# sidfeels/cosmos-predict2.5

Measured on AMD Instinct MI355X. Metric: frames/sec, Predict2.5-2B Image2World 720p×121f, 35 UniPC steps, CP=1/8, higher is better.
Workload: dtype bf16

## Files before the change

cosmos-predict2.5_amd/cosmos_predict2/_native.py:

```python

from __future__ import annotations

import ctypes
import os
from typing import Dict, NamedTuple, Optional, Tuple

import torch

_DEFAULT_LIB_PATH = os.path.join(os.path.dirname(os.path.abspath(__file__)), "_lib", "libcp25.so")
_LIB_PATH = _DEFAULT_LIB_PATH
_lib: Optional[ctypes.CDLL] = None

c_int64_p = ctypes.POINTER(ctypes.c_int64)


class UniPCParams(ctypes.Structure):

    _fields_ = [
        ("sigma", ctypes.c_float),
        ("use_corr", ctypes.c_int),
        ("order_c", ctypes.c_int),
        ("c_a", ctypes.c_float),
        ("c_b", ctypes.c_float),
        ("c_c", ctypes.c_float),
        ("c_inv_rk", ctypes.c_float),
        ("c_rho0", ctypes.c_float),
        ("c_rho_last", ctypes.c_float),
        ("order_p", ctypes.c_int),
        ("p_a", ctypes.c_float),
        ("p_b", ctypes.c_float),
        ("p_c", ctypes.c_float),
        ("p_inv_rk", ctypes.c_float),
        ("p_rho0", ctypes.c_float),
    ]


class CP25Tensor(ctypes.Structure):

    _fields_ = [
        ("data", ctypes.c_void_p),
        ("dtype", ctypes.c_int32),
        ("ndim", ctypes.c_int32),
        ("shape", ctypes.c_int64 * 6),
        ("strides", ctypes.c_int64 * 6),
    ]


DT_BF16, DT_F32, DT_F8E4M3, DT_U8 = 1, 2, 3, 4
_DTYPES = {torch.bfloat16: DT_BF16, torch.float32: DT_F32, torch.float8_e4m3fn: DT_F8E4M3, torch.uint8: DT_U8}

_P = ctypes.c_void_p
_I64 = ctypes.c_int64
_I = ctypes.c_int
_F = ctypes.c_float
_D = ctypes.c_double
_T =ctypes.POINTER(CP25Tensor)

SIGNATURES = {
    "cp25_attn_fwd": [_P, _P, _P, _P, _I, _I, _I, _I, _I, c_int64_p, c_int64_p, c_int64_p, c_int64_p, _F, _P],
    "cp25_attn_fwd_split": [_P, _P, _P, _P, _I, _I, _I, _I, _I, c_int64_p, c_int64_p, c_int64_p, c_int64_p, _F, _I,
                            _P, ctypes.c_size_t, _P],
    "cp25_attn_fwd_bounded": [_P, _P, _P, _P, _I, _I, _I, _I, _I, c_int64_p, c_int64_p, c_int64_p, c_int64_p, _F, _F,
                              _F, _I, _P, ctypes.c_size_t, _P],
    "cp25_attn_fwd_prescaled_kslots": [_P, _P, _P, _P, _I, _I, _I, _I, _I, c_int64_p, c_int64_p, c_int64_p, c_int64_p,
                                       _F, _F, _P, _I, _I, _P, ctypes.c_size_t, _P],
    "cp25_attn_fwd_prescaled": [_P, _P, _P, _P, _I, _I, _I, _I, _I, c_int64_p, c_int64_p, c_int64_p, c_int64_p, _F,
                                _F, _I, _P, ctypes.c_size_t, _P],
    "cp25_attn_fwd_prescaled_fp8qk": [_P, _P, _P, _P, _I, _I, _I, _I, _I, c_int64_p, c_int64_p, c_int64_p, c_int64_p, _F,
                                _F, _I, _P, ctypes.c_size_t, _P],
    "cp25_cast_fp8_e4m3": [_P, _I64, _P, _I64, _I64, _I64, _F, _P],
    "cp25_attn_fwd_prescaled_fp8": [_P, _P, _P, _P, _P, _I, _I, _I, _I, _I, c_int64_p, c_int64_p, c_int64_p, _F, _F, _I,
                                    _P, ctypes.c_size_t, _P],
    "cp25_v_fp8t_bytes": [_I, _I, _I],
    "cp25_cast_v_fp8t": [_P, c_int64_p, _I, _I, _I, _I, _P, _P, _P],
    "cp25_attn_fwd_prescaled_qnorm": [_P, _P, _P, _P, _I, _I, _I, _I, _I, c_int64_p, c_int64_p, c_int64_p, c_int64_p, _F,
                                      _F, _P, _I, _P, _P, _P, _F, _F, _I, _P, ctypes.c_size_t, _P],
    "cp25_attn_workspace_bytes": [_I, _I, _I, _I],
    "cp25_attn_tail_workspace_bytes": [_I, _I, _I, _I],
    "cp25_attn_kernel": [_I, _F, _F, _F, _I, _I],
    "cp25_attn_plan": [_I, _I, _I, _I, _I],
    "cp25_attn_na3d": [_P, _P, _P, _P, _I, _I, _I, _I, _I, _I, c_int64_p, c_int64_p, c_int64_p, c_int64_p, _P, _P, _I, _I,
                       ctypes.POINTER(ctypes.c_int), ctypes.POINTER(ctypes.c_int), _F, _I, _P],
    "cp25_ln_mod": [_P, _I64, _I64, _P, _P, _P, _P, _I64, _I64, _P, _P, _I64, _I, _I, _I64, _I64, _F, _P],
    "cp25_ln_mod_fp8": [_P, _I64, _I64, _P, _P, _P, _P, _I64, _I64, _P, _P, _P, _I64, _I, _I, _I64, _I64, _F, _P],
    "cp25_ln_mod_cam": [_P, _I64, _I64, _P, _P, _P, _P, _I64, _I64, _P, _I64, _I64, _P, _P, _I64, _I, _I, _I64, _I64, _F,
                        _P],
    "cp25_ln_mod_cam_fp8": [_P, _I64, _I64, _P, _P, _P, _P, _I64, _I64, _P, _I64, _I64, _P, _P, _P, _I64, _I, _I, _I64,
                            _I64, _F, _P],
    "cp25_plucker_tokens": [_P, _P, _P, _I, _I, _I, _P],
    "cp25_final_ln_mod": [_P, _P, _P, _I64, _I64, _P, _P, _I64, _I64, _P, _I64, _I, _I, _I64, _I64, _F, _P],
    "cp25_layer_norm": [_P, _I64, _P, _P, _P, _I64, _I64, _I, _F, _P],
    "cp25_head_rmsnorm_rope": [_P, _I64, _I64, _I, _I, _I, _P, _P, _P, _P, _I64, _F, _P],
    "cp25_head_rmsnorm_rope_scaled": [_P, _I64, _I64, _I, _I, _I, _P, _P, _P, _P, _I64, _F, _F, _P],
    "cp25_head_rmsnorm_rope_nmax": [_P, _I64, _I64, _I, _I, _I, _P, _P, _P, _P, _I64, _F, _F, _P, _P],
    "cp25_copy_rows": [_P, _I64, _P, _I64, _I64, _I64, _P],
    "cp25_gelu": [_P, _I64, _P],
    "cp25_gemm_epi": [_P, _I64, _P, _I64, _P, _I64, _I, _I, _I, _I, _P],
    "cp25_gemm_f32": [_P, _I64, _I64, _P, _I64, _I64, _P, _I64, _I64, _P, _I64, _I64, _I, _I, _I, _I, _I, _P, _I64,
                      _P],
    "cp25_gemm_f32_workspace_floats": [_I, _I, _I, _I],
    "cp25_gemm_hnorm": [_P, _I64, _P, _I64, _P, _I64, _I, _I, _I, _P, _F, _F, _P],
    "cp25_gemm_qkv": [_P, _I64, _P, _I64, _P, _I64, _I, _I, _I, _I, _I, _P, _P, _P, _I, _F, _P],
    "cp25_gemm_res": [_P, _I64, _P, _I64, _P, _I64, _I, _I, _I, _P, _I64, _I64, _P, _I64, _I64, _I, _I64, _I64, _P],
    "cp25_gemm_sm_epi": [_P, _I64, _P, _I64, _P, _I64, _I, _I, _I, _I, _I, _P, _I64, _P],
    "cp25_gemm_sm_res": [_P, _I64, _P, _I64, _P, _I64, _I, _I, _I, _P, _I64, _I64, _P, _I64, _I64, _I, _I64, _I64, _I, _P,
                         _I64, _P],
    "cp25_gemm_sm_hnorm": [_P, _I64, _P, _I64, _P, _I64, _I, _I, _I, _P, _F, _F, _I, _P, _I64, _P],
    "cp25_gemm_sm_qkv": [_P, _I64, _P, _I64, _P, _I64, _I, _I, _I, _I, _I, _P, _P, _P, _I, _F, _I, _P, _I64, _P],
    "cp25_gemm_sm_plan": [_I, _I, _I, _I, _I],
    "cp25_gemm_sm_workspace_bytes": [_I, _I, _I, _I],
    "cp25_gemm_fp8": [_P, _I64, _P, _P, _I64, _P, _P, _I64, _I, _I, _I, _P],
    "cp25_gemm_fp8_res": [_P, _I64, _P, _P, _I64, _P, _P, _I64, _I, _I, _I, _P, _I64, _I64, _P, _I64, _I64, _I, _I64,
                          _I64, _P],
    "cp25_quant_fp8_rows": [_P, _P, _P, _I64, _I64, _P],
    "cp25_gelu_quant_fp8": [_P, _P, _P, _I64, _I64, _P],
    "cp25_patchify": [_P, _P, _P, _P, _P, _I64, _I64, _I64, _P],
    "cp25_patchify_ld": [_P, _P, _P, _P, _P, _I64, _I64, _I64, _I64, _P],
    "cp25_cfg_velocity": [_P, _I, _P, _P, _P, _F, _I, _P, _I64, _I64, _I64, _P],
    "cp25_trig_patchify_ld": [_P, _P, _P, _P, _D, _P, _P, _I64, _I64, _I64, _I64, _P],
    "cp25_trig_x0_step": [_P, _P, _P, _P, _P, _P, _P, _I, _D, _D, _D, _I, _I64, _I64, _I64, _P],
    "cp25_kv_put": [_P, _I64, _I64, _I64, _I64, _P, _P, _I64, _I64, _I64, _I, _I64, _I64, _P],
    "cp25_stream_patchify_ld": [_P, _F, _F, _P, _P, _I64, _I64, _P],
    "cp25_stream_x0_step": [_P, _P, _P, _P, _F, _F, _F, _F, _D, _I, _I64, _P],
    "cp25_unipc_step": [_P, _P, _P, _P, _P, _I64, ctypes.POINTER(UniPCParams), _P],
    "cp25_conv3d": [ctypes.POINTER(ctypes.c_void_p), _I, _P, _P, _P, _P, _I, _I, _I, _I, _I, _I, _I, _I, _I, _I,
                    _I, _I, _I, _I, _I, _I, _P],
    "cp25_rms_norm_silu": [_P, _P, _P, _I64, _I, _I, _P],
    "cp25_conv3d_select": [_I],
    "cp25_attn_cross_select": [_I],
    "cp25_attn_self_select": [_I],
    "cp25_softmax_rows": [_P, _I64, _I, _I64, _F, _P, _I64, _P],
    "cp25_vae_attn": [_P, _I64, _I64, _P, _I64, _I64, _P, _I64, _I64, _P, _I64, _I64, _I, _I, _I, _I, _F, _P, _I64,
                      _P],
    "cp25_vae_attn_workspace_bytes": [_I, _I, _I, _I],
    "cp25_attn_fwd_t": [_T, _T, _T, _T, _F, _P, ctypes.c_size_t, _P],
    "cp25_gemm_epi_t": [_T, _T, _T, _I, _P],
    "cp25_conv3d_t": [_T, _I, _T, _T, _T, _I, _I, _I, _I, _I, _I, _P],
    "cp25_resize_crop_u8": [_P, c_int64_p, _I, _I, _I, _I, _P, c_int64_p, _P, _P, _P, _I, _P, _P, _P, _I, _I, _I, _I,
                            _I, _I, _I, _P],
    "cp25_u8_to_clip": [_P, c_int64_p, _I, _I, _I, _I, _P, _P],
    "cp25_clip_to_u8": [_P, c_int64_p, _I, _I, _I, _I, _P, c_int64_p, _P],
    "cp25_lora_merge": [_P, _I64, _P, _P, _I64, _I64, _I, _F, _P],
}


def library_path() -> str:
    return _LIB_PATH


def load_library() -> ctypes.CDLL:
    global _lib
    if _lib is not None:
        return _lib
    if not os.path.exists(_LIB_PATH):
        raise RuntimeError(
            f"libcp25.so not found at {_LIB_PATH}: build it with `make -C cosmos-predict2.5_amd/csrc` "
            "(or __graft_entry__.build()). There is no non-native fallback."
        )
    lib = ctypes.CDLL(_LIB_PATH)
    lab = os.path.abspath(_LIB_PATH) != os.path.abspath(_DEFAULT_LIB_PATH)
    for name, argtypes in SIGNATURES.items():
        fn = getattr(lib, name, None)
        if fn is None:
            if argtypes is None or lab:
                continue
            raise RuntimeError(f"libcp25.so does not export {name}")
        if argtypes is not None:
            fn.argtypes = argtypes
        fn.restype = {"cp25_attn_workspace_bytes": ctypes.c_size_t, "cp25_attn_tail_workspace_bytes": ctypes.c_size_t, "cp25_v_fp8t_bytes": ctypes.c_int64,
                      "cp25_gemm_f32_workspace_floats": ctypes.c_int64,
                      "cp25_gemm_sm_workspace_bytes": ctypes.c_int64,
                      "cp25_attn_kernel": ctypes.c_char_p,
                      "cp25_vae_attn_workspace_bytes": ctypes.c_int64}.get(name, ctypes.c_int)
    _lib = lib
    return lib


_ERRORS = {-22: "invalid shape/stride/pointer", -95: "unsupported dtype/size", -5: "kernel launch failed"}


def _check(name: str, rc: int) -> None:
    if rc != 0:
        msg = f"{name} failed with code {rc} ({_ERRORS.get(rc, 'unknown')})"
        if rc == -5:
            raise RuntimeError(msg)
        raise ValueError(msg)


def _ptr(t: Optional[torch.Tensor]) -> Optional[int]:
    if t is None:
        return None
    if not t.is_cuda:
        raise RuntimeError("cp25 kernels need device (HBM) tensors; got a CPU tensor")
    return t.data_ptr()


def _stream(device: torch.device) -> int:
    return torch.cuda.current_stream(device).cuda_stream


def tensor_desc(t: Optional[torch.Tensor]) -> Optional[CP25Tensor]:
    if t is None:
        return None
    if t.dim() > 6:
        raise ValueError(f"cp25_tensor holds at most 6 dimensions, got {t.dim()}")
    if t.dtype not in _DTYPES:
        raise ValueError(f"no cp25 dtype for {t.dtype}")
    d = CP25Tensor()
    d.data = _ptr(t)
    d.dtype = _DTYPES[t.dtype]
    d.ndim = t.dim()
    for i in range(t.dim()):
        d.shape[i] = t.shape[i]
        d.strides[i] = t.stride(i)
    return d


def _ref(d: Optional[CP25Tensor]):
    return None if d is None else ctypes.byref(d)


def attn_fwd_t(q: torch.Tensor, k: torch.Tensor, v: torch.Tensor, o: torch.Tensor, softmax_scale: float,
               workspace: Optional[torch.Tensor] = None) -> torch.Tensor:
    lib = load_library()
    ws = 0 if workspace is None else workspace.numel() * workspace.element_size()
    _check("cp25_attn_fwd_t", lib.cp25_attn_fwd_t(*(_ref(tensor_desc(t)) for t in (q, k, v, o)), float(softmax_scale),
                                                  _ptr(workspace), ws, _stream(q.device)))
    return o


def gemm_epi_t(a: torch.Tensor, w: torch.Tensor, c: torch.Tensor, epilogue: int = 0) -> torch.Tensor:
    lib = load_library()
    _check("cp25_gemm_epi_t", lib.cp25_gemm_epi_t(_ref(tensor_desc(a)), _ref(tensor_desc(w)), _ref(tensor_desc(c)),
                                                  int(epilogue), _stream(a.device)))
    return c


def conv3d_t(x: torch.Tensor, weight: torch.Tensor, bias: Optional[torch.Tensor], out: torch.Tensor, *,
             pad_front: int = 0, stride_t: int = 1, stride_hw: int = 1, pad: tuple = (0, 0, 0, 0)) -> torch.Tensor:
    lib = load_library()
    _check("cp25_conv3d_t", lib.cp25_conv3d_t(_ref(tensor_desc(x)), int(pad_front), _ref(tensor_desc(weight)),
                                              _ref(tensor_desc(bias)), _ref(tensor_desc(out)), stride_t, stride_hw,
                                              pad[0], pad[1], pad[2], pad[3], _stream(x.device)))
    return out


def _i64x3(vals) -> ctypes.Array:
    arr = (ctypes.c_int64 * 3)(*[int(v) for v in vals])
    return arr


_ATTN_SPLIT: Optional[int] = int(os.environ["CP25_ATTN_SPLIT"]) if os.environ.get("CP25_ATTN_SPLIT") else None


def set_attn_split(n: Optional[int]) -> Optional[int]:
    global _ATTN_SPLIT
    prev, _ATTN_SPLIT = _ATTN_SPLIT, (None if n is None else int(n))
    return prev


def attn_plan(B: int, H: int, Lq: int, Lk: int, D: int = 128) -> int:
    n = load_library().cp25_attn_plan(B, H, Lq, Lk, D)
    _check("cp25_attn_plan", min(n, 0))
    return n


def attn_fwd(q: torch.Tensor, k: torch.Tensor, v: torch.Tensor, out: Optional[torch.Tensor] = None,
             softmax_scale: Optional[float] = None, n_split: Optional[int] = None,
             norm_bounds: Optional[Tuple[float, float]] = None, prescaled: bool = False,
             fp8_qk: Optional[Tuple[torch.Tensor, torch.Tensor]] = None,
             fp8_v: Optional[Tuple[torch.Tensor, torch.Tensor]] = None,
             k_norm_slots: Optional[torch.Tensor] = None, q_norm: Optional[dict] = None) -> torch.Tensor:
    lib = load_library()
    if q.dtype != torch.bfloat16 or k.dtype != torch.bfloat16 or v.dtype != torch.bfloat16:
        raise ValueError("attn_fwd expects bf16 q/k/v (attention() recasts to bf16 first)")
    B, Lq, H, D = q.shape
    Bk, Lk, Hk, Dk = k.shape
    if (Bk, Hk, Dk) != (B, H, D) or tuple(v.shape) != tuple(k.shape):
        raise ValueError(f"shape mismatch q{tuple(q.shape)} k{tuple(k.shape)} v{tuple(v.shape)}")
    for t in (q, k, v):
        if t.stride(3) != 1:
            raise ValueError("head dim must be contiguous")
    if out is None:
        out = torch.empty((B, Lq, H, D), dtype=torch.bfloat16, device=q.device)
    scale = float(D) ** -0.5 if softmax_scale is None else float(softmax_scale)
    planned = n_split is None and not _ATTN_SPLIT
    if n_split is None:
        n_split = min(_ATTN_SPLIT, (Lk + 63) // 64) if _ATTN_SPLIT else attn_plan(B, H, Lq, Lk, D)
    ws_bytes = lib.cp25_attn_workspace_bytes(B, H, Lq, n_split)
    if planned and n_split == 1 and fp8_qk is None and k_norm_slots is None:
        ws_bytes = lib.cp25_attn_tail_workspace_bytes(B, H, Lq, Lk)
    ws = torch.empty(((ws_bytes + 15) // 16 * 4,), dtype=torch.float32, device=q.device) if ws_bytes else None
    qb, kb = (0.0, 0.0) if norm_bounds is None else (float(norm_bounds[0]), float(norm_bounds[1]))
    if not (qb >= 0.0 and kb >= 0.0):
        raise ValueError(f"norm_bounds must be >= 0, got {norm_bounds}")
    strides = [_i64x3((t.stride(0), t.stride(1), t.stride(2))) for t in (q, k, v, out)]
    if prescaled:
        if fp8_qk is not None:
            if q_norm is not None:
                raise ValueError("q_norm: the fp8 forms read e4m3 copies of the normalised q")
            if qb * kb > 60.0 or qb <= 0.0 or kb <= 0.0:
                raise ValueError(f"fp8 Q K^T needs norm bounds with product <= 60, got {norm_bounds}")
            q8, k8 = fp8_qk
            if q8.dtype != torch.uint8 or k8.dtype != torch.uint8 or q8.shape != q.shape or k8.shape != k.shape:
                raise ValueError("fp8_qk: uint8 (e4m3 bit pattern) views shaped like q and k expected")
            if q8.stride(3) != 1 or k8.stride(3) != 1:
                raise ValueError("fp8_qk: head dim must be contiguous")
            strides[0] = _i64x3((q8.stride(0), q8.stride(1), q8.stride(2)))
            strides[1] = _i64x3((k8.stride(0), k8.stride(1), k8.stride(2)))
            if fp8_v is not None:
                if 1.13 * qb * kb > 30.0:
                    raise ValueError(f"fp8 P.V needs 1.13 x the norm-bound product <= 30, got {norm_bounds}")
                v8t, amax = fp8_v
                if v8t.dtype != torch.uint8 or v8t.numel() != lib.cp25_v_fp8t_bytes(B, H, Lk) or \
                        amax.dtype != torch.float32 or amax.numel() < B * H:
                    raise ValueError("fp8_v: (v8t uint8 of cp25_v_fp8t_bytes, v_amax float32 [B*H]) expected")
                rc = lib.cp25_attn_fwd_prescaled_fp8(_ptr(q8), _ptr(k8), _ptr(v8t), _ptr(amax), _ptr(out), B, H, Lq, Lk,
                                                     D, strides[0], strides[1], strides[3], qb, kb, int(n_split),
                                                     _ptr(ws), ws_bytes, _stream(q.device))
                _check("cp25_attn_fwd_prescaled_fp8", rc)
                return out
            rc = lib.cp25_attn_fwd_prescaled_fp8qk(_ptr(q8), _ptr(k8), _ptr(v), _ptr(out), B, H, Lq, Lk, D, *strides,
                                                   qb, kb, int(n_split), _ptr(ws), ws_bytes, _stream(q.device))
            _check("cp25_attn_fwd_prescaled_fp8qk", rc)
            return out
        if k_norm_slots is not None:
            if k_norm_slots.dtype != torch.float32 or k_norm_slots.numel() != 2048 or not k_norm_slots.is_contiguous():
                raise ValueError("k_norm_slots: a contiguous float32 [64, 32] slot buffer expected")
        if q_norm is not None:
            w, cos, sin = q_norm["weight"], q_norm.get("cos"), q_norm.get("sin")
            if w.dtype != torch.bfloat16 or w.numel() != D or not w.is_contiguous() or w.device != q.device:
                raise ValueError("q_norm: weight must be a contiguous bf16 [128] device tensor")
            if (cos is None) != (sin is None):
                raise ValueError("q_norm: cos and sin go together")
            if cos is not None:
                for t in (cos, sin):
                    if t.dtype != torch.float32 or not t.is_contiguous() or t.dim() != 2 or t.shape[1] != 64 or \
                            t.shape[0] < Lq or t.device != q.device:
                        raise ValueError(f"q_norm: cos/sin must be contiguous float32 [>= {Lq}, 64] device tables")
            rc = lib.cp25_attn_fwd_prescaled_qnorm(
                _ptr(q), _ptr(k), _ptr(v), _ptr(out), B, H, Lq, Lk, D, *strides, qb, kb, _ptr(k_norm_slots),
                64 if k_norm_slots is not None else 0, _ptr(w), _ptr(cos), _ptr(sin), float(q_norm.get("eps", 1e-6)),
                float(q_norm.get("out_scale", 1.0)), int(n_split), _ptr(ws), ws_bytes, _stream(q.device))
            _check("cp25_attn_fwd_prescaled_qnorm", rc)
            return out
        if k_norm_slots is not None:
            rc = lib.cp25_attn_fwd_prescaled_kslots(_ptr(q), _ptr(k), _ptr(v), _ptr(out), B, H, Lq, Lk, D, *strides, qb,
                                                    kb, _ptr(k_norm_slots), 64, int(n_split), _ptr(ws), ws_bytes,
                                                    _stream(q.device))
            _check("cp25_attn_fwd_prescaled_kslots", rc)
            return out
        rc = lib.cp25_attn_fwd_prescaled(_ptr(q), _ptr(k), _ptr(v), _ptr(out), B, H, Lq, Lk, D, *strides, qb, kb,
                                         int(n_split), _ptr(ws), ws_bytes, _stream(q.device))
        _check("cp25_attn_fwd_prescaled", rc)
        return out
    if q_norm is not None:
        raise ValueError("q_norm needs prescaled=True (the DiT's attention form)")
    rc = lib.cp25_attn_fwd_bounded(
        _ptr(q), _ptr(k), _ptr(v), _ptr(out), B, H, Lq, Lk, D,
        _i64x3((q.stride(0), q.stride(1), q.stride(2))),
        _i64x3((k.stride(0), k.stride(1), k.stride(2))),
        _i64x3((v.stride(0), v.stride(1), v.stride(2))),
        _i64x3((out.stride(0), out.stride(1), out.stride(2))),
        scale, qb, kb, int(n_split), _ptr(ws), ws_bytes, _stream(q.device),
    )
    _check("cp25_attn_fwd_bounded", rc)
    return out


NA_TILE_ROWS = 128


def attn_na3d(q: torch.Tensor, k: torch.Tensor, v: torch.Tensor, plan, out: Optional[torch.Tensor] = None,
              softmax_scale: Optional[float] = None, prescaled: bool = False) -> torch.Tensor:
    lib = load_library()
    if q.dtype != torch.bfloat16 or k.dtype != torch.bfloat16 or v.dtype != torch.bfloat16:
        raise ValueError("attn_na3d expects bf16 q/k/v")
    if q.dim() != 4 or tuple(k.shape) != tuple(q.shape) or tuple(v.shape) != tuple(q.shape):
        raise ValueError(f"attn_na3d: q/k/v [B, L, H, D] of one shape expected, got q{tuple(q.shape)} "
                         f"k{tuple(k.shape)} v{tuple(v.shape)}")
    B, L, H, D = q.shape
    T, Hg, Wg = (int(x) for x in plan.grid)
    if L != T * Hg * Wg:
        raise ValueError(f"attn_na3d: {L} tokens do not fill the plan's grid {tuple(plan.grid)}")
    for t in (q, k, v):
        if t.stride(3) != 1:
            raise ValueError("head dim must be contiguous")
    q_tok, box = plan.q_tok, plan.box
    if q_tok.dtype != torch.int32 or box.dtype != torch.int32 or not q_tok.is_contiguous() or not box.is_contiguous() \
            or q_tok.dim() != 2 or q_tok.shape[1] != NA_TILE_ROWS or tuple(box.shape) != (q_tok.shape[0], 4) \
            or q_tok.device != q.device or box.device != q.device:
        raise ValueError(f"attn_na3d: plan tables must be contiguous int32 q_tok [n, {NA_TILE_ROWS}] and box [n, 4] "
# ... 882 lines not shown
```

cosmos-predict2.5_amd/cosmos_predict2/dit.py:

```python
from __future__ import annotations

import math
from dataclasses import dataclass
from typing import Dict, List, Optional, Tuple

import torch
import torch.nn.functional as F

from . import _native as N
from .checkpoint import LoraAdapters, split_lora_state_dict
from .context_parallel import all_gather_into_async, kv_chunk_views, run_lanes
from .net_config import DiTConfig
from .sparse_attn import PlanCache, sparse_block_params

BF16 = torch.bfloat16
F32 = torch.float32


def state_dict_shapes(cfg: DiTConfig) -> Dict[str, Tuple[Tuple[int, ...], torch.dtype]]:
    D, A, Ctx = cfg.model_channels, cfg.adaln_lora_dim, cfg.crossattn_emb_channels
    hd = cfg.head_dim
    dim_h = hd // 6 * 2
    dim_t = hd - 2 * dim_h
    len_max = max(cfg.max_img_h // cfg.patch_spatial, cfg.max_img_w // cfg.patch_spatial,
# ... 195 lines not shown
            return self
        return Geometry(T=len(self.frames), Hp=self.Hp, Wp=self.Wp, tok0=0, n_tok=self.n_tok, n_views=self.n_views)

    @property
    def T_view(self) -> int:
        return self.T // self.n_views

    @property
    def L_view(self) -> int:
        return self.L // self.n_views

    @property
    def hw(self) -> int:
        return self.Hp * self.Wp

    @property
    def L(self) -> int:
        return self.T * self.Hp * self.Wp


def _require_gemm(w: torch.Tensor, what: str = "projection") -> None:
    n_out, k = w.shape
    if not N.gemm_supported(n_out, k):
        raise ValueError(f"{what} weight [{n_out}, {k}]: the own GEMM needs N % 256 == 0 and K % 64 == 0")


def _rows(h, m: int):
    return h if isinstance(h, tuple) else h.view(m, -1)


class MinimalV1LVGDiT:

    def __init__(self, cfg: DiTConfig, device="cuda"):
        if cfg.head_dim != 128:
            raise ValueError("the MI355X attention kernel is built for head_dim 128 (2B and 14B both use it)")
        if cfg.patch_temporal != 1 or cfg.patch_spatial != 2 or cfg.out_channels != 16:
            raise ValueError("patch (1,2,2) with 16 latent channels is the layout this build serves")
        self.cfg = cfg
        self.device = torch.device(device)
        self.sd: Dict[str, torch.Tensor] = {}
        self._rope_cache: Dict[Tuple[int, int, int], Tuple[torch.Tensor, torch.Tensor]] = {}
        self.cp_group = None
        self.force_lanes = False
        self.attn_events: Optional[list] = None
        self.comm_events: Optional[list] = None
        self.linear_precision = "bf16"
        self._fp8_w: Dict[str, Tuple[torch.Tensor, torch.Tensor]] = {}
        self.lora_info: List[dict] = []
        self._borrowed: set = set()
        self.exact_q_rounding = False
        self.attention_precision = "bf16"
        self.share_cfg_block0 = True
        self.data_tight_k_bound = True
        self.fused_q_norm = True
        self._x_embed_w128 = None
        self.stream_gemm = "tile256"
        self.stream_gemm_force_split: Optional[int] = None
        self._sg: Optional[str] = None
        self._sg_plans: Dict[Tuple[int, int, int, int], "N.GemmSmPlan"] = {}
        self.sparse_params = sparse_block_params(cfg.num_blocks, cfg.n_dense_blocks, cfg.natten_parameters or None)
        self.has_sparse_blocks = any(sp is not None for sp in self.sparse_params)
        if self.has_sparse_blocks and (cfg.n_cameras_emb or cfg.cross_view_attn_map):
            raise NotImplementedError("sparse (neighborhood) self-attention is not built for multi-view / cross-view "
                                      "nets")
        self._na_plans = PlanCache(self.device)
        self.camera_cache = "all"
        if cfg.camera_dim:
            for other, what in ((self.has_sparse_blocks, "sparse (neighborhood) blocks"),
                                (cfg.action_dim, "action embedders"),
                                (cfg.n_cameras_emb or cfg.cross_view_attn_map or cfg.adaln_view_embedding,
                                 "a multi-view net")):
                if other:
                    raise ValueError(f"a camera-conditioned net (camera_dim = {cfg.camera_dim}) combined with {what} "
                                     "is not built")
            if not N.gemm_supported(cfg.model_channels, cfg.camera_dim):
                raise ValueError(f"cam_encoder weight [{cfg.model_channels}, {cfg.camera_dim}]: the own GEMM needs "
                                 "N % 256 == 0 and K % 64 == 0")

    def set_linear_precision(self, precision: str) -> None:
        if precision not in ("bf16", "fp8"):
            raise ValueError(f"linear precision must be 'bf16' or 'fp8', got {precision!r}")
        self.linear_precision = precision
        self._fp8_w = {}

    STREAM_GEMM_MODES = ("tile256", "small", "small_splitk")

    def _check_stream_gemm(self) -> None:
        if self.stream_gemm not in self.STREAM_GEMM_MODES:
            raise ValueError(f"stream_gemm must be one of {self.STREAM_GEMM_MODES}, got {self.stream_gemm!r}")
        if self.stream_gemm != "tile256" and self.linear_precision == "fp8":
            raise ValueError(f"stream_gemm={self.stream_gemm!r} with linear_precision='fp8': the small-M GEMMs are bf16 "
                             "only (a small-M fp8 form is not built)")
        fs = self.stream_gemm_force_split
        if fs is not None and (not isinstance(fs, int) or fs < 1):
            raise ValueError(f"stream_gemm_force_split must be None or an int >= 1, got {fs!r}")

    def set_stream_gemm(self, mode: str) -> None:
        old, self.stream_gemm = self.stream_gemm, mode
        try:
            self._check_stream_gemm()
        except ValueError:
            self.stream_gemm = old
            raise

    def _sm_split(self, M: int, w: torch.Tensor, epilogue: int) -> Optional[int]:
        if self._sg is None:
# ... 266 lines not shown
        self.refresh_norm_bounds()
        self._rope_cache.clear()

    def refresh_norm_bounds(self) -> None:
        cfg, p = self.cfg, self.sd
        hd = cfg.head_dim

        def nb(w: torch.Tensor) -> float:
            return float(w.float().abs().max()) * hd ** 0.5 * 1.02

        self.attn_bounds = [(nb(p[f"blocks.{i}.self_attn.q_norm.weight"]), nb(p[f"blocks.{i}.self_attn.k_norm.weight"]))
                            for i in range(cfg.num_blocks)]
        self.xattn_bounds = [(nb(p[f"blocks.{i}.cross_attn.q_norm.weight"]),
                              nb(p[f"blocks.{i}.cross_attn.k_norm.weight"])) for i in range(cfg.num_blocks)]
        if cfg.cross_view_attn_map:
            self.cvattn_bounds = [(nb(p[f"blocks.{i}.cross_view_attn.q_norm.weight"]),
                                   nb(p[f"blocks.{i}.cross_view_attn.k_norm.weight"])) for i in range(cfg.num_blocks)]

    def _sparse_plan(self, i: int, geo: "Geometry", cp_size: int = 1, kv=None, cv_nbrs=None):
        sp = self.sparse_params[i]
        if sp is None:
            return None
        if cp_size > 1:
            raise NotImplementedError("sparse (neighborhood) self-attention under context parallelism (cp_size > 1) is "
                                      "not built")
        if kv is not None:
            raise NotImplementedError("sparse (neighborhood) self-attention over a K/V cache (forward_frame) is not "
                                      "built")
        if self.attention_precision != "bf16":
            raise NotImplementedError("fp8 attention is not built for sparse (neighborhood) blocks")
        if cv_nbrs is not None or geo.n_views > 1 or geo.frames is not None:
            raise NotImplementedError("sparse (neighborhood) self-attention is not built for multi-view inputs")
        if geo.tok0 != 0 or geo.n_tok != geo.L:
            raise NotImplementedError("sparse (neighborhood) self-attention needs the whole token grid on one rank")
        if geo.T == 1:
            return None
        return self._na_plans.get((geo.T, geo.Hp, geo.Wp), sp)

    def attention_kernels(self, L: int) -> Dict[str, str]:
        hd = self.cfg.head_dim
        out = {}
        if self.has_sparse_blocks:
            pre = self._self_attn_mode(0, hd)[1].get("prescaled", False)
            out["sparse"] = "attn_na3d<box, %sonline max>" % ("prescaled, " if pre else "")
            out["sparse_blocks"] = ",".join(str(i) for i, sp in enumerate(self.sparse_params) if sp is not None)
        for name, bounds, lk in (("self", self.attn_bounds[0], L), ("cross", self.xattn_bounds[0], 512)):
            _, kw = self._attn_mode(bounds, hd)
            fp8 = 0
            if name == "self" and kw.get("prescaled") and self.attention_precision != "bf16":
                qb, kb = kw["norm_bounds"]
                fp8 = 0 if qb * kb > 60.0 else (2 if self.attention_precision == "fp8" and 1.13 * qb * kb <= 30.0 else 1)
            pre = kw.get("prescaled", False)
            if name == "self" and self._k_slots(kw) is not None and self.cp_group is None:
                pre = 2
            out[name] = N.attn_kernel_name(lk, kw.get("softmax_scale"), kw["norm_bounds"], pre, fp8)
        return out

    def state_dict_keys(self) -> List[str]:
        return list(state_dict_shapes(self.cfg).keys())

    def enable_context_parallel(self, process_group) -> None:
        self.cp_group = process_group

    def disable_context_parallel(self) -> None:
        self.cp_group = None

    @property
    def is_context_parallel_enabled(self) -> bool:
        return self.cp_group is not None

    @torch.no_grad()
    def prepare_context(self, crossattn_emb: torch.Tensor) -> ContextCache:
        cfg = self.cfg
        p = self.sd
        B, Lc, c_in = crossattn_emb.shape
        if cfg.use_crossattn_projection:
            ctx = self._bias_linear(crossattn_emb.reshape(B * Lc, c_in), "crossattn_proj.0", N.EPI_GELU)
        else:
            ctx = crossattn_emb.to(device=self.device, dtype=BF16).reshape(B * Lc, c_in).contiguous()
        H, hd = cfg.num_heads, cfg.head_dim
        ks, vs = [], []
        for i in range(cfg.num_blocks):
            wk, wv = p[f"blocks.{i}.cross_attn.k_proj.weight"], p[f"blocks.{i}.cross_attn.v_proj.weight"]
            _require_gemm(wk, "cross-attention k_proj")
            _require_gemm(wv, "cross-attention v_proj")
            k = N.gemm_epi(ctx, wk)
            N.head_rmsnorm_rope(k, n_rows=B * Lc, B=1, H=H, head_off=0,
                                weight=p[f"blocks.{i}.cross_attn.k_norm.weight"])
            v = N.gemm_epi(ctx, wv)
            ks.append(k.view(B, Lc, H, hd))
            vs.append(v.view(B, Lc, H, hd))
        return ContextCache(B=B, k=ks, v=vs)

    @torch.no_grad()
    def prepare_camera(self, camera_rows: torch.Tensor, geo: Geometry,
                       camera_cache: Optional[str] = None) -> CameraCache:
        cfg = self.cfg
        if not cfg.camera_dim:
            raise ValueError("prepare_camera on a net without cam_encoder (camera_dim = 0)")
        mode = self.camera_cache if camera_cache is None else camera_cache
        if mode not in ("all", "none"):
            raise ValueError(f"camera_cache must be 'all' or 'none', got {mode!r}")
        if camera_rows.dim() == 4:
            camera_rows = camera_rows.reshape(-1, camera_rows.shape[-1])
        n = geo.n_tok or geo.L
        if camera_rows.dim() != 2 or tuple(camera_rows.shape) != (n, cfg.camera_dim):
            raise ValueError(f"camera rows {tuple(camera_rows.shape)}: expected [{n}, {cfg.camera_dim}] for the "
# ... 454 lines not shown
            return m[..., :D], m[..., D:2 * D], m[..., 2 * D:]

        common = dict(n_tok=n, B=B, tok0=geo.tok0, hw=geo.hw)
        lnk = dict(common, fp8=self.linear_precision == "fp8")
        lnk1 = dict(lnk, B=1)

        def cam_kw(i):
            return {} if camera is None else dict(cam=self._cam_emb(camera, i))

        if prefix is None:
            sh, sc, _ = mod(0, 0, 1 if share0 else None)
            x = x_in
            h = N.ln_mod(x, sh, sc, x_st=x_in.stride(0), x_sb=0 if Bx == 1 else x_in.stride(1),
                         **cam_kw(0), **(lnk1 if share0 else lnk))
        else:
            x, h = prefix
        y = None
        gate_prev = None
        for i in range(cfg.num_blocks):
            pre = f"blocks.{i}."
            Bs = 1 if (share0 and i == 0) else B
            if prefix is not None and i == 0:
                pass
            else:
                o = torch.empty((n, Bs, D), dtype=BF16, device=self.device)
                ev = None
                if self.attn_events is not None:
                    ev = (torch.cuda.Event(enable_timing=True), torch.cuda.Event(enable_timing=True))
                plan = self._sparse_plan(i, geo, cp_size if cp is not None else 1, kv, cv_nbrs)
                if plan is not None:
                    q_scale, attn_kw = self._self_attn_mode(i, hd)
                    qkv = self._qkv_k_normed(h, i, n * Bs, Bs, cos, sin)
                    N.head_rmsnorm_rope(qkv, n_rows=n * Bs, B=Bs, H=H, head_off=0,
                                        weight=p[pre + "self_attn.q_norm.weight"], cos=cos, sin=sin, out_scale=q_scale)
                    q3 = qkv.view(n, Bs, 3 * D)
                    q, kk, vv = (q3[:, :, c * D:(c + 1) * D].view(n, Bs, H, hd).transpose(0, 1) for c in range(3))
                    if ev is not None:
                        ev[0].record()
                    N.attn_na3d(q, kk, vv, plan, out=o.view(n, Bs, H, hd).transpose(0, 1),
                                softmax_scale=attn_kw.get("softmax_scale"), prescaled=attn_kw.get("prescaled", False))
                    lk = plan.keys_per_query
                elif cp is None or cp_size == 1:
                    q_scale, attn_kw = self._self_attn_mode(i, hd)
                    kslots = self._k_slots(attn_kw) if kv is None else None
                    qkv = self._qkv_k_normed(h, i, n * Bs, Bs, cos, sin, kslots)
                    if self._q_norm_in_attention(attn_kw):
                        attn_kw = dict(attn_kw, q_norm=dict(weight=p[pre + "self_attn.q_norm.weight"], cos=cos, sin=sin,
                                                            out_scale=q_scale))
                    else:
                        N.head_rmsnorm_rope(qkv, n_rows=n * Bs, B=Bs, H=H, head_off=0,
                                            weight=p[pre + "self_attn.q_norm.weight"], cos=cos, sin=sin,
                                            out_scale=q_scale)
                    if kslots is not None:
                        attn_kw = dict(attn_kw, k_norm_slots=kslots)
                    q = qkv.view(n, Bs, 3 * D)[:, :, :D].view(n, Bs, H, hd).transpose(0, 1)
                    kk = qkv.view(n, Bs, 3 * D)[:, :, D:2 * D].view(n, Bs, H, hd).transpose(0, 1)
                    vv = qkv.view(n, Bs, 3 * D)[:, :, 2 * D:].view(n, Bs, H, hd).transpose(0, 1)
                    if kv is not None:
                        cache, slot, n_valid = kv
                        N.kv_put(qkv, cache.k[i], cache.v[i], B=Bs, k_col0=D, v_col0=2 * D, row0=slot * n)
                        kk, vv = cache.k[i][:, : n_valid * n], cache.v[i][:, : n_valid * n]
                    else:
                        attn_kw = self._fp8_qk(qkv[:, :D], qkv[:, D:2 * D], Bs, H, hd, attn_kw, vv)
                    if ev is not None:
                        ev[0].record()
                    if cv_nbrs is not None:
                        self._per_view_attention(q, kk, vv, o.view(n, Bs, H, hd).transpose(0, 1), geo, attn_kw)
                    else:
                        N.attn_fwd(q, kk, vv, out=o.view(n, Bs, H, hd).transpose(0, 1), **attn_kw)
                    lk = kk.shape[1] if cv_nbrs is None else geo.L_view
                else:
                    yield from self._cp_self_attention(i, h, o, cos, sin, n, B, cp, cp_size,
                                                       ev[0] if ev is not None else None,
                                                       views=geo if cv_nbrs is not None else None)
                    lk = cp_size * (n if cv_nbrs is None else geo.L_view)
                if ev is not None:
                    ev[1].record()
                    self.attn_events.append((ev[0], ev[1], 4.0 * Bs * H * n * lk * hd))
                nb = 1 if Bs == 1 and B > 1 else None
                _, _, g_sa = mod(i, 0, nb)
                sh, sc, _ = mod(i, 1, nb)
                if i == 0:
                    x_st, x_sb = x_in.stride(0), (0 if Bx == 1 else x_in.stride(1))
                else:
                    x_st, x_sb = B * D, D
                wo = p[pre + "self_attn.output_proj.weight"]
                if cv_nbrs is not None:
                    fused = self._fused_res(o.view(n * Bs, D), wo, Bs, geo.hw)
                    x, _ = self._proj_res(o.view(n * Bs, D), wo, pre + "self_attn.output_proj", x, x_st, x_sb, g_sa, Bs,
                                          geo, n, lnk, None if fused else sh, None if fused else sc)
                    x, h = self._cross_view(i, x, B, geo, cv_nbrs, mods[i, 1], lnk, sh, sc)
                else:
                    x, h = self._proj_res(o.view(n * Bs, D), wo, pre + "self_attn.output_proj", x, x_st, x_sb, g_sa, Bs,
                                          geo, n, lnk, sh, sc)
            if prefix_only:
                return x, h
            xq_scale, xattn_kw = self._attn_mode(self.xattn_bounds[i], hd)
            hq, wq = _rows(h, n * Bs), p[pre + "cross_attn.q_proj.weight"]
            qc = None
            if self._own(hq, wq):
                S = self._sm_split(hq.shape[0], wq, N.EPI_HNORM)
                if S is not None:
                    qc = N.gemm_sm_hnorm(hq, wq, p[pre + "cross_attn.q_norm.weight"], out_scale=xq_scale, split=S)
                else:
                    qc = N.gemm_hnorm(hq, wq, p[pre + "cross_attn.q_norm.weight"], out_scale=xq_scale)
            if qc is None:
                qc = self._proj(hq, wq, pre + "cross_attn.q_proj")
# ... 164 lines not shown
```

cosmos-predict2.5_amd/csrc/attn_common.h:

```cpp
#pragma once
#include "cp25_common.h"
#include "attn_route.h"

#include <algorithm>
#include <type_traits>

namespace cp25attn {

constexpr int kWaves = 8;
constexpr int kQRows = 32;
static_assert(kQBlk == kWaves * kQRows && kThreads == kWaves * 64, "attn_route.h's launch geometry");

typedef __attribute__((address_space(3))) const char* lds_char_ptr;

typedef float f32x2 __attribute__((ext_vector_type(2)));
typedef __bf16 bf16x2v __attribute__((ext_vector_type(2)));
__device__ __forceinline__ f32x2 hn2_sumsq8(const f32x2* x) {
#pragma clang fp contract(off)
  f32x2 ss = {0.f, 0.f};
#pragma unroll
  for (int e = 0; e < 8; ++e) ss += x[e] * x[e];
  return ss;
}
__device__ __forceinline__ f32x2 hn2_norm(f32x2 x, f32x2 rstd, f32x2 w) {
// ... 10 lines not shown
template <int N, int I = 0, class F>
__device__ __forceinline__ void static_for(F&& f) {
  if constexpr (I < N) {
    f(std::integral_constant<int, I>{});
    static_for<N, I + 1>(f);
  }
}

__device__ __forceinline__ int lane_fresh() {
  int l;
  asm volatile("v_mbcnt_lo_u32_b32 %0, -1, 0\n\tv_mbcnt_hi_u32_b32 %0, -1, %0" : "=v"(l));
  return l;
}

__device__ __forceinline__ float wave_swap_sum(float x) {
  auto r = __builtin_amdgcn_permlane32_swap(__float_as_uint(x), __float_as_uint(x), false, false);
  return __uint_as_float(r[0]) + __uint_as_float(r[1]);
}
__device__ __forceinline__ float group4_sum(float x) {
  x += __shfl_xor(x, 16);
  return x + __shfl_xor(x, 32);
}
__device__ __forceinline__ float group4_max(float x) {
  auto r = __builtin_amdgcn_permlane16_swap(__float_as_uint(x), __float_as_uint(x), false, false);
  x = fmaxf(__uint_as_float(r[0]), __uint_as_float(r[1]));
  auto s = __builtin_amdgcn_permlane32_swap(__float_as_uint(x), __float_as_uint(x), false, false);
  return fmaxf(__uint_as_float(s[0]), __uint_as_float(s[1]));
}

struct AttnArgs {
  const unsigned short* q; const unsigned short* k; const unsigned short* v; unsigned short* o;
  int64_t q_sb, q_sl, q_sh;
  int64_t k_sb, k_sl, k_sh;
  int64_t v_sb, v_sl, v_sh;
  int64_t o_sb, o_sl, o_sh;
  int B, H, Lq, Lk;
  int nqb;
  int nsplit;
  int tps;
  int ntk_v;
  const float* v_amax;
  float s_init;
  float* o_part;
  float* lse_part;
  float scale_log2;
  float kbound;
  const float* kslots;
  int n_kslots;
  const unsigned short* qn_w;
  const float* qn_cos;
  const float* qn_sin;
  float qn_eps, qn_scale;
  int qn_row0;
#ifdef CP25_ATTN_PROBE
  unsigned long long* probe;
  int probe_t0, probe_wg;
#endif
};

constexpr int kKStride16 = 288;
constexpr int kVStride16 = 288;
constexpr int kKBuf16 = kKBlk * kKStride16;
constexpr int kVBuf16 = kKBlk * kVStride16;
constexpr int kLds16 = 2 * kKBuf16 + 2 * kVBuf16;

typedef void (*AttnKernel)(AttnArgs);
AttnKernel wq_kernel(int rows, int mode, bool tail);

}
```

cosmos-predict2.5_amd/csrc/attn_fwd.hip:

```cpp
#include "attn_common.h"

namespace {
using namespace cp25attn;

constexpr int kAheadDefault = 2;

constexpr bool kQCopyStagger = true;
constexpr int kOStr = 264;
constexpr int kQSlot = kQRows * kOStr;
constexpr int kLdsP = kLds16 + kWaves * kQSlot;

template <int kKind, bool kPre, int kMode, bool kPersist = false, int kGate = 0, int kTail = 0>
__global__ void __launch_bounds__(kThreads, 2) attn_fwd_m16(AttnArgs a) {
  __shared__ __attribute__((aligned(16))) char smem[kPersist ? kLdsP : kLds16];
  constexpr int KB1 = kKBuf16, VB0 = 2 * kKBuf16;
  static_assert(kMode >= 0 && kMode <= 2 && (kMode != 1 || kPre), "kMode: 0 fixed, 1 zero shift, 2 online");
  static_assert(!kPersist || (kKind == 1 && kMode != 0), "persistent form: cross-attention, zero shift or online");
  constexpr bool online = kMode == 2;
  constexpr bool kInit = kPre && kMode != 1;
  constexpr int kAhead = !kPersist ? 3 : kAheadDefault;

  const int tile = xcd_remap(blockIdx.x, gridDim.x);
  int blk0 = 0, blk_end = 0;
  if constexpr (kPersist) {
// ... 61 lines not shown
      const int bh_t = (blk0 + tb) / a.nqb;
      const int b_t = bh_t / a.H, h_t = bh_t % a.H;
      base = group_b ? (const char*)(a.k + b_t * a.k_sb + h_t * a.k_sh) : (const char*)(a.v + b_t * a.v_sb + h_t * a.v_sh);
    } else {
      kt = t;
      base = sbase;
    }
    const int rows = (kPersist && t >= ntiles) ? 0 : min(Lk - kt * kKBlk, kKBlk);
    const int nbytes = rows > 0 ? (int)((rows - 1) * sl * 2) + 2 * kD : 0;
    const auto rsrc = __builtin_amdgcn_make_buffer_rsrc((void*)(base + (int64_t)kt * kKBlk * sl * 2), (short)0, nbytes,
                                                        0x00020000);
    int off = st_off;
    if constexpr (kPersist) {
      const int uf = ((wave_u & 3) << 6) + lane_fresh();
      off = (uf >> 4) * (int)(sl * 2) + (uf & 15) * 16;
    }
#pragma unroll
    for (int i = 0; i < 4; ++i)
      st[i] = __builtin_bit_cast(u32x4, __builtin_amdgcn_raw_buffer_load_b128(rsrc, off + i * st_step, 0, 0));
  };
  char* const k_wr = smem + srow * kKStride16 + sch * 16;
  char* const v_wr = smem + VB0 + srow * kVStride16 + sch * 16;

  constexpr bool kDmaK = !kPersist;
  constexpr bool kDmaV = kDmaK;
  const int wb = wave_u & 3;
  int dma_off[5];
#pragma unroll
  for (int j = 0; j < 5; ++j) {
    const int bb = 1024 * (wb + 4 * j) + 16 * lane;
    const int row = bb / kKStride16, cb = bb - row * kKStride16;
    dma_off[j] = cb < 2 * kD ? row * (int)(sl * 2) + cb : 0;
  }
  auto dma_tile = [&](int t, auto BUF) __attribute__((always_inline)) {
    constexpr int kb = decltype(BUF)::value ? KB1 : 0;
    const char* tsrc = sbase + (int64_t)t * kKBlk * sl * 2;
    const int rows = min(Lk - t * kKBlk, kKBlk);
    if (rows <= 0) return;
    const unsigned lds0 = (unsigned)(uintptr_t)(lds_char_ptr)(smem + (group_b ? kb : VB0 + (kb ? kVBuf16 : 0)));
#pragma unroll
    for (int j = 0; j < 5; ++j) {
      if (wb + 4 * j >= 18) break;
      int off = dma_off[j];
      if (__builtin_expect(rows < kKBlk, 0)) {
        const int bb = 1024 * (wb + 4 * j) + 16 * lane;
        const int row = bb / kKStride16, cb = bb - row * kKStride16;
        off = cb < 2 * kD ? min(row, rows - 1) * (int)(sl * 2) + cb : 0;
      }
      asm volatile("s_mov_b32 m0, %2\n\ts_nop 0\n\tglobal_load_lds_dwordx4 %0, %1" ::"v"(off), "s"(tsrc),
                   "s"(lds0 + 1024 * (wb + 4 * j)) : "memory");
    }
  };

  if constexpr (kDmaK) {
    if (group_b) {
      dma_tile(0, std::integral_constant<int, 0>{});
      if (ntiles > 1) dma_tile(1, std::integral_constant<int, 1>{});
    } else if constexpr (kDmaV) {
      dma_tile(0, std::integral_constant<int, 0>{});
    }
  }

  int q_row[2];
  bf16x8 qf[2][4];
#pragma unroll
  for (int qh = 0; qh < 2; ++qh) {
    q_row[qh] = qb * kQBlk + wave * kQRows + 16 * qh + c16;
    const unsigned short* src = qp + (int64_t)min(q_row[qh], a.Lq - 1) * a.q_sl + 8 * g;
#pragma unroll
    for (int s = 0; s < 4; ++s) qf[qh][s] = *reinterpret_cast<const bf16x8*>(src + 32 * s);
  }
  if constexpr (!kPersist) {
    if (a.qn_w != nullptr) {
      bf16x8 wv[4];
#pragma unroll
      for (int s = 0; s < 4; ++s) wv[s] = *reinterpret_cast<const bf16x8*>(a.qn_w + 32 * s + 8 * g);
      const bool rope = a.qn_cos != nullptr;
      f32x4 rc[2][2][2], rsn[2][2][2];
      if (rope) {
#pragma unroll
        for (int qh = 0; qh < 2; ++qh) {
          const int64_t t0 = (a.qn_row0 + min(q_row[qh], a.Lq - 1)) * 64 + 8 * g;
#pragma unroll
          for (int s1 = 0; s1 < 2; ++s1)
#pragma unroll
            for (int hf = 0; hf < 2; ++hf) {
              rc[qh][s1][hf] = *reinterpret_cast<const f32x4*>(a.qn_cos + t0 + 32 * s1 + 4 * hf);
              rsn[qh][s1][hf] = *reinterpret_cast<const f32x4*>(a.qn_sin + t0 + 32 * s1 + 4 * hf);
            }
        }
      }
      const f32x2 scale2 = {a.qn_scale, a.qn_scale};
#pragma unroll
      for (int qh = 0; qh < 2; ++qh) {
        f32x2 x[4][4];
#pragma unroll
        for (int s = 0; s < 4; ++s)
#pragma unroll
          for (int q = 0; q < 4; ++q)
            x[s][q] = f32x2{static_cast<float>(qf[qh][s][2 * q]), static_cast<float>(qf[qh][s][2 * q + 1])};
        f32x2 c01[8], c23[8];
#pragma unroll
        for (int e = 0; e < 8; ++e) {
          c01[e] = f32x2{x[0][e >> 1][e & 1], x[1][e >> 1][e & 1]};
          c23[e] = f32x2{x[2][e >> 1][e & 1], x[3][e >> 1][e & 1]};
        }
        const f32x2 p01 = hn2_sumsq8(c01), p23 = hn2_sumsq8(c23);
        const f32x2 aa = p01 + p23;
        float ss = aa.x + aa.y;
        ss += __shfl_xor(ss, 32);
        ss += __shfl_xor(ss, 16);
        const float rstd = hn_rstd(ss, a.qn_eps);
        const f32x2 rstd2 = {rstd, rstd};
#pragma unroll
        for (int s = 0; s < 4; ++s)
#pragma unroll
          for (int q = 0; q < 4; ++q)
            x[s][q] = hn2_norm(x[s][q], rstd2,
                               f32x2{static_cast<float>(wv[s][2 * q]), static_cast<float>(wv[s][2 * q + 1])});
        f32x2 y[4][4];
#pragma unroll
        for (int s = 0; s < 4; ++s)
#pragma unroll
          for (int q = 0; q < 4; ++q) y[s][q] = x[s][q];
        if (rope) {
#pragma unroll
          for (int s = 0; s < 4; ++s)
#pragma unroll
            for (int q = 0; q < 4; ++q) {
              const f32x4 cc = rc[qh][s & 1][q >> 1], sn = rsn[qh][s & 1][q >> 1];
              const int o = 2 * (q & 1);
              y[s][q] = hn2_rope(x[s][q], x[s ^ 2][q], s < 2 ? -1.f : 1.f, f32x2{cc[o], cc[o + 1]},
                                 f32x2{sn[o], sn[o + 1]});
            }
        }
#pragma unroll
        for (int s = 0; s < 4; ++s)
#pragma unroll
          for (int q = 0; q < 4; ++q) {
            const bf16x2v h = __builtin_convertvector(y[s][q] * scale2, bf16x2v);
            qf[qh][s][2 * q] = h.x;
            qf[qh][s][2 * q + 1] = h.y;
          }
      }
    }
  }

  float gate_kbound = a.kbound;
  if constexpr (kGate != 0) {
    static_assert(kPre && !kPersist && ((kGate == 1 && kMode == 0) || (kGate == 2 && kMode == 2)), "gated pair");
    __shared__ float gate_max[kWaves];
    float km = lane < a.n_kslots ? a.kslots[32 * lane] : 0.f;
    float qm = 0.f;
#pragma unroll
    for (int qh = 0; qh < 2; ++qh) {
      float qq = 0.f;
#pragma unroll
      for (int s = 0; s < 4; ++s)
#pragma unroll
        for (int e = 0; e < 8; ++e) {
          const float x = static_cast<float>(qf[qh][s][e]);
          qq = fmaf(x, x, qq);
        }
      qm = fmaxf(qm, sqrtf(group4_sum(qq)));
    }
#pragma unroll
    for (int m = 32; m >= 1; m >>= 1) {
      km = fmaxf(km, __shfl_xor(km, m));
      qm = fmaxf(qm, __shfl_xor(qm, m));
    }
    if (lane == 0) gate_max[wave] = qm;
    __syncthreads();
#pragma unroll
    for (int w = 0; w < kWaves; ++w) qm = fmaxf(qm, gate_max[w]);
    const bool fixed_ok = km > 0.f && qm * km * 1.001f <= kGateFixed;
    gate_kbound = km * 1.001f;
    if (fixed_ok != (kGate == 1)) {
      if constexpr (kDmaK) asm volatile("s_waitcnt vmcnt(0)" ::: "memory");
      return;
    }
  }

  f32x4 o[8][2];
#pragma unroll
  for (int d = 0; d < 8; ++d)
#pragma unroll
    for (int qh = 0; qh < 2; ++qh) o[d][qh] = f32x4{0.f, 0.f, 0.f, 0.f};
  f32x4 lsum[2] = {{0.f, 0.f, 0.f, 0.f}, {0.f, 0.f, 0.f, 0.f}};
  typedef short s16x8v __attribute__((ext_vector_type(8)));
  const bf16x8 ones8 = __builtin_bit_cast(bf16x8, s16x8v{0x3f80, 0x3f80, 0x3f80, 0x3f80, 0x3f80, 0x3f80, 0x3f80, 0x3f80});

  const float cs = kPre ? 1.f : a.scale_log2;
  float m_run[2] = {0.f, 0.f};
  if constexpr (kMode == 0) {
#pragma unroll
    for (int qh = 0; qh < 2; ++qh) {
      float qq = 0.f;
#pragma unroll
      for (int s = 0; s < 4; ++s)
#pragma unroll
        for (int e = 0; e < 8; ++e) {
          const float x = static_cast<float>(qf[qh][s][e]);
          qq = fmaf(x, x, qq);
// ... 331 lines not shown
#ifdef CP25_ATTN_PROBE
      probe_t = t;
#endif
      ATTN_STAMP(t, 0);
      if constexpr (kDmaK) {
        if (t + 2 < ntiles) dma_tile(t + 2, PAR);
      } else {
        if (t + 2 < ntiles) write_k(PAR);
      }
      softmax(t);
      if constexpr (!kDmaK) {
        if (t + 2 < ntiles) load_tile(t + 3);
      }
      ATTN_STAMP(t, 1);
      static_for<kAhead>([&](auto NC) __attribute__((always_inline)) { issue_pair(PAR, NC); });
      asm volatile("s_waitcnt lgkmcnt(%0)" ::"i"(2 * kAhead) : "memory");
      __builtin_amdgcn_s_barrier();
      asm volatile("" ::: "memory");
#ifdef CP25_ATTN_PROBE
      if (probe_on && (unsigned)(t - a.probe_t0) < 32u) asm volatile("s_memtime %0" : "=s"(probe_b2)::"memory");
#endif
      mfma_phase(PAR, std::true_type{});
      if constexpr (kDmaK) asm volatile("s_waitcnt vmcnt(0)" ::: "memory");
      __syncthreads();
    };
    for (int t = 0; t + 1 < ntiles; t += 2) {
      step(B0{}, t);
      step(B1{}, t + 1);
    }
    if (ntiles & 1) step(B0{}, ntiles - 1);
  }

#ifdef CP25_ATTN_PROBE
  if (probe_on) {
    asm volatile("s_memtime %0\n\ts_memrealtime %1\n\ts_waitcnt lgkmcnt(0)" : "=s"(probe_clk[2]), "=s"(probe_clk[3])::"memory");
    for (int i = lane; i < 128; i += 64)
      a.probe[((size_t)blockIdx.x * kWaves + wave_u) * 128 + i] = probe_lds[wave_u * 128 + i];
    if (lane < 5)
      a.probe[(size_t)a.probe_wg * kWaves * 128 + ((size_t)blockIdx.x * kWaves + wave_u) * 8 + lane] =
          lane == 0 ? probe_clk[0] : lane == 1 ? probe_clk[1] : lane == 2 ? probe_clk[2] : lane == 3 ? probe_clk[3]
                                                                                                    : probe_resc;
  }
#undef ATTN_STAMP
#endif
  if constexpr (kPersist) {
    store_block(blk_end - 1);
    return;
  }
#pragma unroll
  for (int qh = 0; qh < 2; ++qh) {
    const float l_tot = lsum[qh][0];
    const float inv = 1.f / l_tot;
    if (q_row[qh] >= a.Lq) continue;
    if (a.nsplit > 1) {
      const int64_t row = ((int64_t)(split * a.B + b) * a.H + h) * a.Lq + q_row[qh];
      float* op = a.o_part + row * kD + 4 * g;
#pragma unroll
      for (int db = 0; db < 8; ++db) {
        f32x4 w;
#pragma unroll
        for (int e = 0; e < 4; ++e) w[e] = o[db][qh][e] * inv;
        *reinterpret_cast<f32x4*>(op + 16 * db) = w;
      }
      if (g == 0) a.lse_part[row] = m_run[qh] + __log2f(l_tot);
    } else if constexpr (kKind == 1) {
      store_rows16(a.o + b * a.o_sb + h * a.o_sh + (int64_t)q_row[qh] * a.o_sl, qh, inv, g);
    } else {
      unsigned short* op = a.o + b * a.o_sb + h * a.o_sh + (int64_t)q_row[qh] * a.o_sl + 4 * g;
#pragma unroll
      for (int db = 0; db < 8; ++db) {
        u16x4 w;
#pragma unroll
        for (int e = 0; e < 4; ++e) w[e] = f2bf(o[db][qh][e] * inv);
        *reinterpret_cast<u16x4*>(op + 16 * db) = w;
      }
    }
  }
}

constexpr int kVStride = 320;
constexpr int kVBuf = kKBlk * kVStride;
constexpr int kLdsF8 = 2 * kVBuf + 2 * kKBlk * 144;

template <int kKind, int kF8>
__global__ void __launch_bounds__(kThreads, 2) attn_fwd_f8(AttnArgs a) {
  __shared__ __attribute__((aligned(16))) char smem[kLdsF8];
  static_assert(kF8 == 1 || kF8 == 3, "kF8: 1 fp8 Q K^T, 3 + fp8 P.V with P bytes without exp2");
  constexpr int KSTR = 144;
  constexpr int KB1 = kKBlk * KSTR;
  constexpr int VB0 = 2 * kKBlk * KSTR, VB1 = VB0 + kVBuf;
  constexpr int VSTR8 = 80;
  typedef int i32x8 __attribute__((ext_vector_type(8)));

  const int tile = xcd_remap(blockIdx.x, gridDim.x);
  const int qb = tile % a.nqb;
  const int bhs = tile / a.nqb;
  const int split = bhs % a.nsplit, bh = bhs / a.nsplit;
  const int b = bh / a.H, h = bh % a.H;
  const int key0 = split * a.tps * kKBlk;
  const int Lk = min(a.Lk - key0, a.tps * kKBlk);

  const int tid = threadIdx.x;
  const int lane = tid & 63;
  const int wave = tid >> 6;
  const int l31 = lane & 31;
  const int hl = lane >> 5;
// ... 276 lines not shown
}

__global__ void __launch_bounds__(256) attn_merge_splits(const float* __restrict__ o_part,
                                                        const float* __restrict__ lse_part, unsigned short* o,
                                                        int nsplit, int B, int H, int Lq, int64_t o_sb,
                                                        int64_t o_sl, int64_t o_sh) {
  const int64_t rows = (int64_t)B * H * Lq;
  const int64_t gid = (int64_t)blockIdx.x * blockDim.x + threadIdx.x;
  const int64_t row = gid >> 5;
  if (row >= rows) return;
  const int d = (int)(gid & 31) * 4;
  float mx = -INFINITY;
  for (int s = 0; s < nsplit; ++s) mx = fmaxf(mx, lse_part[s * rows + row]);
  f32x4 acc = {0.f, 0.f, 0.f, 0.f};
  float den = 0.f;
  for (int s = 0; s < nsplit; ++s) {
    const float l = lse_part[s * rows + row];
    if (!(l > -INFINITY)) continue;
    const float w = __builtin_amdgcn_exp2f(l - mx);
    const f32x4 v = *reinterpret_cast<const f32x4*>(o_part + (s * rows + row) * kD + d);
    acc += w * v;
    den += w;
  }
  const float inv = den > 0.f ? 1.f / den : 0.f;
  const int q = (int)(row % Lq);
  const int bh = (int)(row / Lq);
  const int b = bh / H, h = bh % H;
  u16x4 w;
#pragma unroll
  for (int e = 0; e < 4; ++e) w[e] = f2bf(acc[e] * inv);
  *reinterpret_cast<u16x4*>(o + b * o_sb + (int64_t)q * o_sl + h * o_sh + d) = w;
}

int g_num_cus = 0;
int num_cus() {
  if (g_num_cus == 0) {
    int dev = 0, n = 0;
    if (hipGetDevice(&dev) != hipSuccess ||
        hipDeviceGetAttribute(&n, hipDeviceAttributeMultiprocessorCount, dev) != hipSuccess || n <= 0)
      n = 256;
    g_num_cus = n;
  }
  return g_num_cus;
}

int g_self_form = 1;
int g_xattn_form = 1;

unsigned wide_built() {
  unsigned m = 0;
  for (int rows : {320, 384})
    for (int mode : {0, 1})
      if (wq_kernel(rows, mode, false)) m |= wide_bit(rows, mode);
  return m;
}

AttnQuery route_query(int Lk, bool prescaled, float softmax_scale, float q_norm_bound, float k_norm_bound, int fp8,
                      bool has_kslots, bool has_qnorm, int n_split) {
  return AttnQuery{Lk, prescaled, prescaled ? 1.f : softmax_scale * 1.4426950408889634f, q_norm_bound, k_norm_bound,
                   fp8, has_kslots, has_qnorm, n_split, g_self_form, g_xattn_form, wide_built()};
}

template <bool kPre, int kMode>
AttnKernel m16_plain(bool cross, bool tail) {
  if (tail) return attn_fwd_m16<0, kPre, kMode, false, 0, 1>;
  return cross ? attn_fwd_m16<1, kPre, kMode> : attn_fwd_m16<0, kPre, kMode>;
}
AttnKernel m16_kernel(const AttnRoute& r, bool tail) {
  const bool cross = r.kind == AttnKind::cross;
  if (r.gated) return cross ? attn_fwd_m16<1, true, 2, false, 2> : attn_fwd_m16<0, true, 2, false, 2>;
  if (r.persistent) {
    if (!r.prescaled) return attn_fwd_m16<1, false, 2, true>;
    return r.mode == 2 ? attn_fwd_m16<1, true, 2, true> : attn_fwd_m16<1, true, 1, true>;
  }
  if (!r.prescaled) return r.mode == 2 ? m16_plain<false, 2>(cross, tail) : m16_plain<false, 0>(cross, tail);
  return r.mode == 2 ? m16_plain<true, 2>(cross, tail)
                     : (r.mode == 1 ? m16_plain<true, 1>(cross, tail) : m16_plain<true, 0>(cross, tail));
}
AttnKernel m16_gate_fixed_kernel(const AttnRoute& r) {
  return r.kind == AttnKind::cross ? attn_fwd_m16<1, true, 0, false, 1> : attn_fwd_m16<0, true, 0, false, 1>;
}
AttnKernel f8_kernel(const AttnRoute& r) {
  const bool cross = r.kind == AttnKind::cross;
  if (r.f8 == 3) return cross ? attn_fwd_f8<1, 3> : attn_fwd_f8<0, 3>;
  return cross ? attn_fwd_f8<1, 1> : attn_fwd_f8<0, 1>;
}
AttnKernel route_kernel(const AttnRoute& r, bool tail) {
  if (r.family == AttnFamily::f8) return f8_kernel(r);
  return r.family == AttnFamily::wq ? wq_kernel(r.rows, r.mode, tail) : m16_kernel(r, tail);
}

}

extern "C" int cp25_attn_self_select(int form) {
  if (form != 0 && form != 1 && !wq_kernel(form, 0, false)) return CP25_ERR_INVAL;
  const int prev = g_self_form;
  g_self_form = form;
  return prev;
}

extern "C" int cp25_attn_cross_select(int form) {
  if (form != 0 && form != 1) return CP25_ERR_INVAL;
  const int prev = g_xattn_form;
  g_xattn_form = form;
  return prev;
}

#ifdef CP25_ATTN_PROBE
static unsigned long long* g_probe = nullptr;
static int g_probe_t0 = 0, g_probe_wg = 0;
extern "C" void cp25_attn_probe_set(unsigned long long* probe, int t0, int n_wg) {
  g_probe = probe;
  g_probe_t0 = t0;
  g_probe_wg = n_wg;
}
#endif

struct AttnCall {
  const void *q, *k, *v;
  void* o;
  int B, H, Lq, Lk, D;
  const int64_t *q_strides, *k_strides, *v_strides, *o_strides;
  float softmax_scale, q_norm_bound, k_norm_bound;
  int n_split;
  void* workspace;
  size_t ws_bytes;
  hipStream_t stream;
  bool prescaled;
  int fp8;
  const float* v_amax;
  const float* kslots;
  int n_kslots;
  const void* qn_w;
  const float *qn_cos, *qn_sin;
  float qn_eps, qn_scale;
};

static int attn_launch(const AttnCall& c) {
  const int B = c.B, H = c.H, Lq = c.Lq, Lk = c.Lk, fp8 = c.fp8, n_split = c.n_split;
  const float q_norm_bound = c.q_norm_bound, k_norm_bound = c.k_norm_bound;
  const bool fp8qk = fp8 >= 1;
  if (c.D != kD) return CP25_ERR_DTYPE;
  if (fp8qk && !c.prescaled) return CP25_ERR_INVAL;
  if (fp8 == 2 && (!c.v_amax || ((uintptr_t)c.v_amax & 3))) return CP25_ERR_INVAL;
  if (fp8qk && !(q_norm_bound > 0.f && k_norm_bound > 0.f && (double)q_norm_bound * k_norm_bound <= (double)kTopF8))
    return CP25_ERR_INVAL;
  if (fp8 == 2 && kF8Round * (double)q_norm_bound * k_norm_bound > kF8PvSpan) return CP25_ERR_INVAL;
  if (B <= 0 || H <= 0 || Lq <= 0 || Lk <= 0) return CP25_ERR_INVAL;
  if (!c.q || !c.k || !c.v || !c.o) return CP25_ERR_INVAL;
  if (!(c.softmax_scale > 0.f) || !(q_norm_bound >= 0.f) || !(k_norm_bound >= 0.f) || q_norm_bound > 1e18f ||
      k_norm_bound > 1e18f)
    return CP25_ERR_INVAL;
  const int64_t* ss[4] = {c.q_strides, c.k_strides, c.v_strides, c.o_strides};
  for (int i = 0; i < 4; ++i)
    for (int j = 0; j < 3; ++j)
      if (!(fp8 == 2 && i == 2) && ss[i][j] % (fp8qk && i < 2 ? 16 : 8) != 0) return CP25_ERR_INVAL;
  if ((int64_t)kKBlk * c.k_strides[1] * (fp8qk ? 1 : 2) >= (1ll << 31) ||
      (fp8 != 2 && (int64_t)kKBlk * c.v_strides[1] * 2 >= (1ll << 31)))
    return CP25_ERR_INVAL;
  if (c.k_strides[1] <= 0 || (fp8 != 2 && c.v_strides[1] <= 0)) return CP25_ERR_INVAL;
  if (((uintptr_t)c.q | (uintptr_t)c.k | (uintptr_t)c.v | (uintptr_t)c.o) & 15) return CP25_ERR_INVAL;
  const int64_t ntiles = cdiv(Lk, kKBlk);
  if (n_split < 1 || n_split > ntiles) return CP25_ERR_INVAL;
  const int64_t tps = cdiv(ntiles, n_split);
  if (cdiv(ntiles, tps) != n_split) return CP25_ERR_INVAL;
  const int64_t rows = (int64_t)B * H * Lq;
  if (n_split > 1) {
    if (!c.workspace || ((uintptr_t)c.workspace & 15) || c.ws_bytes < cp25_attn_workspace_bytes(B, H, Lq, n_split))
      return CP25_ERR_INVAL;
  }
  const AttnQuery query = route_query(Lk, c.prescaled, c.softmax_scale, q_norm_bound, k_norm_bound, fp8,
                                      c.kslots != nullptr, c.qn_w != nullptr, n_split);
  const AttnRoute route = attn_route(query);
  const int qblk = route.rows;
  const int64_t cus = num_cus();
  TailSeg tail[kMaxTailSegs];
  int n_tail = 0;
  if (n_split == 1 && fp8 == 0 && !c.kslots && c.workspace && !((uintptr_t)c.workspace & 15)) {
    size_t need = 0;
    n_tail = plan_tail(B, H, Lq, Lk, qblk, cus, tail, &need, nullptr);
    if (c.ws_bytes < need) n_tail = 0;
  }
  AttnArgs a;
  a.q = (const unsigned short*)c.q; a.k = (const unsigned short*)c.k; a.v = (const unsigned short*)c.v;
  a.o = (unsigned short*)c.o;
  a.q_sb = c.q_strides[0]; a.q_sl = c.q_strides[1]; a.q_sh = c.q_strides[2];
  a.k_sb = c.k_strides[0]; a.k_sl = c.k_strides[1]; a.k_sh = c.k_strides[2];
  a.v_sb = c.v_strides[0]; a.v_sl = c.v_strides[1]; a.v_sh = c.v_strides[2];
  a.o_sb = c.o_strides[0]; a.o_sl = c.o_strides[1]; a.o_sh = c.o_strides[2];
  a.B = B; a.H = H; a.Lq = Lq; a.Lk = Lk;
  a.nqb = (int)cdiv(Lq, qblk);
  a.nsplit = n_split;
  a.tps = (int)tps;
  a.ntk_v = (int)ntiles;
  a.v_amax = c.v_amax;
  a.s_init = fp8 == 2 ? -std::max(0.f, (float)kF8Round * q_norm_bound * k_norm_bound - 15.f) : 0.f;
  a.o_part = n_split > 1 ? (float*)c.workspace : nullptr;
  a.lse_part = n_split > 1 ? (float*)c.workspace + (size_t)n_split * rows * kD : nullptr;
  a.scale_log2 = query.scale_log2;
  a.kbound = q_norm_bound > 0.f ? k_norm_bound : 0.f;
  a.kslots = c.kslots;
  a.n_kslots = c.n_kslots;
  a.qn_w = (const unsigned short*)c.qn_w;
  a.qn_cos = c.qn_cos;
  a.qn_sin = c.qn_sin;
  a.qn_eps = c.qn_eps;
  a.qn_scale = c.qn_w ? c.qn_scale : 1.f;
  a.qn_row0 = 0;
#ifdef CP25_ATTN_PROBE
  a.probe = g_probe;
  a.probe_t0 = g_probe_t0;
  a.probe_wg = g_probe_wg;
#endif
  const int64_t nwg = (int64_t)a.nqb * B * H * n_split;
  if (nwg > 0x7fffffff) return CP25_ERR_INVAL;
  const dim3 threads(route.threads);
  int64_t grid = nwg;
  if (route.gated) {
    hipLaunchKernelGGL(m16_gate_fixed_kernel(route), dim3((unsigned)nwg), threads, 0, c.stream, a);
    CP25_LAUNCH_CHECK();
  } else if (route.persistent) {
    grid = std::min<int64_t>(nwg, cus);
  } else if (n_tail) {
    grid = nwg - nwg % cus;
  }
  hipLaunchKernelGGL(route_kernel(route, false), dim3((unsigned)grid), threads, 0, c.stream, a);
  CP25_LAUNCH_CHECK();
  for (int i = grid < nwg ? 0 : n_tail; i < n_tail; ++i) {
    const TailSeg& g = tail[i];
    const int b = g.bh / H, h = g.bh % H;
    const int64_t row0 = (int64_t)g.qb_lo * qblk;
    AttnArgs t = a;
    t.q = a.q + b * a.q_sb + h * a.q_sh + row0 * a.q_sl;
    t.k = a.k + b * a.k_sb + h * a.k_sh;
    t.v = a.v + b * a.v_sb + h * a.v_sh;
    t.o = a.o + b * a.o_sb + h * a.o_sh + row0 * a.o_sl;
    t.B = 1; t.H = 1;
    t.Lq = (int)(std::min<int64_t>(Lq, row0 + (int64_t)g.nblk * qblk) - row0);
    t.qn_row0 = (int)row0;
    t.nqb = g.nblk;
    t.nsplit = g.s;
    t.tps = (int)cdiv(ntiles, g.s);
    t.o_part = (float*)c.workspace;
    t.lse_part = (float*)c.workspace + (size_t)g.s * t.Lq * kD;
    hipLaunchKernelGGL(route_kernel(route, true), dim3((unsigned)(g.nblk * g.s)), threads, 0, c.stream, t);
    CP25_LAUNCH_CHECK();
    hipLaunchKernelGGL(attn_merge_splits, dim3((unsigned)cdiv((int64_t)t.Lq * 32, 256)), dim3(256), 0, c.stream,
                       t.o_part, t.lse_part, t.o, g.s, 1, 1, t.Lq, a.o_sb, a.o_sl, a.o_sh);
    CP25_LAUNCH_CHECK();
  }
  if (n_split > 1) {
    hipLaunchKernelGGL(attn_merge_splits, dim3((unsigned)cdiv(rows * 32, 256)), dim3(256), 0, c.stream, a.o_part,
                       a.lse_part, a.o, n_split, B, H, Lq, a.o_sb, a.o_sl, a.o_sh);
    CP25_LAUNCH_CHECK();
  }
  return CP25_OK;
}

constexpr float kLn2 = 0.6931471805599453f;

extern "C" int cp25_attn_fwd_prescaled_fp8qk(const void* q8, const void* k8, const void* v, void* o, int B, int H,
                                             int Lq, int Lk, int D, const int64_t* q_strides,
                                             const int64_t* k_strides, const int64_t* v_strides,
                                             const int64_t* o_strides, float q_norm_bound, float k_norm_bound,
                                             int n_split, void* workspace, size_t ws_bytes, hipStream_t stream) {
  return attn_launch({.q = q8, .k = k8, .v = v, .o = o, .B = B, .H = H, .Lq = Lq, .Lk = Lk, .D = D,
                      .q_strides = q_strides, .k_strides = k_strides, .v_strides = v_strides, .o_strides = o_strides,
                      .softmax_scale = kLn2, .q_norm_bound = q_norm_bound, .k_norm_bound = k_norm_bound,
                      .n_split = n_split, .workspace = workspace, .ws_bytes = ws_bytes, .stream = stream,
                      .prescaled = true, .fp8 = 1});
}
// ... 52 lines not shown
                                     float q_norm_bound, float k_norm_bound, int n_split, void* workspace,
                                     size_t ws_bytes, hipStream_t stream) {
  return attn_launch({.q = q, .k = k, .v = v, .o = o, .B = B, .H = H, .Lq = Lq, .Lk = Lk, .D = D,
                      .q_strides = q_strides, .k_strides = k_strides, .v_strides = v_strides, .o_strides = o_strides,
                      .softmax_scale = softmax_scale, .q_norm_bound = q_norm_bound, .k_norm_bound = k_norm_bound,
                      .n_split = n_split, .workspace = workspace, .ws_bytes = ws_bytes, .stream = stream});
}

extern "C" int cp25_attn_fwd_prescaled(const void* q, const void* k, const void* v, void* o, int B, int H, int Lq,
                                       int Lk, int D, const int64_t* q_strides, const int64_t* k_strides,
                                       const int64_t* v_strides, const int64_t* o_strides, float q_norm_bound,
                                       float k_norm_bound, int n_split, void* workspace, size_t ws_bytes,
                                       hipStream_t stream) {
  return attn_launch({.q = q, .k = k, .v = v, .o = o, .B = B, .H = H, .Lq = Lq, .Lk = Lk, .D = D,
                      .q_strides = q_strides, .k_strides = k_strides, .v_strides = v_strides, .o_strides = o_strides,
                      .softmax_scale = kLn2, .q_norm_bound = q_norm_bound, .k_norm_bound = k_norm_bound,
                      .n_split = n_split, .workspace = workspace, .ws_bytes = ws_bytes, .stream = stream,
                      .prescaled = true});
}

extern "C" int cp25_attn_fwd_prescaled_kslots(const void* q, const void* k, const void* v, void* o, int B, int H, int Lq,
                                              int Lk, int D, const int64_t* q_strides, const int64_t* k_strides,
                                              const int64_t* v_strides, const int64_t* o_strides, float q_norm_bound,
                                              float k_norm_bound, const float* k_norm_slots, int n_slots, int n_split,
                                              void* workspace, size_t ws_bytes, hipStream_t stream) {
  if (!k_norm_slots || n_slots < 1 || n_slots > 64 || ((uintptr_t)k_norm_slots & 3)) return CP25_ERR_INVAL;
  return attn_launch({.q = q, .k = k, .v = v, .o = o, .B = B, .H = H, .Lq = Lq, .Lk = Lk, .D = D,
                      .q_strides = q_strides, .k_strides = k_strides, .v_strides = v_strides, .o_strides = o_strides,
                      .softmax_scale = kLn2, .q_norm_bound = q_norm_bound, .k_norm_bound = k_norm_bound,
                      .n_split = n_split, .workspace = workspace, .ws_bytes = ws_bytes, .stream = stream,
                      .prescaled = true, .kslots = k_norm_slots, .n_kslots = n_slots});
}

extern "C" int cp25_attn_fwd_prescaled_qnorm(const void* q, const void* k, const void* v, void* o, int B, int H, int Lq,
                                             int Lk, int D, const int64_t* q_strides, const int64_t* k_strides,
                                             const int64_t* v_strides, const int64_t* o_strides, float q_norm_bound,
                                             float k_norm_bound, const float* k_norm_slots, int n_slots,
                                             const void* q_norm_weight, const float* cos_tab, const float* sin_tab,
                                             float eps, float q_scale, int n_split, void* workspace, size_t ws_bytes,
                                             hipStream_t stream) {
  if (k_norm_slots && (n_slots < 1 || n_slots > 64 || ((uintptr_t)k_norm_slots & 3))) return CP25_ERR_INVAL;
  if (!q_norm_weight || ((uintptr_t)q_norm_weight & 15) || (!cos_tab) != (!sin_tab) || !(eps >= 0.f) ||
      !(q_scale > 0.f))
    return CP25_ERR_INVAL;
  if ((((uintptr_t)cos_tab) | ((uintptr_t)sin_tab)) & 15) return CP25_ERR_INVAL;
  return attn_launch({.q = q, .k = k, .v = v, .o = o, .B = B, .H = H, .Lq = Lq, .Lk = Lk, .D = D,
                      .q_strides = q_strides, .k_strides = k_strides, .v_strides = v_strides, .o_strides = o_strides,
                      .softmax_scale = kLn2, .q_norm_bound = q_norm_bound, .k_norm_bound = k_norm_bound,
                      .n_split = n_split, .workspace = workspace, .ws_bytes = ws_bytes, .stream = stream,
                      .prescaled = true, .kslots = k_norm_slots, .n_kslots = k_norm_slots ? n_slots : 0,
                      .qn_w = q_norm_weight, .qn_cos = cos_tab, .qn_sin = sin_tab, .qn_eps = eps, .qn_scale = q_scale});
}

extern "C" const char* cp25_attn_kernel(int Lk, float softmax_scale, float q_norm_bound, float k_norm_bound,
                                        int prescaled, int fp8) {
  return attn_route_name(attn_route(route_query(Lk, prescaled != 0, softmax_scale, q_norm_bound, k_norm_bound, fp8,
                                                prescaled == 2, false, 1)));
}
```

cosmos-predict2.5_amd/csrc/attn_route.h:

```cpp
#pragma once
#include <algorithm>
#include <cstddef>
#include <cstdint>

namespace cp25attn {

constexpr int kD = 128;
constexpr int kQBlk = 256;
constexpr int kKBlk = 64;
constexpr int kThreads = 512;
constexpr int kWqThreads = 256;
constexpr float kTop = 96.f;
constexpr float kMaxBound = 98.f;
constexpr float kPDrop = 60.f;
constexpr float kGateFixed = 110.f;
constexpr float kTopF8 = 60.f;
constexpr float kLazy = 24.f;
constexpr double kF8Round = 1.13;
constexpr double kF8PvSpan = 30.0;
constexpr int kCrossMaxKeys = 4096;
constexpr int kWq320MaxKeys = 8192;

constexpr int64_t ceil_div(int64_t a, int64_t b) { return (a + b - 1) / b; }


enum class AttnFamily { m16, wq, f8 };
enum class AttnKind { self, cross };

constexpr unsigned wide_bit(int rows, int mode) {
  return (rows == 320 || rows == 384) && (mode == 0 || mode == 1) ? 1u << (2 * (rows == 384) + mode) : 0u;
}

struct AttnQuery {
  int Lk;
  bool prescaled;
  float scale_log2;
  float q_norm_bound, k_norm_bound;
  int fp8;
  bool has_kslots;
  bool has_qnorm;
  int n_split;
  int self_form;
  int cross_form;
  unsigned wide_built;
};

struct AttnRoute {
  AttnFamily family;
  AttnKind kind;
  bool prescaled;
  int mode;
  bool gated;
  bool persistent;
  int f8;
  int rows;
  int threads;
};

inline int wide_rows_of(int self_form, int Lk) {
  if (self_form == 0 || Lk <= kCrossMaxKeys) return 0;
  return self_form == 1 ? (Lk > kWq320MaxKeys ? 384 : 320) : self_form;
}

inline AttnRoute attn_route(const AttnQuery& q) {
  const bool cross = q.Lk <= kCrossMaxKeys;
  const double bb = (double)q.q_norm_bound * q.k_norm_bound * (q.prescaled ? 1.0 : q.scale_log2);
  int mode;
  if (!(q.q_norm_bound > 0.f && q.k_norm_bound > 0.f)) mode = 2;
  else if (!cross && bb <= kGateFixed) mode = 0;
  else if (bb > kMaxBound) mode = 2;
  else mode = q.prescaled && bb <= kTop ? 1 : 0;

  AttnRoute r{AttnFamily::m16, cross ? AttnKind::cross : AttnKind::self, q.prescaled, mode, false, false, 0, kQBlk,
              kThreads};
  if (q.prescaled && q.has_kslots && (cross ? mode != 1 : mode == 2)) {
    r.gated = true;
    r.mode = 2;
  } else if (q.fp8 != 0) {
    r.family = AttnFamily::f8;
    r.prescaled = true;
    r.mode = 0;
    r.f8 = q.fp8 == 2 ? 3 : 1;
  } else if (q.cross_form == 1 && cross && q.n_split == 1 && !q.has_qnorm && mode != 0 &&
             ceil_div(q.Lk, kKBlk) >= 2) {
    r.persistent = true;
  } else if (q.prescaled && mode != 2) {
    const int rows = wide_rows_of(q.self_form, q.Lk);
    if (rows && (q.wide_built & wide_bit(rows, mode))) {
      r.family = AttnFamily::wq;
      r.rows = rows;
      r.threads = kWqThreads;
    }
  }
  return r;
}

struct AttnRouteName { AttnFamily family; AttnKind kind; bool prescaled; int mode; bool gated, persistent; int f8, rows;
                       const char* name; };
constexpr AttnRouteName kRouteNames[] = {
    {AttnFamily::m16, AttnKind::self, false, 0, false, false, 0, 256, "attn_fwd_m16<self, fixed shift>"},
    {AttnFamily::m16, AttnKind::self, false, 2, false, false, 0, 256, "attn_fwd_m16<self, online max>"},
    {AttnFamily::m16, AttnKind::self, true, 0, false, false, 0, 256, "attn_fwd_m16<self, prescaled, fixed shift>"},
    {AttnFamily::m16, AttnKind::self, true, 1, false, false, 0, 256, "attn_fwd_m16<self, prescaled, zero shift>"},
    {AttnFamily::m16, AttnKind::self, true, 2, false, false, 0, 256, "attn_fwd_m16<self, prescaled, online max>"},
    {AttnFamily::m16, AttnKind::cross, false, 0, false, false, 0, 256, "attn_fwd_m16<cross, fixed shift>"},
    {AttnFamily::m16, AttnKind::cross, false, 2, false, false, 0, 256, "attn_fwd_m16<cross, online max>"},
    {AttnFamily::m16, AttnKind::cross, true, 0, false, false, 0, 256, "attn_fwd_m16<cross, prescaled, fixed shift>"},
    {AttnFamily::m16, AttnKind::cross, true, 1, false, false, 0, 256, "attn_fwd_m16<cross, prescaled, zero shift>"},
    {AttnFamily::m16, AttnKind::cross, true, 2, false, false, 0, 256, "attn_fwd_m16<cross, prescaled, online max>"},
    {AttnFamily::m16, AttnKind::self, true, 2, true, false, 0, 256,
     "attn_fwd_m16<self, prescaled, gated fixed shift | online max>"},
    {AttnFamily::m16, AttnKind::cross, true, 2, true, false, 0, 256,
     "attn_fwd_m16<cross, prescaled, gated fixed shift | online max>"},
    {AttnFamily::m16, AttnKind::cross, false, 2, false, true, 0, 256, "attn_fwd_m16<cross, online max, persistent>"},
    {AttnFamily::m16, AttnKind::cross, true, 1, false, true, 0, 256,
     "attn_fwd_m16<cross, prescaled, zero shift, persistent>"},
    {AttnFamily::m16, AttnKind::cross, true, 2, false, true, 0, 256,
     "attn_fwd_m16<cross, prescaled, online max, persistent>"},
    {AttnFamily::wq, AttnKind::self, true, 0, false, false, 0, 320,
     "attn_fwd_wq<self, prescaled, 320 rows, fixed shift>"},
    {AttnFamily::wq, AttnKind::self, true, 1, false, false, 0, 320,
     "attn_fwd_wq<self, prescaled, 320 rows, zero shift>"},
    {AttnFamily::wq, AttnKind::self, true, 0, false, false, 0, 384,
     "attn_fwd_wq<self, prescaled, 384 rows, fixed shift>"},
    {AttnFamily::wq, AttnKind::self, true, 1, false, false, 0, 384,
     "attn_fwd_wq<self, prescaled, 384 rows, zero shift>"},
    {AttnFamily::f8, AttnKind::self, true, 0, false, false, 1, 256, "attn_fwd_f8<self, fp8 Q K^T>"},
    {AttnFamily::f8, AttnKind::cross, true, 0, false, false, 1, 256, "attn_fwd_f8<cross, fp8 Q K^T>"},
    {AttnFamily::f8, AttnKind::self, true, 0, false, false, 3, 256, "attn_fwd_f8<self, fp8 Q K^T + fp8 P.V>"},
    {AttnFamily::f8, AttnKind::cross, true, 0, false, false, 3, 256, "attn_fwd_f8<cross, fp8 Q K^T + fp8 P.V>"},
};

inline const char* attn_route_name(const AttnRoute& r) {
  for (const AttnRouteName& n : kRouteNames)
    if (n.family == r.family && n.kind == r.kind && n.prescaled == r.prescaled && n.mode == r.mode &&
        n.gated == r.gated && n.persistent == r.persistent && n.f8 == r.f8 && n.rows == r.rows)
      return n.name;
  return nullptr;
}


inline double split_cost(int64_t nwg, int64_t ntiles, int s, int64_t rows, int64_t cus) {
  const int64_t tps = ceil_div(ntiles, s);
  double cost = (double)ceil_div(nwg * s, cus) * (double)(tps + 44);
  if (s > 1) cost += (2.0 * s + 0.5) * (double)rows * kD * 4 / 9.0e6;
  return cost;
}

struct TailSeg { int bh, qb_lo, nblk, s; };
constexpr int kMaxTailSegs = 4;
inline int plan_tail(int B, int H, int Lq, int Lk, int qblk, int64_t cus, TailSeg* seg, size_t* ws_need,
                     double* saved) {
  const int64_t nqb = ceil_div(Lq, qblk), ntiles = ceil_div(Lk, kKBlk);
  const int64_t nwg = nqb * B * H;
  const int64_t r = nwg % cus;
  *ws_need = 0;
  if (saved) *saved = 0.0;
  if (r == 0 || nwg < cus || Lk <= kCrossMaxKeys) return 0;
  int n = 0;
  double cost = 0.0;
  size_t need = 0;
  for (int64_t t = nwg - r; t < nwg;) {
    const int bh = (int)(t / nqb), qb = (int)(t % nqb);
    const int nblk = (int)std::min<int64_t>(nqb - qb, nwg - t);
    if (n == kMaxTailSegs) return 0;
    const int64_t rows = std::min<int64_t>(Lq, (int64_t)(qb + nblk) * qblk) - (int64_t)qb * qblk;
    int s = 1;
    for (int c = 2; c <= 8 && c <= ntiles; ++c) {
      const int64_t tps = ceil_div(ntiles, c);
      if (ceil_div(ntiles, tps) == c && (int64_t)nblk * c <= cus) s = c;
    }
    if (s == 1 && qblk != kQBlk) {
      double best = 1e300;
      for (int c = 2; c <= 8 && c <= ntiles; ++c) {
        const int64_t tps = ceil_div(ntiles, c);
        if (ceil_div(ntiles, tps) != c) continue;
        const double cc = split_cost(nblk, ntiles, c, rows, cus);
        if (cc < best) { best = cc; s = c; }
      }
    }
    if (s == 1) return 0;
    seg[n++] = TailSeg{bh, qb, nblk, s};
    cost += split_cost(nblk, ntiles, s, rows, cus) + 8.0;
    need = std::max<size_t>(need, (size_t)s * rows * (kD + 1) * sizeof(float));
    t += nblk;
  }
  const double unsplit = (double)(ntiles + 44);
  if (cost >= 0.9 * unsplit) return 0;
  if (qblk != kQBlk && unsplit - cost < 0.005 * (double)ceil_div(nwg, cus) * unsplit) return 0;
  *ws_need = need;
  if (saved) *saved = unsplit - cost;
  return n;
}

inline int plan_split(int B, int H, int Lq, int Lk, int qblk, int64_t cus) {
  const int64_t nqb = ceil_div(Lq, qblk), ntiles = ceil_div(Lk, kKBlk);
  const int64_t nwg = nqb * B * H;
  const int64_t rows = (int64_t)B * H * Lq;
  int best = 1;
  double best_cost = 1e300;
  for (int s = 1; s <= 8 && s <= ntiles; ++s) {
    const int64_t tps = ceil_div(ntiles, s);
    if (ceil_div(ntiles, tps) != s) continue;
    double cost = split_cost(nwg, ntiles, s, rows, cus);
    if (s == 1) {
      TailSeg seg[kMaxTailSegs];
      size_t need;
      double saved;
      if (plan_tail(B, H, Lq, Lk, qblk, cus, seg, &need, &saved) > 0) cost -= saved;
    }
    if (cost < best_cost * 0.995) { best_cost = cost; best = s; }
  }
  return best;
}

inline size_t tail_workspace_bytes(int B, int H, int Lq, int Lk, int self_form, int64_t cus) {
  TailSeg seg[kMaxTailSegs];
  size_t need = 0, best = 0;
  for (int qblk : {kQBlk, wide_rows_of(self_form, Lk)})
    if (qblk > 0 && plan_tail(B, H, Lq, Lk, qblk, cus, seg, &need, nullptr) > 0) best = std::max(best, need);
  return best;
}

}
```

cosmos-predict2.5_amd/csrc/attn_wide.hip:

```cpp
#include "attn_common.h"

namespace cp25attn {
namespace {

constexpr int kAheadWq = 2;
constexpr int kRingWq = kAheadWq + 1;
static_assert(kWqThreads == 4 * 64, "one wave per SIMD");

constexpr int wq_stage(int nq) { return 17 * nq; }
constexpr int wq_frag(int nq, int m) { return m < nq ? -1 : (m - nq) / nq; }
constexpr int wq_qb(int nq, int m) { return m < nq ? m : (m - nq) % nq; }
constexpr bool wq_read_gap(int nq, int m) { return m >= nq && (m - nq) % nq == 0; }
constexpr int wq_sm_op(int nq, int m) {
  if (wq_read_gap(nq, m)) return -1;
  int idx = 0;
  for (int x = 0; x < m; ++x) idx += !wq_read_gap(nq, x);
  return idx < 12 * nq ? idx : -1;
}
constexpr int wq_sm_count(int nq) {
  int n = 0;
  for (int m = 0; m < wq_stage(nq); ++m) n += wq_sm_op(nq, m) >= 0;
  return n;
}
static_assert(wq_sm_count(5) == 60 && wq_sm_count(6) == 72, "every softmax instruction has a gap");
constexpr int wq_dma_at(int nq, int M) {
  return M < wq_stage(nq) && wq_read_gap(nq, M) && wq_frag(nq, M) < 10 ? wq_frag(nq, M) : -1;
}
constexpr int wq_m0_at(int nq, int M) { return wq_dma_at(nq, M + 1); }

__device__ __forceinline__ u32x4 tile_rsrc(const char* base, int64_t sl, int rows) {
  const uint64_t p = (uint64_t)base;
  const unsigned n = rows > 0 ? (unsigned)((rows - 1) * sl * 2 + 2 * kD) : 0u;
  return u32x4{(unsigned)p, (unsigned)(p >> 32) & 0xffffu, n, 0x00020000u};
}

#define WQ_MFMA "v_mfma_f32_16x16x32_bf16 "

template <int kNQ, int kMode, int kTail = 0>
__global__ void __launch_bounds__(kWqThreads, 1) attn_fwd_wq(AttnArgs a) {
  static_assert(kMode == 0 || kMode == 1, "kMode: 0 fixed shift, 1 zero shift");
  static_assert(kNQ >= 4 && kNQ <= 6, "query blocks per wave");
  __shared__ __attribute__((aligned(16))) char smem[kLds16];
  constexpr bool kInit = kMode != 1;
  constexpr int KB1 = kKBuf16, VB0 = 2 * kKBuf16;
  constexpr int kR = kRingWq;
  constexpr int kRowsW = 16 * kNQ;
  constexpr int kRowsG = 4 * kRowsW;
  constexpr int kNS = wq_stage(kNQ);
  constexpr int kQA = (256 - 36 * kNQ - 4) / 16 < kNQ ? (256 - 36 * kNQ - 4) / 16 : kNQ;

  const int tile = xcd_remap(blockIdx.x, gridDim.x);
  const int qblk = tile % a.nqb;
  const int bhs = tile / a.nqb;
  const int split = bhs % a.nsplit, bh = bhs / a.nsplit;
  const int b = bh / a.H, h = bh % a.H;
  const int key0 = split * a.tps * kKBlk;
  const int Lk = min(a.Lk - key0, a.tps * kKBlk);
  const int ntk = (Lk + kKBlk - 1) / kKBlk;
  const int tid = threadIdx.x;
  const int lane = tid & 63;
  const int wave = __builtin_amdgcn_readfirstlane(tid >> 6);
  const int c16 = lane & 15;
  const int g = lane >> 4;
  const int row_w = qblk * kRowsG + wave * kRowsW;

  const unsigned short* qp = a.q + b * a.q_sb + h * a.q_sh;
  const char* const kbase = (const char*)(a.k + b * a.k_sb + h * a.k_sh + (int64_t)key0 * a.k_sl);
  const char* const vbase = (const char*)(a.v + b * a.v_sb + h * a.v_sh + (int64_t)key0 * a.v_sl);

  int dk[5], dv[5];
#pragma unroll
  for (int j = 0; j < 5; ++j) {
    const int bb = 1024 * (wave + 4 * j) + 16 * lane;
    const int row = bb / kKStride16, cb = bb - row * kKStride16;
    dk[j] = cb < 2 * kD ? row * (int)(a.k_sl * 2) + cb : 0;
    dv[j] = cb < 2 * kD ? row * (int)(a.v_sl * 2) + cb : 0;
  }
  const unsigned lds_wave = (unsigned)(uintptr_t)(lds_char_ptr)smem + 1024u * (unsigned)wave;
  auto k_rsrc = [&](int t) __attribute__((always_inline)) {
    return tile_rsrc(kbase + (int64_t)t * kKBlk * a.k_sl * 2, a.k_sl, min(Lk - t * kKBlk, kKBlk));
  };
  auto v_rsrc = [&](int t) __attribute__((always_inline)) {
    return tile_rsrc(vbase + (int64_t)t * kKBlk * a.v_sl * 2, a.v_sl, min(Lk - t * kKBlk, kKBlk));
  };
  auto set_m0 = [&](unsigned dst, auto OFFC) __attribute__((always_inline)) {
    asm volatile("s_add_u32 m0, %0, %1" ::"s"(dst), "i"(decltype(OFFC)::value) : "memory");
  };
  auto dma_load = [&](const u32x4& rs, int off) __attribute__((always_inline)) {
    asm volatile("buffer_load_dwordx4 %0, %1, 0 offen lds" ::"v"(off), "s"(rs) : "memory");
  };
  auto dma_tile = [&](const u32x4& rs, const int* offs, unsigned dst) __attribute__((always_inline)) {
    static_for<5>([&](auto JC) __attribute__((always_inline)) {
      constexpr int j = decltype(JC)::value;
      if (j < 4 || wave < 2) {
        set_m0(dst, std::integral_constant<int, 4096 * j>{});
        asm volatile("s_nop 0" ::: "memory");
        dma_load(rs, offs[j]);
      }
    });
  };

  dma_tile(k_rsrc(0), dk, lds_wave);
  dma_tile(k_rsrc(1), dk, lds_wave + KB1);
  dma_tile(v_rsrc(0), dv, lds_wave + VB0);

  bf16x8 qa[kNQ][4];
#pragma unroll
  for (int qb = 0; qb < kNQ; ++qb) {
    const int r = row_w + 16 * qb + c16;
    const unsigned short* src = qp + (int64_t)min(r, a.Lq - 1) * a.q_sl + 8 * g;
#pragma unroll
    for (int s = 0; s < 4; ++s) qa[qb][s] = *reinterpret_cast<const bf16x8*>(src + 32 * s);
  }
  if (a.qn_w != nullptr) {
    bf16x8 wv[4];
#pragma unroll
    for (int s = 0; s < 4; ++s) wv[s] = *reinterpret_cast<const bf16x8*>(a.qn_w + 32 * s + 8 * g);
    const bool rope = a.qn_cos != nullptr;
    const f32x2 scale2 = {a.qn_scale, a.qn_scale};
#pragma unroll
    for (int qb = 0; qb < kNQ; ++qb) {
      const int r = row_w + 16 * qb + c16;
      f32x4 rc[2][2], rsn[2][2];
      if (rope) {
        const int64_t t0 = (a.qn_row0 + min(r, a.Lq - 1)) * 64 + 8 * g;
#pragma unroll
        for (int s1 = 0; s1 < 2; ++s1)
#pragma unroll
          for (int hf = 0; hf < 2; ++hf) {
            rc[s1][hf] = *reinterpret_cast<const f32x4*>(a.qn_cos + t0 + 32 * s1 + 4 * hf);
            rsn[s1][hf] = *reinterpret_cast<const f32x4*>(a.qn_sin + t0 + 32 * s1 + 4 * hf);
          }
      }
      f32x2 x[4][4];
#pragma unroll
      for (int s = 0; s < 4; ++s)
#pragma unroll
        for (int q = 0; q < 4; ++q)
          x[s][q] = f32x2{static_cast<float>(qa[qb][s][2 * q]), static_cast<float>(qa[qb][s][2 * q + 1])};
      f32x2 c01[8], c23[8];
#pragma unroll
      for (int e = 0; e < 8; ++e) {
        c01[e] = f32x2{x[0][e >> 1][e & 1], x[1][e >> 1][e & 1]};
        c23[e] = f32x2{x[2][e >> 1][e & 1], x[3][e >> 1][e & 1]};
      }
      const f32x2 p01 = hn2_sumsq8(c01), p23 = hn2_sumsq8(c23);
      const f32x2 aa = p01 + p23;
      float ss = aa.x + aa.y;
      ss += __shfl_xor(ss, 32);
      ss += __shfl_xor(ss, 16);
      const float rstd = hn_rstd(ss, a.qn_eps);
      const f32x2 rstd2 = {rstd, rstd};
#pragma unroll
      for (int s = 0; s < 4; ++s)
#pragma unroll
        for (int q = 0; q < 4; ++q)
          x[s][q] = hn2_norm(x[s][q], rstd2,
                             f32x2{static_cast<float>(wv[s][2 * q]), static_cast<float>(wv[s][2 * q + 1])});
      f32x2 y[4][4];
#pragma unroll
      for (int s = 0; s < 4; ++s)
#pragma unroll
        for (int q = 0; q < 4; ++q) y[s][q] = x[s][q];
      if (rope) {
#pragma unroll
        for (int s = 0; s < 4; ++s)
#pragma unroll
          for (int q = 0; q < 4; ++q) {
            const f32x4 cc = rc[s & 1][q >> 1], sn = rsn[s & 1][q >> 1];
            const int o = 2 * (q & 1);
            y[s][q] = hn2_rope(x[s][q], x[s ^ 2][q], s < 2 ? -1.f : 1.f, f32x2{cc[o], cc[o + 1]},
                               f32x2{sn[o], sn[o + 1]});
          }
      }
#pragma unroll
      for (int s = 0; s < 4; ++s)
#pragma unroll
        for (int q = 0; q < 4; ++q) {
          const bf16x2v hh = __builtin_convertvector(y[s][q] * scale2, bf16x2v);
          qa[qb][s][2 * q] = hh.x;
          qa[qb][s][2 * q + 1] = hh.y;
        }
    }
  }

  float m_run[kNQ];
#pragma unroll
  for (int qb = 0; qb < kNQ; ++qb) m_run[qb] = 0.f;
  if constexpr (kMode == 0) {
#pragma unroll
    for (int qb = 0; qb < kNQ; ++qb) {
      float qq = 0.f;
#pragma unroll
      for (int s = 0; s < 4; ++s)
#pragma unroll
        for (int e = 0; e < 8; ++e) {
          const float x = static_cast<float>(qa[qb][s][e]);
          qq = fmaf(x, x, qq);
        }
      const float b_row = sqrtf(group4_sum(qq)) * a.kbound;
      m_run[qb] = floorf(fminf(b_row + kPDrop, 126.f - b_row));
    }
  }
  f32x4 minit[kNQ];
#pragma unroll
  for (int qb = 0; qb < kNQ; ++qb) {
    minit[qb] = f32x4{-m_run[qb], -m_run[qb], -m_run[qb], -m_run[qb]};
    asm volatile("" : "+v"(minit[qb]));
  }

  f32x4 oacc[8][kNQ], lacc[kNQ];
#pragma unroll
  for (int db = 0; db < 8; ++db)
#pragma unroll
    for (int qb = 0; qb < kNQ; ++qb) {
      oacc[db][qb] = f32x4{0.f, 0.f, 0.f, 0.f};
      asm volatile("s_nop 2" : "+a"(oacc[db][qb]));
    }
#pragma unroll
  for (int qb = 0; qb < kNQ; ++qb) {
    lacc[qb] = f32x4{0.f, 0.f, 0.f, 0.f};
    asm volatile("s_nop 2" : "+a"(lacc[qb]));
  }
  static_for<kNQ>([&](auto QC) __attribute__((always_inline)) {
    constexpr int qb = decltype(QC)::value;
    (void)qa;
#pragma unroll
    for (int s = 0; s < 4; ++s) {
      if constexpr (qb < kQA) asm volatile("s_nop 2" : "+a"(qa[qb][s]));
      else asm volatile("s_nop 2" : "+v"(qa[qb][s]));
    }
  });
  typedef short s16x8v __attribute__((ext_vector_type(8)));
  bf16x8 ones8 = __builtin_bit_cast(bf16x8, s16x8v{0x3f80, 0x3f80, 0x3f80, 0x3f80, 0x3f80, 0x3f80, 0x3f80, 0x3f80});
  asm volatile("s_nop 2" : "+a"(ones8));
  const unsigned k_rd_lds = (unsigned)(uintptr_t)(lds_char_ptr)(smem + c16 * kKStride16 + 16 * g);
  const unsigned v_rd_lds =
      (unsigned)(uintptr_t)(lds_char_ptr)(smem + VB0 + (4 * g + (c16 >> 2)) * kVStride16 + 8 * (c16 & 3));

  f32x4 S[2][2][kNQ];
  bf16x8 P[2][kNQ];
  bf16x8 ring[kR];
  float ex[2];
  unsigned pk[4];
  unsigned k_cur = 0, v_cur = 0;

  auto issue = [&](auto FC, auto SLOTC) __attribute__((always_inline)) {
    constexpr int F = decltype(FC)::value, slot = decltype(SLOTC)::value;
    constexpr int st = F / 16, f = F % 16;
    (void)ring;
    (void)k_cur;
    (void)v_cur;
    if constexpr (f >= 8) {
      constexpr int j = f - 8;
      constexpr int off = (2 * st + (j & 1)) * 16 * kKStride16 + 64 * (j >> 1);
      asm volatile("ds_read_b128 %0, %1 offset:%2" : "=v"(ring[slot]) : "v"(k_cur), "i"(off));
    } else {
      constexpr int off = 32 * st * kVStride16 + 32 * f;
      s16x4 lo, hi;
      asm volatile("ds_read_b64_tr_b16 %0, %1 offset:%2" : "=v"(lo) : "v"(v_cur), "i"(off));
      asm volatile("ds_read_b64_tr_b16 %0, %1 offset:%2" : "=v"(hi) : "v"(v_cur), "i"(off + 16 * kVStride16));
      typedef short s16x8 __attribute__((ext_vector_type(8)));
      const s16x8 r = {lo[0], lo[1], lo[2], lo[3], hi[0], hi[1], hi[2], hi[3]};
      ring[slot] = __builtin_bit_cast(bf16x8, r);
    }
  };

  auto mask_keys = [&](auto SPC, int k0) __attribute__((always_inline)) {
    constexpr int SP = decltype(SPC)::value;
    if (__builtin_expect(k0 + 32 > Lk, 0)) {
      asm volatile("s_nop 15\n\ts_nop 15" ::: "memory");
#pragma unroll
      for (int kbl = 0; kbl < 2; ++kbl)
#pragma unroll
        for (int i = 0; i < 4; ++i)
          if (k0 + 16 * kbl + 4 * g + i >= Lk) {
#pragma unroll
            for (int qb = 0; qb < kNQ; ++qb) S[SP][kbl][qb][i] = -INFINITY;
          }
    }
  };

  auto body = [&](auto FULLC, int t) __attribute__((always_inline)) {
    constexpr bool FULL = decltype(FULLC)::value;
    constexpr int NF = FULL ? 32 : 16;
    constexpr auto frag_of = [](int n) constexpr { return FULL ? n : (n < 8 ? 8 + n : 16 + n); };
    constexpr auto seq_of = [](int F) constexpr { return FULL ? F : (F < 16 ? F - 8 : F - 16); };
    constexpr auto nreads = [](int F) constexpr { return F % 16 < 8 ? 2 : 1; };
    k_cur = k_rd_lds + (((t + 1) & 1) ? (unsigned)KB1 : 0u);
    v_cur = v_rd_lds + ((t & 1) ? (unsigned)kVBuf16 : 0u);
    u32x4 rk = {0u, 0u, 0u, 0u}, rv = {0u, 0u, 0u, 0u};
    unsigned dst_k = 0, dst_v = 0;
    if constexpr (FULL) {
      mask_keys(std::integral_constant<int, 1>{}, 64 * t + 32);
      rk = k_rsrc(t + 2);
      rv = v_rsrc(t + 1);
      dst_k = lds_wave + ((t & 1) ? (unsigned)KB1 : 0u);
      dst_v = lds_wave + (unsigned)VB0 + (((t + 1) & 1) ? (unsigned)kVBuf16 : 0u);
    }
    static_for<kAheadWq>([&](auto IC) __attribute__((always_inline)) {
      constexpr int n = decltype(IC)::value;
      issue(std::integral_constant<int, frag_of(n)>{}, std::integral_constant<int, n % kR>{});
    });
    __builtin_amdgcn_sched_barrier(0);
    static_for<2 * kNS>([&](auto MC) __attribute__((always_inline)) {
      constexpr int M = decltype(MC)::value;
      constexpr int st = M / kNS, m = M % kNS;
      constexpr int f = wq_frag(kNQ, m), qb = wq_qb(kNQ, m);
      constexpr int F = 16 * st + (f < 0 ? 0 : f);
      constexpr bool has_mfma = f >= 8 || FULL;
      constexpr bool has_sm = st == 1 || FULL;
      (void)S;
      (void)ex;
      (void)pk;
      (void)oacc;
      (void)lacc;
      (void)ones8;
      (void)P;
      (void)minit;
      (void)qa;
      (void)ring;
      (void)rk;
      (void)rv;
      (void)dst_k;
      (void)dst_v;
      if constexpr (m == 0 && st == 1) {
        if constexpr (!FULL) asm volatile("s_nop 15" ::: "memory");
        mask_keys(std::integral_constant<int, 0>{}, 64 * (t + 1));
        __builtin_amdgcn_sched_barrier(0);
      }
      if constexpr (has_mfma) {
        if constexpr (f >= 0 && qb == 0) {
          constexpr int n = seq_of(F);
          constexpr int pending = [=]() constexpr {
            int p = 0;
            for (int i = 1; i < kAheadWq; ++i)
              if (n + i < NF) p += nreads(frag_of(n + i));
            return p;
          }();
          asm volatile("s_waitcnt lgkmcnt(%0)" ::"i"(pending), "v"(ring[n % kR]) : "memory");
        }
        if constexpr (f < 0) {
          asm volatile(WQ_MFMA "%0, %1, %2, %0" : "+a"(lacc[qb]) : "a"(ones8), "v"(P[st][qb]));
        } else if constexpr (f < 8) {
          asm volatile(WQ_MFMA "%0, %1, %2, %0" : "+a"(oacc[f][qb]) : "v"(ring[seq_of(F) % kR]), "v"(P[st][qb]));
        } else {
          constexpr int kbl = (f - 8) & 1, s = (f - 8) >> 1;
          constexpr int ri = seq_of(F) % kR;
          if constexpr (qb < kQA) {
            if constexpr (s == 0 && kInit)
              asm volatile(WQ_MFMA "%0, %1, %2, %3"
                           : "=&v"(S[st][kbl][qb]) : "v"(ring[ri]), "a"(qa[qb][s]), "v"(minit[qb]));
            else if constexpr (s == 0)
              asm volatile(WQ_MFMA "%0, %1, %2, 0" : "=&v"(S[st][kbl][qb]) : "v"(ring[ri]), "a"(qa[qb][s]));
            else
              asm volatile(WQ_MFMA "%0, %1, %2, %0" : "+v"(S[st][kbl][qb]) : "v"(ring[ri]), "a"(qa[qb][s]));
          } else {
            if constexpr (s == 0 && kInit)
              asm volatile(WQ_MFMA "%0, %1, %2, %3"
                           : "=&v"(S[st][kbl][qb]) : "v"(ring[ri]), "v"(qa[qb][s]), "v"(minit[qb]));
            else if constexpr (s == 0)
              asm volatile(WQ_MFMA "%0, %1, %2, 0" : "=&v"(S[st][kbl][qb]) : "v"(ring[ri]), "v"(qa[qb][s]));
            else
              asm volatile(WQ_MFMA "%0, %1, %2, %0" : "+v"(S[st][kbl][qb]) : "v"(ring[ri]), "v"(qa[qb][s]));
          }
        }
      }
      __builtin_amdgcn_sched_barrier(0);
      if constexpr (has_mfma && f >= 0 && qb == 0) {
        constexpr int n = seq_of(F) + kAheadWq;
        if constexpr (n < NF) issue(std::integral_constant<int, frag_of(n)>{}, std::integral_constant<int, n % kR>{});
      }
      if constexpr (FULL) {
        constexpr int dm = wq_m0_at(kNQ, M), dl = wq_dma_at(kNQ, M);
        if constexpr (dm >= 0) {
          constexpr int j = dm % 5;
          if (j < 4 || wave < 2) set_m0(dm < 5 ? dst_k : dst_v, std::integral_constant<int, 4096 * j>{});
        }
        if constexpr (dl >= 0) {
          constexpr int j = dl % 5;
          if (j < 4 || wave < 2) dma_load(dl < 5 ? rk : rv, dl < 5 ? dk[j] : dv[j]);
        }
      }
      if constexpr (has_sm) {
        if constexpr (!has_mfma) asm volatile("s_nop 1" ::: "memory");
        constexpr int op = wq_sm_op(kNQ, m);
        if constexpr (op >= 0) {
          constexpr int q = op / 12, r = op % 12, pair = r / 3, w = r % 3;
          if constexpr (w < 2) {
            constexpr int j = 2 * pair + w;
            asm volatile("v_exp_f32 %0, %1" : "=v"(ex[w]) : "v"(S[1 - st][j >> 2][q][j & 3]));
          } else {
            pk[pair] = __builtin_bit_cast(unsigned, __builtin_convertvector(f32x2{ex[0], ex[1]}, bf16x2v));
            asm volatile("" ::"v"(pk[pair]));
            if constexpr (pair == 3) P[1 - st][q] = __builtin_bit_cast(bf16x8, u32x4{pk[0], pk[1], pk[2], pk[3]});
          }
        }
      }
      __builtin_amdgcn_sched_barrier(0);
    });
    if constexpr (FULL) {
      static_for<kNQ>([&](auto QC) __attribute__((always_inline)) {
        constexpr int qb = decltype(QC)::value;
        (void)P;
        asm volatile("" ::"v"(P[0][qb]), "v"(P[1][qb]));
      });
    }
    asm volatile("s_waitcnt vmcnt(0)" ::: "memory");
    __builtin_amdgcn_s_barrier();
    __builtin_amdgcn_sched_barrier(0);
  };

  asm volatile("s_waitcnt vmcnt(0) lgkmcnt(0)" ::: "memory");
  __builtin_amdgcn_s_barrier();
  body(std::false_type{}, -1);
  for (int t = 0; t < ntk; ++t) body(std::true_type{}, t);

  asm volatile("s_nop 15\n\ts_nop 15" ::: "memory");
#pragma unroll
  for (int db = 0; db < 8; ++db)
#pragma unroll
    for (int qb = 0; qb < kNQ; ++qb) asm volatile("s_nop 0" : "+a"(oacc[db][qb]));
#pragma unroll
  for (int qb = 0; qb < kNQ; ++qb) asm volatile("s_nop 0" : "+a"(lacc[qb]));
#pragma unroll
  for (int qb = 0; qb < kNQ; ++qb) {
    const int q_row = row_w + 16 * qb + c16;
    const float l_tot = lacc[qb][0];
    float inv = 1.f / l_tot;
    if (l_tot > 3.0e38f) inv = __uint_as_float(0x7fc00000u);
    if (q_row >= a.Lq) continue;
    if (a.nsplit > 1) {
      const int64_t row = ((int64_t)(split * a.B + b) * a.H + h) * a.Lq + q_row;
      float* op = a.o_part + row * kD + 4 * g;
#pragma unroll
      for (int db = 0; db < 8; ++db) {
        f32x4 w;
#pragma unroll
        for (int e = 0; e < 4; ++e) w[e] = oacc[db][qb][e] * inv;
        *reinterpret_cast<f32x4*>(op + 16 * db) = w;
      }
      if (g == 0) a.lse_part[row] = m_run[qb] + __log2f(l_tot);
    } else {
      unsigned short* op = a.o + b * a.o_sb + h * a.o_sh + (int64_t)q_row * a.o_sl + 4 * g;
#pragma unroll
      for (int db = 0; db < 8; ++db) {
        u16x4 w;
#pragma unroll
        for (int e = 0; e < 4; ++e) w[e] = f2bf(oacc[db][qb][e] * inv);
        *reinterpret_cast<u16x4*>(op + 16 * db) = w;
      }
    }
  }
}

#undef WQ_MFMA

}

AttnKernel wq_kernel(int rows, int mode, bool tail) {
  if (mode != 0) return nullptr;
  if (rows == 320) return tail ? attn_fwd_wq<5, 0, 1> : attn_fwd_wq<5, 0>;
  if (rows == 384) return tail ? attn_fwd_wq<6, 0, 1> : attn_fwd_wq<6, 0>;
  return nullptr;
}

}
```

include/cp25.h:

```cpp
#ifndef CP25_H
#define CP25_H

#include <stdint.h>
#include <hip/hip_runtime_api.h>

#ifdef __cplusplus
extern "C" {
#endif

#define CP25_MAX_DIMS 6
#define CP25_DT_BF16 1
#define CP25_DT_F32 2
#define CP25_DT_F8E4M3 3
#define CP25_DT_U8 4
typedef struct cp25_tensor {
  void* data;
  int32_t dtype;
  int32_t ndim;
  int64_t shape[CP25_MAX_DIMS];
  int64_t strides[CP25_MAX_DIMS];
} cp25_tensor;

int cp25_attn_fwd_t(const cp25_tensor* q, const cp25_tensor* k, const cp25_tensor* v, const cp25_tensor* o,
                    float softmax_scale, void* workspace, size_t ws_bytes, hipStream_t stream);

int cp25_gemm_epi_t(const cp25_tensor* a, const cp25_tensor* w, const cp25_tensor* c, int epilogue,
                    hipStream_t stream);

int cp25_conv3d_t(const cp25_tensor* x, int pad_front, const cp25_tensor* weight, const cp25_tensor* bias,
                  const cp25_tensor* out, int stride_t, int stride_hw, int pad_top, int pad_left, int pad_bottom,
                  int pad_right, hipStream_t stream);

int cp25_attn_fwd(const void* q, const void* k, const void* v, void* o, int B, int H, int Lq, int Lk, int D,
                  const int64_t* q_strides, const int64_t* k_strides, const int64_t* v_strides,
                  const int64_t* o_strides, float softmax_scale, hipStream_t stream);

int cp25_attn_fwd_split(const void* q, const void* k, const void* v, void* o, int B, int H, int Lq, int Lk, int D,
                        const int64_t* q_strides, const int64_t* k_strides, const int64_t* v_strides,
                        const int64_t* o_strides, float softmax_scale, int n_split, void* workspace,
                        size_t ws_bytes, hipStream_t stream);

int cp25_attn_fwd_bounded(const void* q, const void* k, const void* v, void* o, int B, int H, int Lq, int Lk,
                          int D, const int64_t* q_strides, const int64_t* k_strides, const int64_t* v_strides,
                          const int64_t* o_strides, float softmax_scale, float q_norm_bound, float k_norm_bound,
                          int n_split, void* workspace, size_t ws_bytes, hipStream_t stream);

int cp25_attn_fwd_prescaled(const void* q, const void* k, const void* v, void* o, int B, int H, int Lq, int Lk, int D,
                            const int64_t* q_strides, const int64_t* k_strides, const int64_t* v_strides,
                            const int64_t* o_strides, float q_norm_bound, float k_norm_bound, int n_split,
                            void* workspace, size_t ws_bytes, hipStream_t stream);

int cp25_attn_fwd_prescaled_kslots(const void* q, const void* k, const void* v, void* o, int B, int H, int Lq, int Lk,
                                   int D, const int64_t* q_strides, const int64_t* k_strides, const int64_t* v_strides,
                                   const int64_t* o_strides, float q_norm_bound, float k_norm_bound,
                                   const float* k_norm_slots, int n_slots, int n_split, void* workspace,
                                   size_t ws_bytes, hipStream_t stream);

int cp25_attn_fwd_prescaled_qnorm(const void* q, const void* k, const void* v, void* o, int B, int H, int Lq, int Lk,
                                  int D, const int64_t* q_strides, const int64_t* k_strides, const int64_t* v_strides,
                                  const int64_t* o_strides, float q_norm_bound, float k_norm_bound,
                                  const float* k_norm_slots, int n_slots, const void* q_norm_weight,
                                  const float* cos_tab, const float* sin_tab, float eps, float q_scale, int n_split,
                                  void* workspace, size_t ws_bytes, hipStream_t stream);

int cp25_cast_fp8_e4m3(const void* src, int64_t src_stride, void* dst, int64_t dst_stride, int64_t n_rows,
                       int64_t width, float scale, hipStream_t stream);

int cp25_attn_fwd_prescaled_fp8qk(const void* q8, const void* k8, const void* v, void* o, int B, int H, int Lq, int Lk,
                                  int D, const int64_t* q_strides, const int64_t* k_strides, const int64_t* v_strides,
                                  const int64_t* o_strides, float q_norm_bound, float k_norm_bound, int n_split,
                                  void* workspace, size_t ws_bytes, hipStream_t stream);

int64_t cp25_v_fp8t_bytes(int B, int H, int L);
int cp25_cast_v_fp8t(const void* v, const int64_t* v_strides, int B, int H, int L, int D, void* v8t, float* v_amax,
                     hipStream_t stream);

int cp25_attn_fwd_prescaled_fp8(const void* q8, const void* k8, const void* v8t, const float* v_amax, void* o, int B,
                                int H, int Lq, int Lk, int D, const int64_t* q_strides, const int64_t* k_strides,
                                const int64_t* o_strides, float q_norm_bound, float k_norm_bound, int n_split,
                                void* workspace, size_t ws_bytes, hipStream_t stream);

const char* cp25_attn_kernel(int Lk, float softmax_scale, float q_norm_bound, float k_norm_bound, int prescaled,
                             int fp8);

size_t cp25_attn_workspace_bytes(int B, int H, int Lq, int n_split);

size_t cp25_attn_tail_workspace_bytes(int B, int H, int Lq, int Lk);

int cp25_attn_plan(int B, int H, int Lq, int Lk, int D);

int cp25_attn_cross_select(int form);

int cp25_attn_self_select(int form);

int cp25_attn_na3d(const void* q, const void* k, const void* v, void* o, int B, int H, int T, int Hg, int Wg, int D,
                   const int64_t* q_strides, const int64_t* k_strides, const int64_t* v_strides,
                   const int64_t* o_strides, const int* q_tok, const int* box, int n_tiles, int tile_rows,
                   const int* window, const int* dilation, float softmax_scale, int prescaled, hipStream_t stream);

int cp25_ln_mod(const void* x, int64_t x_st, int64_t x_sb, const void* y, const void* gate, const void* shift,
                const void* scale, int64_t mod_sb, int64_t mod_st, void* x_out, void* h_out, int64_t n_tok, int B,
                int D, int64_t tok0, int64_t hw, float eps, hipStream_t stream);

int cp25_ln_mod_fp8(const void* x, int64_t x_st, int64_t x_sb, const void* y, const void* gate, const void* shift,
                    const void* scale, int64_t mod_sb, int64_t mod_st, void* x_out, void* h8_out, float* h_scale,
                    int64_t n_tok, int B, int D, int64_t tok0, int64_t hw, float eps, hipStream_t stream);

int cp25_ln_mod_cam(const void* x, int64_t x_st, int64_t x_sb, const void* y, const void* gate, const void* shift,
                    const void* scale, int64_t mod_sb, int64_t mod_st, const void* cam, int64_t cam_st, int64_t cam_sb,
                    void* x_out, void* h_out, int64_t n_tok, int B, int D, int64_t tok0, int64_t hw, float eps,
                    hipStream_t stream);
int cp25_ln_mod_cam_fp8(const void* x, int64_t x_st, int64_t x_sb, const void* y, const void* gate, const void* shift,
                        const void* scale, int64_t mod_sb, int64_t mod_st, const void* cam, int64_t cam_st,
                        int64_t cam_sb, void* x_out, void* h8_out, float* h_scale, int64_t n_tok, int B, int D,
                        int64_t tok0, int64_t hw, float eps, hipStream_t stream);

int cp25_final_ln_mod(const void* x, const void* y, const void* gate, int64_t gmod_sb, int64_t gmod_st,
// ... 156 lines not shown
```

Baseline: 0.8376.

## Gate self-attention onto the wide-Q kernel with per-block fallback to m16 kernel

Adds a gated wide-Q attention path. A wide kernel (320/384 query rows) runs first and, per query block, checks a norm-bound gate. It writes a flag to a workspace array and finishes the rows it can handle safely. A second m16 kernel then reprocesses only the blocks flagged as needing the safe path and exits early for the rest. The intent is to use the faster wide kernel on most self-attention blocks while keeping correctness for outliers, at the cost of an extra launch, a flag workspace and more routing complexity.

```diff
diff --git a/cosmos-predict2.5_amd/cosmos_predict2/_native.py b/cosmos-predict2.5_amd/cosmos_predict2/_native.py
--- a/cosmos-predict2.5_amd/cosmos_predict2/_native.py
+++ b/cosmos-predict2.5_amd/cosmos_predict2/_native.py
@@ -75,8 +75,11 @@
     "cp25_cast_v_fp8t": [_P, c_int64_p, _I, _I, _I, _I, _P, _P, _P],
     "cp25_attn_fwd_prescaled_qnorm": [_P, _P, _P, _P, _I, _I, _I, _I, _I, c_int64_p, c_int64_p, c_int64_p, c_int64_p, _F,
                                       _F, _P, _I, _P, _P, _P, _F, _F, _I, _P, ctypes.c_size_t, _P],
+    "cp25_attn_fwd_prescaled_gate": [_P, _P, _P, _P, _I, _I, _I, _I, _I, c_int64_p, c_int64_p, c_int64_p, c_int64_p, _F,
+                                     _F, _P, _I, _P, _P, _P, _F, _F, _I, _I, _P, ctypes.c_size_t, _P],
     "cp25_attn_workspace_bytes": [_I, _I, _I, _I],
     "cp25_attn_tail_workspace_bytes": [_I, _I, _I, _I],
+    "cp25_attn_gate_workspace_bytes": [_I, _I, _I, _I],
     "cp25_attn_kernel": [_I, _F, _F, _F, _I, _I],
     "cp25_attn_plan": [_I, _I, _I, _I, _I],
     "cp25_attn_na3d": [_P, _P, _P, _P, _I, _I, _I, _I, _I, _I, c_int64_p, c_int64_p, c_int64_p, c_int64_p, _P, _P, _I, _I,
@@ -167,7 +170,8 @@
             raise RuntimeError(f"libcp25.so does not export {name}")
         if argtypes is not None:
             fn.argtypes = argtypes
-        fn.restype = {"cp25_attn_workspace_bytes": ctypes.c_size_t, "cp25_attn_tail_workspace_bytes": ctypes.c_size_t, "cp25_v_fp8t_bytes": ctypes.c_int64,
+        fn.restype = {"cp25_attn_workspace_bytes": ctypes.c_size_t, "cp25_attn_tail_workspace_bytes": ctypes.c_size_t,
+                      "cp25_attn_gate_workspace_bytes": ctypes.c_size_t, "cp25_v_fp8t_bytes": ctypes.c_int64,
                       "cp25_gemm_f32_workspace_floats": ctypes.c_int64,
                       "cp25_gemm_sm_workspace_bytes": ctypes.c_int64,
                       "cp25_attn_kernel": ctypes.c_char_p,
@@ -265,12 +269,27 @@
     return n
 
 
+def _check_q_norm(q_norm: dict, q: torch.Tensor, Lq: int, D: int):
+    w, cos, sin = q_norm["weight"], q_norm.get("cos"), q_norm.get("sin")
+    if w.dtype != torch.bfloat16 or w.numel() != D or not w.is_contiguous() or w.device != q.device:
+        raise ValueError("q_norm: weight must be a contiguous bf16 [128] device tensor")
+    if (cos is None) != (sin is None):
+        raise ValueError("q_norm: cos and sin go together")
+    if cos is not None:
+        for t in (cos, sin):
+            if t.dtype != torch.float32 or not t.is_contiguous() or t.dim() != 2 or t.shape[1] != 64 or \
+                    t.shape[0] < Lq or t.device != q.device:
+                raise ValueError(f"q_norm: cos/sin must be contiguous float32 [>= {Lq}, 64] device tables")
+    return w, cos, sin
+
+
 def attn_fwd(q: torch.Tensor, k: torch.Tensor, v: torch.Tensor, out: Optional[torch.Tensor] = None,
              softmax_scale: Optional[float] = None, n_split: Optional[int] = None,
              norm_bounds: Optional[Tuple[float, float]] = None, prescaled: bool = False,
              fp8_qk: Optional[Tuple[torch.Tensor, torch.Tensor]] = None,
              fp8_v: Optional[Tuple[torch.Tensor, torch.Tensor]] = None,
-             k_norm_slots: Optional[torch.Tensor] = None, q_norm: Optional[dict] = None) -> torch.Tensor:
+             k_norm_slots: Optional[torch.Tensor] = None, q_norm: Optional[dict] = None, gate_wide: bool = False,
+             gate_workspace: Optional[torch.Tensor] = None) -> torch.Tensor:
     lib = load_library()
     if q.dtype != torch.bfloat16 or k.dtype != torch.bfloat16 or v.dtype != torch.bfloat16:
         raise ValueError("attn_fwd expects bf16 q/k/v (attention() recasts to bf16 first)")
@@ -327,17 +346,27 @@
         if k_norm_slots is not None:
             if k_norm_slots.dtype != torch.float32 or k_norm_slots.numel() != 2048 or not k_norm_slots.is_contiguous():
                 raise ValueError("k_norm_slots: a contiguous float32 [64, 32] slot buffer expected")
+        if gate_wide and k_norm_slots is not None:
+            if n_split == 1:
+                if gate_workspace is None:
+                    nb = lib.cp25_attn_gate_workspace_bytes(B, H, Lq, Lk)
+                    gate_workspace = torch.empty(((nb + 3) // 4,), dtype=torch.int32, device=q.device) if nb else None
+                elif gate_workspace.dtype != torch.int32 or not gate_workspace.is_contiguous() or \
+                        gate_workspace.device != q.device:
+                    raise ValueError("gate_workspace: a contiguous int32 device tensor expected")
+                ws, ws_bytes = gate_workspace, (0 if gate_workspace is None else gate_workspace.numel() * 4)
+            w = cos = sin = None
+            if q_norm is not None:
+                w, cos, sin = _check_q_norm(q_norm, q, Lq, D)
+            rc = lib.cp25_attn_fwd_prescaled_gate(
+                _ptr(q), _ptr(k), _ptr(v), _ptr(out), B, H, Lq, Lk, D, *strides, qb, kb, _ptr(k_norm_slots), 64,
+                _ptr(w), _ptr(cos), _ptr(sin), float(q_norm.get("eps", 1e-6)) if q_norm else 0.0,
+                float(q_norm.get("out_scale", 1.0)) if q_norm else 1.0, 1, int(n_split), _ptr(ws), ws_bytes,
+                _stream(q.device))
+            _check("cp25_attn_fwd_prescaled_gate", rc)
+            return out
         if q_norm is not None:
-            w, cos, sin = q_norm["weight"], q_norm.get("cos"), q_norm.get("sin")
-            if w.dtype != torch.bfloat16 or w.numel() != D or not w.is_contiguous() or w.device != q.device:
-                raise ValueError("q_norm: weight must be a contiguous bf16 [128] device tensor")
-            if (cos is None) != (sin is None):
-                raise ValueError("q_norm: cos and sin go together")
-            if cos is not None:
-                for t in (cos, sin):
-                    if t.dtype != torch.float32 or not t.is_contiguous() or t.dim() != 2 or t.shape[1] != 64 or \
-                            t.shape[0] < Lq or t.device != q.device:
-                        raise ValueError(f"q_norm: cos/sin must be contiguous float32 [>= {Lq}, 64] device tables")
+            w, cos, sin = _check_q_norm(q_norm, q, Lq, D)
             rc = lib.cp25_attn_fwd_prescaled_qnorm(
                 _ptr(q), _ptr(k), _ptr(v), _ptr(out), B, H, Lq, Lk, D, *strides, qb, kb, _ptr(k_norm_slots),
                 64 if k_norm_slots is not None else 0, _ptr(w), _ptr(cos), _ptr(sin), float(q_norm.get("eps", 1e-6)),
diff --git a/cosmos-predict2.5_amd/cosmos_predict2/dit.py b/cosmos-predict2.5_amd/cosmos_predict2/dit.py
--- a/cosmos-predict2.5_amd/cosmos_predict2/dit.py
+++ b/cosmos-predict2.5_amd/cosmos_predict2/dit.py
@@ -271,6 +271,7 @@
         self.attention_precision = "bf16"
         self.share_cfg_block0 = True
         self.data_tight_k_bound = True
+        self.gate_wide = True
         self.fused_q_norm = True
         self._x_embed_w128 = None
         self.stream_gemm = "tile256"
@@ -643,7 +644,7 @@
                 fp8 = 0 if qb * kb > 60.0 else (2 if self.attention_precision == "fp8" and 1.13 * qb * kb <= 30.0 else 1)
             pre = kw.get("prescaled", False)
             if name == "self" and self._k_slots(kw) is not None and self.cp_group is None:
-                pre = 2
+                pre = 3 if self.gate_wide else 2
             out[name] = N.attn_kernel_name(lk, kw.get("softmax_scale"), kw["norm_bounds"], pre, fp8)
         return out
 
@@ -1204,7 +1205,7 @@
                                             weight=p[pre + "self_attn.q_norm.weight"], cos=cos, sin=sin,
                                             out_scale=q_scale)
                     if kslots is not None:
-                        attn_kw = dict(attn_kw, k_norm_slots=kslots)
+                        attn_kw = dict(attn_kw, k_norm_slots=kslots, gate_wide=self.gate_wide)
                     q = qkv.view(n, Bs, 3 * D)[:, :, :D].view(n, Bs, H, hd).transpose(0, 1)
                     kk = qkv.view(n, Bs, 3 * D)[:, :, D:2 * D].view(n, Bs, H, hd).transpose(0, 1)
                     vv = qkv.view(n, Bs, 3 * D)[:, :, 2 * D:].view(n, Bs, H, hd).transpose(0, 1)
diff --git a/cosmos-predict2.5_amd/csrc/attn_common.h b/cosmos-predict2.5_amd/csrc/attn_common.h
--- a/cosmos-predict2.5_amd/csrc/attn_common.h
+++ b/cosmos-predict2.5_amd/csrc/attn_common.h
@@ -86,6 +86,8 @@
   const float* qn_sin;
   float qn_eps, qn_scale;
   int qn_row0;
+  int* gate_flags;
+  int gate_rows;
 #ifdef CP25_ATTN_PROBE
   unsigned long long* probe;
   int probe_t0, probe_wg;
@@ -100,5 +102,6 @@
 
 typedef void (*AttnKernel)(AttnArgs);
 AttnKernel wq_kernel(int rows, int mode, bool tail);
+AttnKernel wq_gate_kernel(int rows);
 
 }
diff --git a/cosmos-predict2.5_amd/csrc/attn_fwd.hip b/cosmos-predict2.5_amd/csrc/attn_fwd.hip
--- a/cosmos-predict2.5_amd/csrc/attn_fwd.hip
+++ b/cosmos-predict2.5_amd/csrc/attn_fwd.hip
@@ -137,6 +137,17 @@
     }
   };
 
+  int gate_f0 = 0, gate_f1 = 0, gate_row1 = 0;
+  if constexpr (kGate == 3) {
+    const int r0 = min(qb * kQBlk, a.Lq - 1), r1 = min(qb * kQBlk + kQBlk - 1, a.Lq - 1);
+    const int w0 = r0 / a.gate_rows, w1 = r1 / a.gate_rows;
+    const int* flags = a.gate_flags + (int64_t)bh * ((a.Lq + a.gate_rows - 1) / a.gate_rows);
+    gate_f0 = flags[w0];
+    gate_f1 = flags[w1];
+    gate_row1 = w1 * a.gate_rows;
+    if (gate_f0 != 2 && gate_f1 != 2) return;
+    if (w1 == w0) gate_row1 = 0x7fffffff;
+  }
   if constexpr (kDmaK) {
     if (group_b) {
       dma_tile(0, std::integral_constant<int, 0>{});
@@ -232,8 +243,10 @@
   }
 
   float gate_kbound = a.kbound;
-  if constexpr (kGate != 0) {
-    static_assert(kPre && !kPersist && ((kGate == 1 && kMode == 0) || (kGate == 2 && kMode == 2)), "gated pair");
+  static_assert(kGate == 0 || (kPre && !kPersist && ((kGate == 1 && kMode == 0) || (kGate == 2 && kMode == 2) ||
+                                                     (kGate == 3 && kMode == 2 && kKind == 0))),
+                "gated pair");
+  if constexpr (kGate == 1 || kGate == 2) {
     __shared__ float gate_max[kWaves];
     float km = lane < a.n_kslots ? a.kslots[32 * lane] : 0.f;
     float qm = 0.f;
@@ -671,6 +684,9 @@
     const float l_tot = lsum[qh][0];
     const float inv = 1.f / l_tot;
     if (q_row[qh] >= a.Lq) continue;
+    if constexpr (kGate == 3) {
+      if ((q_row[qh] < gate_row1 ? gate_f0 : gate_f1) != 2) continue;
+    }
     if (a.nsplit > 1) {
       const int64_t row = ((int64_t)(split * a.B + b) * a.H + h) * a.Lq + q_row[qh];
       float* op = a.o_part + row * kD + 4 * g;
@@ -1053,13 +1069,15 @@
   for (int rows : {320, 384})
     for (int mode : {0, 1})
       if (wq_kernel(rows, mode, false)) m |= wide_bit(rows, mode);
+  for (int rows : {320, 384})
+    if (wq_gate_kernel(rows)) m |= wide_gate_bit(rows);
   return m;
 }
 
 AttnQuery route_query(int Lk, bool prescaled, float softmax_scale, float q_norm_bound, float k_norm_bound, int fp8,
-                      bool has_kslots, bool has_qnorm, int n_split) {
+                      bool has_kslots, bool has_qnorm, int n_split, bool wide_gate = false) {
   return AttnQuery{Lk, prescaled, prescaled ? 1.f : softmax_scale * 1.4426950408889634f, q_norm_bound, k_norm_bound,
-                   fp8, has_kslots, has_qnorm, n_split, g_self_form, g_xattn_form, wide_built()};
+                   fp8, has_kslots, has_qnorm, n_split, g_self_form, g_xattn_form, wide_built(), wide_gate};
 }
 
 template <bool kPre, int kMode>
@@ -1088,6 +1106,7 @@
 }
 AttnKernel route_kernel(const AttnRoute& r, bool tail) {
   if (r.family == AttnFamily::f8) return f8_kernel(r);
+  if (r.family == AttnFamily::wq && r.gated) return attn_fwd_m16<0, true, 2, false, 3>;
   return r.family == AttnFamily::wq ? wq_kernel(r.rows, r.mode, tail) : m16_kernel(r, tail);
 }
 
@@ -1132,6 +1151,7 @@
   const float* v_amax;
   const float* kslots;
   int n_kslots;
+  bool wide_gate;
   const void* qn_w;
   const float *qn_cos, *qn_sin;
   float qn_eps, qn_scale;
@@ -1171,9 +1191,13 @@
       return CP25_ERR_INVAL;
   }
   const AttnQuery query = route_query(Lk, c.prescaled, c.softmax_scale, q_norm_bound, k_norm_bound, fp8,
-                                      c.kslots != nullptr, c.qn_w != nullptr, n_split);
+                                      c.kslots != nullptr, c.qn_w != nullptr, n_split, c.wide_gate);
   const AttnRoute route = attn_route(query);
   const int qblk = route.rows;
+  const bool wide_pair = route.family == AttnFamily::wq && route.gated;
+  if (wide_pair && (!c.workspace || ((uintptr_t)c.workspace & 3) ||
+                    c.ws_bytes < gate_workspace_bytes(B, H, Lq, qblk) || !wq_gate_kernel(qblk)))
+    return CP25_ERR_INVAL;
   const int64_t cus = num_cus();
   TailSeg tail[kMaxTailSegs];
   int n_tail = 0;
@@ -1208,6 +1232,8 @@
   a.qn_eps = c.qn_eps;
   a.qn_scale = c.qn_w ? c.qn_scale : 1.f;
   a.qn_row0 = 0;
+  a.gate_flags = wide_pair ? (int*)c.workspace : nullptr;
+  a.gate_rows = wide_pair ? qblk : 0;
 #ifdef CP25_ATTN_PROBE
   a.probe = g_probe;
   a.probe_t0 = g_probe_t0;
@@ -1215,9 +1241,16 @@
 #endif
   const int64_t nwg = (int64_t)a.nqb * B * H * n_split;
   if (nwg > 0x7fffffff) return CP25_ERR_INVAL;
-  const dim3 threads(route.threads);
+  dim3 threads(route.threads);
   int64_t grid = nwg;
-  if (route.gated) {
+  if (wide_pair) {
+    hipLaunchKernelGGL(wq_gate_kernel(qblk), dim3((unsigned)nwg), threads, 0, c.stream, a);
+    CP25_LAUNCH_CHECK();
+    a.nqb = (int)cdiv(Lq, kQBlk);
+    grid = (int64_t)a.nqb * B * H;
+    if (grid > 0x7fffffff) return CP25_ERR_INVAL;
+    threads = dim3(kThreads);
+  } else if (route.gated) {
     hipLaunchKernelGGL(m16_gate_fixed_kernel(route), dim3((unsigned)nwg), threads, 0, c.stream, a);
     CP25_LAUNCH_CHECK();
   } else if (route.persistent) {
@@ -1376,8 +1409,37 @@
                       .qn_w = q_norm_weight, .qn_cos = cos_tab, .qn_sin = sin_tab, .qn_eps = eps, .qn_scale = q_scale});
 }
 
+extern "C" size_t cp25_attn_gate_workspace_bytes(int B, int H, int Lq, int Lk) {
+  if (B <= 0 || H <= 0 || Lq <= 0 || Lk <= kCrossMaxKeys) return 0;
+  return std::max(gate_workspace_bytes(B, H, Lq, 320), gate_workspace_bytes(B, H, Lq, 384));
+}
+
+extern "C" int cp25_attn_fwd_prescaled_gate(const void* q, const void* k, const void* v, void* o, int B, int H, int Lq,
+                                            int Lk, int D, const int64_t* q_strides, const int64_t* k_strides,
+                                            const int64_t* v_strides, const int64_t* o_strides, float q_norm_bound,
+                                            float k_norm_bound, const float* k_norm_slots, int n_slots,
+                                            const void* q_norm_weight, const float* cos_tab, const float* sin_tab,
+                                            float eps, float q_scale, int wide_gate, int n_split, void* workspace,
+                                            size_t ws_bytes, hipStream_t stream) {
+  if (!k_norm_slots || n_slots < 1 || n_slots > 64 || ((uintptr_t)k_norm_slots & 3)) return CP25_ERR_INVAL;
+  if (q_norm_weight) {
+    if (((uintptr_t)q_norm_weight & 15) || (!cos_tab) != (!sin_tab) || !(eps >= 0.f) || !(q_scale > 0.f))
+      return CP25_ERR_INVAL;
+    if ((((uintptr_t)cos_tab) | ((uintptr_t)sin_tab)) & 15) return CP25_ERR_INVAL;
+  } else if (cos_tab || sin_tab) {
+    return CP25_ERR_INVAL;
+  }
+  return attn_launch({.q = q, .k = k, .v = v, .o = o, .B = B, .H = H, .Lq = Lq, .Lk = Lk, .D = D,
+                      .q_strides = q_strides, .k_strides = k_strides, .v_strides = v_strides, .o_strides = o_strides,
+                      .softmax_scale = kLn2, .q_norm_bound = q_norm_bound, .k_norm_bound = k_norm_bound,
+                      .n_split = n_split, .workspace = workspace, .ws_bytes = ws_bytes, .stream = stream,
+                      .prescaled = true, .kslots = k_norm_slots, .n_kslots = n_slots, .wide_gate = wide_gate != 0,
+                      .qn_w = q_norm_weight, .qn_cos = cos_tab, .qn_sin = sin_tab, .qn_eps = eps,
+                      .qn_scale = q_scale});
+}
+
 extern "C" const char* cp25_attn_kernel(int Lk, float softmax_scale, float q_norm_bound, float k_norm_bound,
                                         int prescaled, int fp8) {
   return attn_route_name(attn_route(route_query(Lk, prescaled != 0, softmax_scale, q_norm_bound, k_norm_bound, fp8,
-                                                prescaled == 2, false, 1)));
-}
+                                                prescaled >= 2, false, 1, prescaled == 3)));
+}
diff --git a/cosmos-predict2.5_amd/csrc/attn_route.h b/cosmos-predict2.5_amd/csrc/attn_route.h
--- a/cosmos-predict2.5_amd/csrc/attn_route.h
+++ b/cosmos-predict2.5_amd/csrc/attn_route.h
@@ -30,6 +30,7 @@
 constexpr unsigned wide_bit(int rows, int mode) {
   return (rows == 320 || rows == 384) && (mode == 0 || mode == 1) ? 1u << (2 * (rows == 384) + mode) : 0u;
 }
+constexpr unsigned wide_gate_bit(int rows) { return rows == 320 || rows == 384 ? 1u << (4 + (rows == 384)) : 0u; }
 
 struct AttnQuery {
   int Lk;
@@ -43,6 +44,7 @@
   int self_form;
   int cross_form;
   unsigned wide_built;
+  bool wide_gate = false;
 };
 
 struct AttnRoute {
@@ -76,6 +78,12 @@
   if (q.prescaled && q.has_kslots && (cross ? mode != 1 : mode == 2)) {
     r.gated = true;
     r.mode = 2;
+    const int rows = cross ? 0 : wide_rows_of(q.self_form, q.Lk);
+    if (q.wide_gate && q.n_split == 1 && rows && (q.wide_built & wide_gate_bit(rows))) {
+      r.family = AttnFamily::wq;
+      r.rows = rows;
+      r.threads = kWqThreads;
+    }
   } else if (q.fp8 != 0) {
     r.family = AttnFamily::f8;
     r.prescaled = true;
@@ -125,6 +133,10 @@
      "attn_fwd_wq<self, prescaled, 384 rows, fixed shift>"},
     {AttnFamily::wq, AttnKind::self, true, 1, false, false, 0, 384,
      "attn_fwd_wq<self, prescaled, 384 rows, zero shift>"},
+    {AttnFamily::wq, AttnKind::self, true, 2, true, false, 0, 320,
+     "attn_fwd_wq<self, prescaled, 320 rows, gated fixed shift> | attn_fwd_m16<online max>"},
+    {AttnFamily::wq, AttnKind::self, true, 2, true, false, 0, 384,
+     "attn_fwd_wq<self, prescaled, 384 rows, gated fixed shift> | attn_fwd_m16<online max>"},
     {AttnFamily::f8, AttnKind::self, true, 0, false, false, 1, 256, "attn_fwd_f8<self, fp8 Q K^T>"},
     {AttnFamily::f8, AttnKind::cross, true, 0, false, false, 1, 256, "attn_fwd_f8<cross, fp8 Q K^T>"},
     {AttnFamily::f8, AttnKind::self, true, 0, false, false, 3, 256, "attn_fwd_f8<self, fp8 Q K^T + fp8 P.V>"},
@@ -214,6 +226,10 @@
   return best;
 }
 
+inline size_t gate_workspace_bytes(int B, int H, int Lq, int rows) {
+  return rows > 0 ? (size_t)ceil_div(Lq, rows) * B * H * sizeof(int) : 0;
+}
+
 inline size_t tail_workspace_bytes(int B, int H, int Lq, int Lk, int self_form, int64_t cus) {
   TailSeg seg[kMaxTailSegs];
   size_t need = 0, best = 0;
diff --git a/cosmos-predict2.5_amd/csrc/attn_wide.hip b/cosmos-predict2.5_amd/csrc/attn_wide.hip
--- a/cosmos-predict2.5_amd/csrc/attn_wide.hip
+++ b/cosmos-predict2.5_amd/csrc/attn_wide.hip
@@ -1,460 +1,16 @@
-#include "attn_common.h"
+#include "attn_wide_body.h"
 
 namespace cp25attn {
 namespace {
 
-constexpr int kAheadWq = 2;
-constexpr int kRingWq = kAheadWq + 1;
-static_assert(kWqThreads == 4 * 64, "one wave per SIMD");
-
-constexpr int wq_stage(int nq) { return 17 * nq; }
-constexpr int wq_frag(int nq, int m) { return m < nq ? -1 : (m - nq) / nq; }
-constexpr int wq_qb(int nq, int m) { return m < nq ? m : (m - nq) % nq; }
-constexpr bool wq_read_gap(int nq, int m) { return m >= nq && (m - nq) % nq == 0; }
-constexpr int wq_sm_op(int nq, int m) {
-  if (wq_read_gap(nq, m)) return -1;
-  int idx = 0;
-  for (int x = 0; x < m; ++x) idx += !wq_read_gap(nq, x);
-  return idx < 12 * nq ? idx : -1;
-}
-constexpr int wq_sm_count(int nq) {
-  int n = 0;
-  for (int m = 0; m < wq_stage(nq); ++m) n += wq_sm_op(nq, m) >= 0;
-  return n;
-}
-static_assert(wq_sm_count(5) == 60 && wq_sm_count(6) == 72, "every softmax instruction has a gap");
-constexpr int wq_dma_at(int nq, int M) {
-  return M < wq_stage(nq) && wq_read_gap(nq, M) && wq_frag(nq, M) < 10 ? wq_frag(nq, M) : -1;
-}
-constexpr int wq_m0_at(int nq, int M) { return wq_dma_at(nq, M + 1); }
-
-__device__ __forceinline__ u32x4 tile_rsrc(const char* base, int64_t sl, int rows) {
-  const uint64_t p = (uint64_t)base;
-  const unsigned n = rows > 0 ? (unsigned)((rows - 1) * sl * 2 + 2 * kD) : 0u;
-  return u32x4{(unsigned)p, (unsigned)(p >> 32) & 0xffffu, n, 0x00020000u};
-}
-
-#define WQ_MFMA "v_mfma_f32_16x16x32_bf16 "
-
 template <int kNQ, int kMode, int kTail = 0>
 __global__ void __launch_bounds__(kWqThreads, 1) attn_fwd_wq(AttnArgs a) {
-  static_assert(kMode == 0 || kMode == 1, "kMode: 0 fixed shift, 1 zero shift");
-  static_assert(kNQ >= 4 && kNQ <= 6, "query blocks per wave");
   __shared__ __attribute__((aligned(16))) char smem[kLds16];
-  constexpr bool kInit = kMode != 1;
-  constexpr int KB1 = kKBuf16, VB0 = 2 * kKBuf16;
-  constexpr int kR = kRingWq;
-  constexpr int kRowsW = 16 * kNQ;
-  constexpr int kRowsG = 4 * kRowsW;
-  constexpr int kNS = wq_stage(kNQ);
-  constexpr int kQA = (256 - 36 * kNQ - 4) / 16 < kNQ ? (256 - 36 * kNQ - 4) / 16 : kNQ;
-
-  const int tile = xcd_remap(blockIdx.x, gridDim.x);
-  const int qblk = tile % a.nqb;
-  const int bhs = tile / a.nqb;
-  const int split = bhs % a.nsplit, bh = bhs / a.nsplit;
-  const int b = bh / a.H, h = bh % a.H;
-  const int key0 = split * a.tps * kKBlk;
-  const int Lk = min(a.Lk - key0, a.tps * kKBlk);
-  const int ntk = (Lk + kKBlk - 1) / kKBlk;
-  const int tid = threadIdx.x;
-  const int lane = tid & 63;
-  const int wave = __builtin_amdgcn_readfirstlane(tid >> 6);
-  const int c16 = lane & 15;
-  const int g = lane >> 4;
-  const int row_w = qblk * kRowsG + wave * kRowsW;
-
-  const unsigned short* qp = a.q + b * a.q_sb + h * a.q_sh;
-  const char* const kbase = (const char*)(a.k + b * a.k_sb + h * a.k_sh + (int64_t)key0 * a.k_sl);
-  const char* const vbase = (const char*)(a.v + b * a.v_sb + h * a.v_sh + (int64_t)key0 * a.v_sl);
-
-  int dk[5], dv[5];
-#pragma unroll
-  for (int j = 0; j < 5; ++j) {
-    const int bb = 1024 * (wave + 4 * j) + 16 * lane;
-    const int row = bb / kKStride16, cb = bb - row * kKStride16;
-    dk[j] = cb < 2 * kD ? row * (int)(a.k_sl * 2) + cb : 0;
-    dv[j] = cb < 2 * kD ? row * (int)(a.v_sl * 2) + cb : 0;
-  }
-  const unsigned lds_wave = (unsigned)(uintptr_t)(lds_char_ptr)smem + 1024u * (unsigned)wave;
-  auto k_rsrc = [&](int t) __attribute__((always_inline)) {
-    return tile_rsrc(kbase + (int64_t)t * kKBlk * a.k_sl * 2, a.k_sl, min(Lk - t * kKBlk, kKBlk));
-  };
-  auto v_rsrc = [&](int t) __attribute__((always_inline)) {
-    return tile_rsrc(vbase + (int64_t)t * kKBlk * a.v_sl * 2, a.v_sl, min(Lk - t * kKBlk, kKBlk));
-  };
-  auto set_m0 = [&](unsigned dst, auto OFFC) __attribute__((always_inline)) {
-    asm volatile("s_add_u32 m0, %0, %1" ::"s"(dst), "i"(decltype(OFFC)::value) : "memory");
-  };
-  auto dma_load = [&](const u32x4& rs, int off) __attribute__((always_inline)) {
-    asm volatile("buffer_load_dwordx4 %0, %1, 0 offen lds" ::"v"(off), "s"(rs) : "memory");
-  };
-  auto dma_tile = [&](const u32x4& rs, const int* offs, unsigned dst) __attribute__((always_inline)) {
-    static_for<5>([&](auto JC) __attribute__((always_inline)) {
-      constexpr int j = decltype(JC)::value;
-      if (j < 4 || wave < 2) {
-        set_m0(dst, std::integral_constant<int, 4096 * j>{});
-        asm volatile("s_nop 0" ::: "memory");
-        dma_load(rs, offs[j]);
-      }
-    });
-  };
-
-  dma_tile(k_rsrc(0), dk, lds_wave);
-  dma_tile(k_rsrc(1), dk, lds_wave + KB1);
-  dma_tile(v_rsrc(0), dv, lds_wave + VB0);
-
-  bf16x8 qa[kNQ][4];
-#pragma unroll
-  for (int qb = 0; qb < kNQ; ++qb) {
-    const int r = row_w + 16 * qb + c16;
-    const unsigned short* src = qp + (int64_t)min(r, a.Lq - 1) * a.q_sl + 8 * g;
-#pragma unroll
-    for (int s = 0; s < 4; ++s) qa[qb][s] = *reinterpret_cast<const bf16x8*>(src + 32 * s);
-  }
-  if (a.qn_w != nullptr) {
-    bf16x8 wv[4];
-#pragma unroll
-    for (int s = 0; s < 4; ++s) wv[s] = *reinterpret_cast<const bf16x8*>(a.qn_w + 32 * s + 8 * g);
-    const bool rope = a.qn_cos != nullptr;
-    const f32x2 scale2 = {a.qn_scale, a.qn_scale};
-#pragma unroll
-    for (int qb = 0; qb < kNQ; ++qb) {
-      const int r = row_w + 16 * qb + c16;
-      f32x4 rc[2][2], rsn[2][2];
-      if (rope) {
-        const int64_t t0 = (a.qn_row0 + min(r, a.Lq - 1)) * 64 + 8 * g;
-#pragma unroll
-        for (int s1 = 0; s1 < 2; ++s1)
-#pragma unroll
-          for (int hf = 0; hf < 2; ++hf) {
-            rc[s1][hf] = *reinterpret_cast<const f32x4*>(a.qn_cos + t0 + 32 * s1 + 4 * hf);
-            rsn[s1][hf] = *reinterpret_cast<const f32x4*>(a.qn_sin + t0 + 32 * s1 + 4 * hf);
-          }
-      }
-      f32x2 x[4][4];
-#pragma unroll
-      for (int s = 0; s < 4; ++s)
-#pragma unroll
-        for (int q = 0; q < 4; ++q)
-          x[s][q] = f32x2{static_cast<float>(qa[qb][s][2 * q]), static_cast<float>(qa[qb][s][2 * q + 1])};
-      f32x2 c01[8], c23[8];
-#pragma unroll
-      for (int e = 0; e < 8; ++e) {
-        c01[e] = f32x2{x[0][e >> 1][e & 1], x[1][e >> 1][e & 1]};
-        c23[e] = f32x2{x[2][e >> 1][e & 1], x[3][e >> 1][e & 1]};
-      }
-      const f32x2 p01 = hn2_sumsq8(c01), p23 = hn2_sumsq8(c23);
-      const f32x2 aa = p01 + p23;
-      float ss = aa.x + aa.y;
-      ss += __shfl_xor(ss, 32);
-      ss += __shfl_xor(ss, 16);
-      const float rstd = hn_rstd(ss, a.qn_eps);
-      const f32x2 rstd2 = {rstd, rstd};
-#pragma unroll
-      for (int s = 0; s < 4; ++s)
-#pragma unroll
-        for (int q = 0; q < 4; ++q)
-          x[s][q] = hn2_norm(x[s][q], rstd2,
-                             f32x2{static_cast<float>(wv[s][2 * q]), static_cast<float>(wv[s][2 * q + 1])});
-      f32x2 y[4][4];
-#pragma unroll
-      for (int s = 0; s < 4; ++s)
-#pragma unroll
-        for (int q = 0; q < 4; ++q) y[s][q] = x[s][q];
-      if (rope) {
-#pragma unroll
-        for (int s = 0; s < 4; ++s)
-#pragma unroll
-          for (int q = 0; q < 4; ++q) {
-            const f32x4 cc = rc[s & 1][q >> 1], sn = rsn[s & 1][q >> 1];
-            const int o = 2 * (q & 1);
-            y[s][q] = hn2_rope(x[s][q], x[s ^ 2][q], s < 2 ? -1.f : 1.f, f32x2{cc[o], cc[o + 1]},
-                               f32x2{sn[o], sn[o + 1]});
-          }
-      }
-#pragma unroll
-      for (int s = 0; s < 4; ++s)
-#pragma unroll
-        for (int q = 0; q < 4; ++q) {
-          const bf16x2v hh = __builtin_convertvector(y[s][q] * scale2, bf16x2v);
-          qa[qb][s][2 * q] = hh.x;
-          qa[qb][s][2 * q + 1] = hh.y;
-        }
-    }
-  }
-
-  float m_run[kNQ];
-#pragma unroll
-  for (int qb = 0; qb < kNQ; ++qb) m_run[qb] = 0.f;
-  if constexpr (kMode == 0) {
-#pragma unroll
-    for (int qb = 0; qb < kNQ; ++qb) {
-      float qq = 0.f;
-#pragma unroll
-      for (int s = 0; s < 4; ++s)
-#pragma unroll
-        for (int e = 0; e < 8; ++e) {
-          const float x = static_cast<float>(qa[qb][s][e]);
-          qq = fmaf(x, x, qq);
-        }
-      const float b_row = sqrtf(group4_sum(qq)) * a.kbound;
-      m_run[qb] = floorf(fminf(b_row + kPDrop, 126.f - b_row));
-    }
-  }
-  f32x4 minit[kNQ];
-#pragma unroll
-  for (int qb = 0; qb < kNQ; ++qb) {
-    minit[qb] = f32x4{-m_run[qb], -m_run[qb], -m_run[qb], -m_run[qb]};
-    asm volatile("" : "+v"(minit[qb]));
-  }
-
-  f32x4 oacc[8][kNQ], lacc[kNQ];
-#pragma unroll
-  for (int db = 0; db < 8; ++db)
-#pragma unroll
-    for (int qb = 0; qb < kNQ; ++qb) {
-      oacc[db][qb] = f32x4{0.f, 0.f, 0.f, 0.f};
-      asm volatile("s_nop 2" : "+a"(oacc[db][qb]));
-    }
-#pragma unroll
-  for (int qb = 0; qb < kNQ; ++qb) {
-    lacc[qb] = f32x4{0.f, 0.f, 0.f, 0.f};
-    asm volatile("s_nop 2" : "+a"(lacc[qb]));
-  }
-  static_for<kNQ>([&](auto QC) __attribute__((always_inline)) {
-    constexpr int qb = decltype(QC)::value;
-    (void)qa;
-#pragma unroll
-    for (int s = 0; s < 4; ++s) {
-      if constexpr (qb < kQA) asm volatile("s_nop 2" : "+a"(qa[qb][s]));
-      else asm volatile("s_nop 2" : "+v"(qa[qb][s]));
-    }
-  });
-  typedef short s16x8v __attribute__((ext_vector_type(8)));
-  bf16x8 ones8 = __builtin_bit_cast(bf16x8, s16x8v{0x3f80, 0x3f80, 0x3f80, 0x3f80, 0x3f80, 0x3f80, 0x3f80, 0x3f80});
-  asm volatile("s_nop 2" : "+a"(ones8));
-  const unsigned k_rd_lds = (unsigned)(uintptr_t)(lds_char_ptr)(smem + c16 * kKStride16 + 16 * g);
-  const unsigned v_rd_lds =
-      (unsigned)(uintptr_t)(lds_char_ptr)(smem + VB0 + (4 * g + (c16 >> 2)) * kVStride16 + 8 * (c16 & 3));
-
-  f32x4 S[2][2][kNQ];
-  bf16x8 P[2][kNQ];
-  bf16x8 ring[kR];
-  float ex[2];
-  unsigned pk[4];
-  unsigned k_cur = 0, v_cur = 0;
-
-  auto issue = [&](auto FC, auto SLOTC) __attribute__((always_inline)) {
-    constexpr int F = decltype(FC)::value, slot = decltype(SLOTC)::value;
-    constexpr int st = F / 16, f = F % 16;
-    (void)ring;
-    (void)k_cur;
-    (void)v_cur;
-    if constexpr (f >= 8) {
-      constexpr int j = f - 8;
-      constexpr int off = (2 * st + (j & 1)) * 16 * kKStride16 + 64 * (j >> 1);
-      asm volatile("ds_read_b128 %0, %1 offset:%2" : "=v"(ring[slot]) : "v"(k_cur), "i"(off));
-    } else {
-      constexpr int off = 32 * st * kVStride16 + 32 * f;
-      s16x4 lo, hi;
-      asm volatile("ds_read_b64_tr_b16 %0, %1 offset:%2" : "=v"(lo) : "v"(v_cur), "i"(off));
-      asm volatile("ds_read_b64_tr_b16 %0, %1 offset:%2" : "=v"(hi) : "v"(v_cur), "i"(off + 16 * kVStride16));
-      typedef short s16x8 __attribute__((ext_vector_type(8)));
-      const s16x8 r = {lo[0], lo[1], lo[2], lo[3], hi[0], hi[1], hi[2], hi[3]};
-      ring[slot] = __builtin_bit_cast(bf16x8, r);
-    }
-  };
-
-  auto mask_keys = [&](auto SPC, int k0) __attribute__((always_inline)) {
-    constexpr int SP = decltype(SPC)::value;
-    if (__builtin_expect(k0 + 32 > Lk, 0)) {
-      asm volatile("s_nop 15\n\ts_nop 15" ::: "memory");
-#pragma unroll
-      for (int kbl = 0; kbl < 2; ++kbl)
-#pragma unroll
-        for (int i = 0; i < 4; ++i)
-          if (k0 + 16 * kbl + 4 * g + i >= Lk) {
-#pragma unroll
-            for (int qb = 0; qb < kNQ; ++qb) S[SP][kbl][qb][i] = -INFINITY;
-          }
-    }
-  };
-
-  auto body = [&](auto FULLC, int t) __attribute__((always_inline)) {
-    constexpr bool FULL = decltype(FULLC)::value;
-    constexpr int NF = FULL ? 32 : 16;
-    constexpr auto frag_of = [](int n) constexpr { return FULL ? n : (n < 8 ? 8 + n : 16 + n); };
-    constexpr auto seq_of = [](int F) constexpr { return FULL ? F : (F < 16 ? F - 8 : F - 16); };
-    constexpr auto nreads = [](int F) constexpr { return F % 16 < 8 ? 2 : 1; };
-    k_cur = k_rd_lds + (((t + 1) & 1) ? (unsigned)KB1 : 0u);
-    v_cur = v_rd_lds + ((t & 1) ? (unsigned)kVBuf16 : 0u);
-    u32x4 rk = {0u, 0u, 0u, 0u}, rv = {0u, 0u, 0u, 0u};
-    unsigned dst_k = 0, dst_v = 0;
-    if constexpr (FULL) {
-      mask_keys(std::integral_constant<int, 1>{}, 64 * t + 32);
-      rk = k_rsrc(t + 2);
-      rv = v_rsrc(t + 1);
-      dst_k = lds_wave + ((t & 1) ? (unsigned)KB1 : 0u);
-      dst_v = lds_wave + (unsigned)VB0 + (((t + 1) & 1) ? (unsigned)kVBuf16 : 0u);
-    }
-    static_for<kAheadWq>([&](auto IC) __attribute__((always_inline)) {
-      constexpr int n = decltype(IC)::value;
-      issue(std::integral_constant<int, frag_of(n)>{}, std::integral_constant<int, n % kR>{});
-    });
-    __builtin_amdgcn_sched_barrier(0);
-    static_for<2 * kNS>([&](auto MC) __attribute__((always_inline)) {
-      constexpr int M = decltype(MC)::value;
-      constexpr int st = M / kNS, m = M % kNS;
-      constexpr int f = wq_frag(kNQ, m), qb = wq_qb(kNQ, m);
-      constexpr int F = 16 * st + (f < 0 ? 0 : f);
-      constexpr bool has_mfma = f >= 8 || FULL;
-      constexpr bool has_sm = st == 1 || FULL;
-      (void)S;
-      (void)ex;
-      (void)pk;
-      (void)oacc;
-      (void)lacc;
-      (void)ones8;
-      (void)P;
-      (void)minit;
-      (void)qa;
-      (void)ring;
-      (void)rk;
-      (void)rv;
-      (void)dst_k;
-      (void)dst_v;
-      if constexpr (m == 0 && st == 1) {
-        if constexpr (!FULL) asm volatile("s_nop 15" ::: "memory");
-        mask_keys(std::integral_constant<int, 0>{}, 64 * (t + 1));
-        __builtin_amdgcn_sched_barrier(0);
-      }
-      if constexpr (has_mfma) {
-        if constexpr (f >= 0 && qb == 0) {
-          constexpr int n = seq_of(F);
-          constexpr int pending = [=]() constexpr {
-            int p = 0;
-            for (int i = 1; i < kAheadWq; ++i)
-              if (n + i < NF) p += nreads(frag_of(n + i));
-            return p;
-          }();
-          asm volatile("s_waitcnt lgkmcnt(%0)" ::"i"(pending), "v"(ring[n % kR]) : "memory");
-        }
-        if constexpr (f < 0) {
-          asm volatile(WQ_MFMA "%0, %1, %2, %0" : "+a"(lacc[qb]) : "a"(ones8), "v"(P[st][qb]));
-        } else if constexpr (f < 8) {
-          asm volatile(WQ_MFMA "%0, %1, %2, %0" : "+a"(oacc[f][qb]) : "v"(ring[seq_of(F) % kR]), "v"(P[st][qb]));
-        } else {
-          constexpr int kbl = (f - 8) & 1, s = (f - 8) >> 1;
-          constexpr int ri = seq_of(F) % kR;
-          if constexpr (qb < kQA) {
-            if constexpr (s == 0 && kInit)
-              asm volatile(WQ_MFMA "%0, %1, %2, %3"
-                           : "=&v"(S[st][kbl][qb]) : "v"(ring[ri]), "a"(qa[qb][s]), "v"(minit[qb]));
-            else if constexpr (s == 0)
-              asm volatile(WQ_MFMA "%0, %1, %2, 0" : "=&v"(S[st][kbl][qb]) : "v"(ring[ri]), "a"(qa[qb][s]));
-            else
-              asm volatile(WQ_MFMA "%0, %1, %2, %0" : "+v"(S[st][kbl][qb]) : "v"(ring[ri]), "a"(qa[qb][s]));
-          } else {
-            if constexpr (s == 0 && kInit)
-              asm volatile(WQ_MFMA "%0, %1, %2, %3"
-                           : "=&v"(S[st][kbl][qb]) : "v"(ring[ri]), "v"(qa[qb][s]), "v"(minit[qb]));
-            else if constexpr (s == 0)
-              asm volatile(WQ_MFMA "%0, %1, %2, 0" : "=&v"(S[st][kbl][qb]) : "v"(ring[ri]), "v"(qa[qb][s]));
-            else
-              asm volatile(WQ_MFMA "%0, %1, %2, %0" : "+v"(S[st][kbl][qb]) : "v"(ring[ri]), "v"(qa[qb][s]));
-          }
-        }
-      }
-      __builtin_amdgcn_sched_barrier(0);
-      if constexpr (has_mfma && f >= 0 && qb == 0) {
-        constexpr int n = seq_of(F) + kAheadWq;
-        if constexpr (n < NF) issue(std::integral_constant<int, frag_of(n)>{}, std::integral_constant<int, n % kR>{});
-      }
-      if constexpr (FULL) {
-        constexpr int dm = wq_m0_at(kNQ, M), dl = wq_dma_at(kNQ, M);
-        if constexpr (dm >= 0) {
-          constexpr int j = dm % 5;
-          if (j < 4 || wave < 2) set_m0(dm < 5 ? dst_k : dst_v, std::integral_constant<int, 4096 * j>{});
-        }
-        if constexpr (dl >= 0) {
-          constexpr int j = dl % 5;
-          if (j < 4 || wave < 2) dma_load(dl < 5 ? rk : rv, dl < 5 ? dk[j] : dv[j]);
-        }
-      }
-      if constexpr (has_sm) {
-        if constexpr (!has_mfma) asm volatile("s_nop 1" ::: "memory");
-        constexpr int op = wq_sm_op(kNQ, m);
-        if constexpr (op >= 0) {
-          constexpr int q = op / 12, r = op % 12, pair = r / 3, w = r % 3;
-          if constexpr (w < 2) {
-            constexpr int j = 2 * pair + w;
-            asm volatile("v_exp_f32 %0, %1" : "=v"(ex[w]) : "v"(S[1 - st][j >> 2][q][j & 3]));
-          } else {
-            pk[pair] = __builtin_bit_cast(unsigned, __builtin_convertvector(f32x2{ex[0], ex[1]}, bf16x2v));
-            asm volatile("" ::"v"(pk[pair]));
-            if constexpr (pair == 3) P[1 - st][q] = __builtin_bit_cast(bf16x8, u32x4{pk[0], pk[1], pk[2], pk[3]});
-          }
-        }
-      }
-      __builtin_amdgcn_sched_barrier(0);
-    });
-    if constexpr (FULL) {
-      static_for<kNQ>([&](auto QC) __attribute__((always_inline)) {
-        constexpr int qb = decltype(QC)::value;
-        (void)P;
-        asm volatile("" ::"v"(P[0][qb]), "v"(P[1][qb]));
-      });
-    }
-    asm volatile("s_waitcnt vmcnt(0)" ::: "memory");
-    __builtin_amdgcn_s_barrier();
-    __builtin_amdgcn_sched_barrier(0);
-  };
-
-  asm volatile("s_waitcnt vmcnt(0) lgkmcnt(0)" ::: "memory");
-  __builtin_amdgcn_s_barrier();
-  body(std::false_type{}, -1);
-  for (int t = 0; t < ntk; ++t) body(std::true_type{}, t);
-
-  asm volatile("s_nop 15\n\ts_nop 15" ::: "memory");
-#pragma unroll
-  for (int db = 0; db < 8; ++db)
-#pragma unroll
-    for (int qb = 0; qb < kNQ; ++qb) asm volatile("s_nop 0" : "+a"(oacc[db][qb]));
-#pragma unroll
-  for (int qb = 0; qb < kNQ; ++qb) asm volatile("s_nop 0" : "+a"(lacc[qb]));
-#pragma unroll
-  for (int qb = 0; qb < kNQ; ++qb) {
-    const int q_row = row_w + 16 * qb + c16;
-    const float l_tot = lacc[qb][0];
-    float inv = 1.f / l_tot;
-    if (l_tot > 3.0e38f) inv = __uint_as_float(0x7fc00000u);
-    if (q_row >= a.Lq) continue;
-    if (a.nsplit > 1) {
-      const int64_t row = ((int64_t)(split * a.B + b) * a.H + h) * a.Lq + q_row;
-      float* op = a.o_part + row * kD + 4 * g;
-#pragma unroll
-      for (int db = 0; db < 8; ++db) {
-        f32x4 w;
-#pragma unroll
-        for (int e = 0; e < 4; ++e) w[e] = oacc[db][qb][e] * inv;
-        *reinterpret_cast<f32x4*>(op + 16 * db) = w;
-      }
-      if (g == 0) a.lse_part[row] = m_run[qb] + __log2f(l_tot);
-    } else {
-      unsigned short* op = a.o + b * a.o_sb + h * a.o_sh + (int64_t)q_row * a.o_sl + 4 * g;
-#pragma unroll
-      for (int db = 0; db < 8; ++db) {
-        u16x4 w;
-#pragma unroll
-        for (int e = 0; e < 4; ++e) w[e] = f2bf(oacc[db][qb][e] * inv);
-        *reinterpret_cast<u16x4*>(op + 16 * db) = w;
-      }
-    }
-  }
+  constexpr int kGate = 0;
+  float* const gate_max = nullptr;
+  (void)gate_max;
+#include "attn_wide_body.inc"
 }
-
-#undef WQ_MFMA
 
 }
 
diff --git a/cosmos-predict2.5_amd/csrc/attn_wide_body.h b/cosmos-predict2.5_amd/csrc/attn_wide_body.h
--- /dev/null
+++ b/cosmos-predict2.5_amd/csrc/attn_wide_body.h
@@ -0,0 +1,39 @@
+#pragma once
+#include "attn_common.h"
+
+namespace cp25attn {
+namespace {
+
+constexpr int kAheadWq = 2;
+constexpr int kRingWq = kAheadWq + 1;
+static_assert(kWqThreads == 4 * 64, "one wave per SIMD");
+
+constexpr int wq_stage(int nq) { return 17 * nq; }
+constexpr int wq_frag(int nq, int m) { return m < nq ? -1 : (m - nq) / nq; }
+constexpr int wq_qb(int nq, int m) { return m < nq ? m : (m - nq) % nq; }
+constexpr bool wq_read_gap(int nq, int m) { return m >= nq && (m - nq) % nq == 0; }
+constexpr int wq_sm_op(int nq, int m) {
+  if (wq_read_gap(nq, m)) return -1;
+  int idx = 0;
+  for (int x = 0; x < m; ++x) idx += !wq_read_gap(nq, x);
+  return idx < 12 * nq ? idx : -1;
+}
+constexpr int wq_sm_count(int nq) {
+  int n = 0;
+  for (int m = 0; m < wq_stage(nq); ++m) n += wq_sm_op(nq, m) >= 0;
+  return n;
+}
+static_assert(wq_sm_count(5) == 60 && wq_sm_count(6) == 72, "every softmax instruction has a gap");
+constexpr int wq_dma_at(int nq, int M) {
+  return M < wq_stage(nq) && wq_read_gap(nq, M) && wq_frag(nq, M) < 10 ? wq_frag(nq, M) : -1;
+}
+constexpr int wq_m0_at(int nq, int M) { return wq_dma_at(nq, M + 1); }
+
+__device__ __forceinline__ u32x4 tile_rsrc(const char* base, int64_t sl, int rows) {
+  const uint64_t p = (uint64_t)base;
+  const unsigned n = rows > 0 ? (unsigned)((rows - 1) * sl * 2 + 2 * kD) : 0u;
+  return u32x4{(unsigned)p, (unsigned)(p >> 32) & 0xffffu, n, 0x00020000u};
+}
+
+}
+}
diff --git a/cosmos-predict2.5_amd/csrc/attn_wide_body.inc b/cosmos-predict2.5_amd/csrc/attn_wide_body.inc
--- /dev/null
+++ b/cosmos-predict2.5_amd/csrc/attn_wide_body.inc
@@ -0,0 +1,449 @@
+  static_assert(kMode == 0 || kMode == 1, "kMode: 0 fixed shift, 1 zero shift");
+  static_assert(kNQ >= 4 && kNQ <= 6, "query blocks per wave");
+  static_assert(kGate == 0 || (kGate == 1 && kMode == 0), "kGate 1: the gated pair's first launch, fixed shift");
+#define WQ_MFMA "v_mfma_f32_16x16x32_bf16 "
+  constexpr bool kInit = kMode != 1;
+  constexpr int KB1 = kKBuf16, VB0 = 2 * kKBuf16;
+  constexpr int kR = kRingWq;
+  constexpr int kRowsW = 16 * kNQ;
+  constexpr int kRowsG = 4 * kRowsW;
+  constexpr int kNS = wq_stage(kNQ);
+  constexpr int kQA = (256 - 36 * kNQ - 4) / 16 < kNQ ? (256 - 36 * kNQ - 4) / 16 : kNQ;
+
+  const int tile = xcd_remap(blockIdx.x, gridDim.x);
+  const int qblk = tile % a.nqb;
+  const int bhs = tile / a.nqb;
+  const int split = bhs % a.nsplit, bh = bhs / a.nsplit;
+  const int b = bh / a.H, h = bh % a.H;
+  const int key0 = split * a.tps * kKBlk;
+  const int Lk = min(a.Lk - key0, a.tps * kKBlk);
+  const int ntk = (Lk + kKBlk - 1) / kKBlk;
+  const int tid = threadIdx.x;
+  const int lane = tid & 63;
+  const int wave = __builtin_amdgcn_readfirstlane(tid >> 6);
+  const int c16 = lane & 15;
+  const int g = lane >> 4;
+  const int row_w = qblk * kRowsG + wave * kRowsW;
+
+  const unsigned short* qp = a.q + b * a.q_sb + h * a.q_sh;
+  const char* const kbase = (const char*)(a.k + b * a.k_sb + h * a.k_sh + (int64_t)key0 * a.k_sl);
+  const char* const vbase = (const char*)(a.v + b * a.v_sb + h * a.v_sh + (int64_t)key0 * a.v_sl);
+
+  int dk[5], dv[5];
+#pragma unroll
+  for (int j = 0; j < 5; ++j) {
+    const int bb = 1024 * (wave + 4 * j) + 16 * lane;
+    const int row = bb / kKStride16, cb = bb - row * kKStride16;
+    dk[j] = cb < 2 * kD ? row * (int)(a.k_sl * 2) + cb : 0;
+    dv[j] = cb < 2 * kD ? row * (int)(a.v_sl * 2) + cb : 0;
+  }
+  const unsigned lds_wave = (unsigned)(uintptr_t)(lds_char_ptr)smem + 1024u * (unsigned)wave;
+  auto k_rsrc = [&](int t) __attribute__((always_inline)) {
+    return tile_rsrc(kbase + (int64_t)t * kKBlk * a.k_sl * 2, a.k_sl, min(Lk - t * kKBlk, kKBlk));
+  };
+  auto v_rsrc = [&](int t) __attribute__((always_inline)) {
+    return tile_rsrc(vbase + (int64_t)t * kKBlk * a.v_sl * 2, a.v_sl, min(Lk - t * kKBlk, kKBlk));
+  };
+  auto set_m0 = [&](unsigned dst, auto OFFC) __attribute__((always_inline)) {
+    asm volatile("s_add_u32 m0, %0, %1" ::"s"(dst), "i"(decltype(OFFC)::value) : "memory");
+  };
+  auto dma_load = [&](const u32x4& rs, int off) __attribute__((always_inline)) {
+    asm volatile("buffer_load_dwordx4 %0, %1, 0 offen lds" ::"v"(off), "s"(rs) : "memory");
+  };
+  auto dma_tile = [&](const u32x4& rs, const int* offs, unsigned dst) __attribute__((always_inline)) {
+    static_for<5>([&](auto JC) __attribute__((always_inline)) {
+      constexpr int j = decltype(JC)::value;
+      if (j < 4 || wave < 2) {
+        set_m0(dst, std::integral_constant<int, 4096 * j>{});
+        asm volatile("s_nop 0" ::: "memory");
+        dma_load(rs, offs[j]);
+      }
+    });
+  };
+
+  dma_tile(k_rsrc(0), dk, lds_wave);
+  dma_tile(k_rsrc(1), dk, lds_wave + KB1);
+  dma_tile(v_rsrc(0), dv, lds_wave + VB0);
+
+  bf16x8 qa[kNQ][4];
+#pragma unroll
+  for (int qb = 0; qb < kNQ; ++qb) {
+    const int r = row_w + 16 * qb + c16;
+    const unsigned short* src = qp + (int64_t)min(r, a.Lq - 1) * a.q_sl + 8 * g;
+#pragma unroll
+    for (int s = 0; s < 4; ++s) qa[qb][s] = *reinterpret_cast<const bf16x8*>(src + 32 * s);
+  }
+  if (a.qn_w != nullptr) {
+    bf16x8 wv[4];
+#pragma unroll
+    for (int s = 0; s < 4; ++s) wv[s] = *reinterpret_cast<const bf16x8*>(a.qn_w + 32 * s + 8 * g);
+    const bool rope = a.qn_cos != nullptr;
+    const f32x2 scale2 = {a.qn_scale, a.qn_scale};
+#pragma unroll
+    for (int qb = 0; qb < kNQ; ++qb) {
+      const int r = row_w + 16 * qb + c16;
+      f32x4 rc[2][2], rsn[2][2];
+      if (rope) {
+        const int64_t t0 = (a.qn_row0 + min(r, a.Lq - 1)) * 64 + 8 * g;
+#pragma unroll
+        for (int s1 = 0; s1 < 2; ++s1)
+#pragma unroll
+          for (int hf = 0; hf < 2; ++hf) {
+            rc[s1][hf] = *reinterpret_cast<const f32x4*>(a.qn_cos + t0 + 32 * s1 + 4 * hf);
+            rsn[s1][hf] = *reinterpret_cast<const f32x4*>(a.qn_sin + t0 + 32 * s1 + 4 * hf);
+          }
+      }
+      f32x2 x[4][4];
+#pragma unroll
+      for (int s = 0; s < 4; ++s)
+#pragma unroll
+        for (int q = 0; q < 4; ++q)
+          x[s][q] = f32x2{static_cast<float>(qa[qb][s][2 * q]), static_cast<float>(qa[qb][s][2 * q + 1])};
+      f32x2 c01[8], c23[8];
+#pragma unroll
+      for (int e = 0; e < 8; ++e) {
+        c01[e] = f32x2{x[0][e >> 1][e & 1], x[1][e >> 1][e & 1]};
+        c23[e] = f32x2{x[2][e >> 1][e & 1], x[3][e >> 1][e & 1]};
+      }
+      const f32x2 p01 = hn2_sumsq8(c01), p23 = hn2_sumsq8(c23);
+      const f32x2 aa = p01 + p23;
+      float ss = aa.x + aa.y;
+      ss += __shfl_xor(ss, 32);
+      ss += __shfl_xor(ss, 16);
+      const float rstd = hn_rstd(ss, a.qn_eps);
+      const f32x2 rstd2 = {rstd, rstd};
+#pragma unroll
+      for (int s = 0; s < 4; ++s)
+#pragma unroll
+        for (int q = 0; q < 4; ++q)
+          x[s][q] = hn2_norm(x[s][q], rstd2,
+                             f32x2{static_cast<float>(wv[s][2 * q]), static_cast<float>(wv[s][2 * q + 1])});
+      f32x2 y[4][4];
+#pragma unroll
+      for (int s = 0; s < 4; ++s)
+#pragma unroll
+        for (int q = 0; q < 4; ++q) y[s][q] = x[s][q];
+      if (rope) {
+#pragma unroll
+        for (int s = 0; s < 4; ++s)
+#pragma unroll
+          for (int q = 0; q < 4; ++q) {
+            const f32x4 cc = rc[s & 1][q >> 1], sn = rsn[s & 1][q >> 1];
+            const int o = 2 * (q & 1);
+            y[s][q] = hn2_rope(x[s][q], x[s ^ 2][q], s < 2 ? -1.f : 1.f, f32x2{cc[o], cc[o + 1]},
+                               f32x2{sn[o], sn[o + 1]});
+          }
+      }
+#pragma unroll
+      for (int s = 0; s < 4; ++s)
+#pragma unroll
+        for (int q = 0; q < 4; ++q) {
+          const bf16x2v hh = __builtin_convertvector(y[s][q] * scale2, bf16x2v);
+          qa[qb][s][2 * q] = hh.x;
+          qa[qb][s][2 * q + 1] = hh.y;
+        }
+    }
+  }
+
+  float m_run[kNQ];
+#pragma unroll
+  for (int qb = 0; qb < kNQ; ++qb) m_run[qb] = 0.f;
+  if constexpr (kMode == 0) {
+    float kbound = a.kbound;
+    if constexpr (kGate == 1) {
+      float km = lane < a.n_kslots ? a.kslots[32 * lane] : 0.f;
+      float qm = 0.f;
+#pragma unroll
+      for (int qb = 0; qb < kNQ; ++qb) {
+        float qq = 0.f;
+#pragma unroll
+        for (int s = 0; s < 4; ++s)
+#pragma unroll
+          for (int e = 0; e < 8; ++e) {
+            const float x = static_cast<float>(qa[qb][s][e]);
+            qq = fmaf(x, x, qq);
+          }
+        qm = fmaxf(qm, sqrtf(group4_sum(qq)));
+      }
+#pragma unroll
+      for (int m = 32; m >= 1; m >>= 1) {
+        km = fmaxf(km, __shfl_xor(km, m));
+        qm = fmaxf(qm, __shfl_xor(qm, m));
+      }
+      if (lane == 0) gate_max[wave] = qm;
+      __syncthreads();
+#pragma unroll
+      for (int w = 0; w < 4; ++w) qm = fmaxf(qm, gate_max[w]);
+      const bool fixed_ok = km > 0.f && qm * km * 1.001f <= kGateFixed;
+      if (tid == 0) a.gate_flags[tile] = fixed_ok ? 1 : 2;
+      if (!fixed_ok) {
+        asm volatile("s_waitcnt vmcnt(0)" ::: "memory");
+        return;
+      }
+      kbound = km * 1.001f;
+    }
+#pragma unroll
+    for (int qb = 0; qb < kNQ; ++qb) {
+      float qq = 0.f;
+#pragma unroll
+      for (int s = 0; s < 4; ++s)
+#pragma unroll
+        for (int e = 0; e < 8; ++e) {
+          const float x = static_cast<float>(qa[qb][s][e]);
+          qq = fmaf(x, x, qq);
+        }
+      const float b_row = sqrtf(group4_sum(qq)) * kbound;
+      m_run[qb] = floorf(fminf(b_row + kPDrop, 126.f - b_row));
+    }
+  }
+  f32x4 minit[kNQ];
+#pragma unroll
+  for (int qb = 0; qb < kNQ; ++qb) {
+    minit[qb] = f32x4{-m_run[qb], -m_run[qb], -m_run[qb], -m_run[qb]};
+    asm volatile("" : "+v"(minit[qb]));
+  }
+
+  f32x4 oacc[8][kNQ], lacc[kNQ];
+#pragma unroll
+  for (int db = 0; db < 8; ++db)
+#pragma unroll
+    for (int qb = 0; qb < kNQ; ++qb) {
+      oacc[db][qb] = f32x4{0.f, 0.f, 0.f, 0.f};
+      asm volatile("s_nop 2" : "+a"(oacc[db][qb]));
+    }
+#pragma unroll
+  for (int qb = 0; qb < kNQ; ++qb) {
+    lacc[qb] = f32x4{0.f, 0.f, 0.f, 0.f};
+    asm volatile("s_nop 2" : "+a"(lacc[qb]));
+  }
+  static_for<kNQ>([&](auto QC) __attribute__((always_inline)) {
+    constexpr int qb = decltype(QC)::value;
+    (void)qa;
+#pragma unroll
+    for (int s = 0; s < 4; ++s) {
+      if constexpr (qb < kQA) asm volatile("s_nop 2" : "+a"(qa[qb][s]));
+      else asm volatile("s_nop 2" : "+v"(qa[qb][s]));
+    }
+  });
+  typedef short s16x8v __attribute__((ext_vector_type(8)));
+  bf16x8 ones8 = __builtin_bit_cast(bf16x8, s16x8v{0x3f80, 0x3f80, 0x3f80, 0x3f80, 0x3f80, 0x3f80, 0x3f80, 0x3f80});
+  asm volatile("s_nop 2" : "+a"(ones8));
+  const unsigned k_rd_lds = (unsigned)(uintptr_t)(lds_char_ptr)(smem + c16 * kKStride16 + 16 * g);
+  const unsigned v_rd_lds =
+      (unsigned)(uintptr_t)(lds_char_ptr)(smem + VB0 + (4 * g + (c16 >> 2)) * kVStride16 + 8 * (c16 & 3));
+
+  f32x4 S[2][2][kNQ];
+  bf16x8 P[2][kNQ];
+  bf16x8 ring[kR];
+  float ex[2];
+  unsigned pk[4];
+  unsigned k_cur = 0, v_cur = 0;
+
+  auto issue = [&](auto FC, auto SLOTC) __attribute__((always_inline)) {
+    constexpr int F = decltype(FC)::value, slot = decltype(SLOTC)::value;
+    constexpr int st = F / 16, f = F % 16;
+    (void)ring;
+    (void)k_cur;
+    (void)v_cur;
+    if constexpr (f >= 8) {
+      constexpr int j = f - 8;
+      constexpr int off = (2 * st + (j & 1)) * 16 * kKStride16 + 64 * (j >> 1);
+      asm volatile("ds_read_b128 %0, %1 offset:%2" : "=v"(ring[slot]) : "v"(k_cur), "i"(off));
+    } else {
+      constexpr int off = 32 * st * kVStride16 + 32 * f;
+      s16x4 lo, hi;
+      asm volatile("ds_read_b64_tr_b16 %0, %1 offset:%2" : "=v"(lo) : "v"(v_cur), "i"(off));
+      asm volatile("ds_read_b64_tr_b16 %0, %1 offset:%2" : "=v"(hi) : "v"(v_cur), "i"(off + 16 * kVStride16));
+      typedef short s16x8 __attribute__((ext_vector_type(8)));
+      const s16x8 r = {lo[0], lo[1], lo[2], lo[3], hi[0], hi[1], hi[2], hi[3]};
+      ring[slot] = __builtin_bit_cast(bf16x8, r);
+    }
+  };
+
+  auto mask_keys = [&](auto SPC, int k0) __attribute__((always_inline)) {
+    constexpr int SP = decltype(SPC)::value;
+    if (__builtin_expect(k0 + 32 > Lk, 0)) {
+      asm volatile("s_nop 15\n\ts_nop 15" ::: "memory");
+#pragma unroll
+      for (int kbl = 0; kbl < 2; ++kbl)
+#pragma unroll
+        for (int i = 0; i < 4; ++i)
+          if (k0 + 16 * kbl + 4 * g + i >= Lk) {
+#pragma unroll
+            for (int qb = 0; qb < kNQ; ++qb) S[SP][kbl][qb][i] = -INFINITY;
+          }
+    }
+  };
+
+  auto body = [&](auto FULLC, int t) __attribute__((always_inline)) {
+    constexpr bool FULL = decltype(FULLC)::value;
+    constexpr int NF = FULL ? 32 : 16;
+    constexpr auto frag_of = [](int n) constexpr { return FULL ? n : (n < 8 ? 8 + n : 16 + n); };
+    constexpr auto seq_of = [](int F) constexpr { return FULL ? F : (F < 16 ? F - 8 : F - 16); };
+    constexpr auto nreads = [](int F) constexpr { return F % 16 < 8 ? 2 : 1; };
+    k_cur = k_rd_lds + (((t + 1) & 1) ? (unsigned)KB1 : 0u);
+    v_cur = v_rd_lds + ((t & 1) ? (unsigned)kVBuf16 : 0u);
+    u32x4 rk = {0u, 0u, 0u, 0u}, rv = {0u, 0u, 0u, 0u};
+    unsigned dst_k = 0, dst_v = 0;
+    if constexpr (FULL) {
+      mask_keys(std::integral_constant<int, 1>{}, 64 * t + 32);
+      rk = k_rsrc(t + 2);
+      rv = v_rsrc(t + 1);
+      dst_k = lds_wave + ((t & 1) ? (unsigned)KB1 : 0u);
+      dst_v = lds_wave + (unsigned)VB0 + (((t + 1) & 1) ? (unsigned)kVBuf16 : 0u);
+    }
+    static_for<kAheadWq>([&](auto IC) __attribute__((always_inline)) {
+      constexpr int n = decltype(IC)::value;
+      issue(std::integral_constant<int, frag_of(n)>{}, std::integral_constant<int, n % kR>{});
+    });
+    __builtin_amdgcn_sched_barrier(0);
+    static_for<2 * kNS>([&](auto MC) __attribute__((always_inline)) {
+      constexpr int M = decltype(MC)::value;
+      constexpr int st = M / kNS, m = M % kNS;
+      constexpr int f = wq_frag(kNQ, m), qb = wq_qb(kNQ, m);
+      constexpr int F = 16 * st + (f < 0 ? 0 : f);
+      constexpr bool has_mfma = f >= 8 || FULL;
+      constexpr bool has_sm = st == 1 || FULL;
+      (void)S;
+      (void)ex;
+      (void)pk;
+      (void)oacc;
+      (void)lacc;
+      (void)ones8;
+      (void)P;
+      (void)minit;
+      (void)qa;
+      (void)ring;
+      (void)rk;
+      (void)rv;
+      (void)dst_k;
+      (void)dst_v;
+      if constexpr (m == 0 && st == 1) {
+        if constexpr (!FULL) asm volatile("s_nop 15" ::: "memory");
+        mask_keys(std::integral_constant<int, 0>{}, 64 * (t + 1));
+        __builtin_amdgcn_sched_barrier(0);
+      }
+      if constexpr (has_mfma) {
+        if constexpr (f >= 0 && qb == 0) {
+          constexpr int n = seq_of(F);
+          constexpr int pending = [=]() constexpr {
+            int p = 0;
+            for (int i = 1; i < kAheadWq; ++i)
+              if (n + i < NF) p += nreads(frag_of(n + i));
+            return p;
+          }();
+          asm volatile("s_waitcnt lgkmcnt(%0)" ::"i"(pending), "v"(ring[n % kR]) : "memory");
+        }
+        if constexpr (f < 0) {
+          asm volatile(WQ_MFMA "%0, %1, %2, %0" : "+a"(lacc[qb]) : "a"(ones8), "v"(P[st][qb]));
+        } else if constexpr (f < 8) {
+          asm volatile(WQ_MFMA "%0, %1, %2, %0" : "+a"(oacc[f][qb]) : "v"(ring[seq_of(F) % kR]), "v"(P[st][qb]));
+        } else {
+          constexpr int kbl = (f - 8) & 1, s = (f - 8) >> 1;
+          constexpr int ri = seq_of(F) % kR;
+          if constexpr (qb < kQA) {
+            if constexpr (s == 0 && kInit)
+              asm volatile(WQ_MFMA "%0, %1, %2, %3"
+                           : "=&v"(S[st][kbl][qb]) : "v"(ring[ri]), "a"(qa[qb][s]), "v"(minit[qb]));
+            else if constexpr (s == 0)
+              asm volatile(WQ_MFMA "%0, %1, %2, 0" : "=&v"(S[st][kbl][qb]) : "v"(ring[ri]), "a"(qa[qb][s]));
+            else
+              asm volatile(WQ_MFMA "%0, %1, %2, %0" : "+v"(S[st][kbl][qb]) : "v"(ring[ri]), "a"(qa[qb][s]));
+          } else {
+            if constexpr (s == 0 && kInit)
+              asm volatile(WQ_MFMA "%0, %1, %2, %3"
+                           : "=&v"(S[st][kbl][qb]) : "v"(ring[ri]), "v"(qa[qb][s]), "v"(minit[qb]));
+            else if constexpr (s == 0)
+              asm volatile(WQ_MFMA "%0, %1, %2, 0" : "=&v"(S[st][kbl][qb]) : "v"(ring[ri]), "v"(qa[qb][s]));
+            else
+              asm volatile(WQ_MFMA "%0, %1, %2, %0" : "+v"(S[st][kbl][qb]) : "v"(ring[ri]), "v"(qa[qb][s]));
+          }
+        }
+      }
+      __builtin_amdgcn_sched_barrier(0);
+      if constexpr (has_mfma && f >= 0 && qb == 0) {
+        constexpr int n = seq_of(F) + kAheadWq;
+        if constexpr (n < NF) issue(std::integral_constant<int, frag_of(n)>{}, std::integral_constant<int, n % kR>{});
+      }
+      if constexpr (FULL) {
+        constexpr int dm = wq_m0_at(kNQ, M), dl = wq_dma_at(kNQ, M);
+        if constexpr (dm >= 0) {
+          constexpr int j = dm % 5;
+          if (j < 4 || wave < 2) set_m0(dm < 5 ? dst_k : dst_v, std::integral_constant<int, 4096 * j>{});
+        }
+        if constexpr (dl >= 0) {
+          constexpr int j = dl % 5;
+          if (j < 4 || wave < 2) dma_load(dl < 5 ? rk : rv, dl < 5 ? dk[j] : dv[j]);
+        }
+      }
+      if constexpr (has_sm) {
+        if constexpr (!has_mfma) asm volatile("s_nop 1" ::: "memory");
+        constexpr int op = wq_sm_op(kNQ, m);
+        if constexpr (op >= 0) {
+          constexpr int q = op / 12, r = op % 12, pair = r / 3, w = r % 3;
+          if constexpr (w < 2) {
+            constexpr int j = 2 * pair + w;
+            asm volatile("v_exp_f32 %0, %1" : "=v"(ex[w]) : "v"(S[1 - st][j >> 2][q][j & 3]));
+          } else {
+            pk[pair] = __builtin_bit_cast(unsigned, __builtin_convertvector(f32x2{ex[0], ex[1]}, bf16x2v));
+            asm volatile("" ::"v"(pk[pair]));
+            if constexpr (pair == 3) P[1 - st][q] = __builtin_bit_cast(bf16x8, u32x4{pk[0], pk[1], pk[2], pk[3]});
+          }
+        }
+      }
+      __builtin_amdgcn_sched_barrier(0);
+    });
+    if constexpr (FULL) {
+      static_for<kNQ>([&](auto QC) __attribute__((always_inline)) {
+        constexpr int qb = decltype(QC)::value;
+        (void)P;
+        asm volatile("" ::"v"(P[0][qb]), "v"(P[1][qb]));
+      });
+    }
+    asm volatile("s_waitcnt vmcnt(0)" ::: "memory");
+    __builtin_amdgcn_s_barrier();
+    __builtin_amdgcn_sched_barrier(0);
+  };
+
+  asm volatile("s_waitcnt vmcnt(0) lgkmcnt(0)" ::: "memory");
+  __builtin_amdgcn_s_barrier();
+  body(std::false_type{}, -1);
+  for (int t = 0; t < ntk; ++t) body(std::true_type{}, t);
+
+  asm volatile("s_nop 15\n\ts_nop 15" ::: "memory");
+#pragma unroll
+  for (int db = 0; db < 8; ++db)
+#pragma unroll
+    for (int qb = 0; qb < kNQ; ++qb) asm volatile("s_nop 0" : "+a"(oacc[db][qb]));
+#pragma unroll
+  for (int qb = 0; qb < kNQ; ++qb) asm volatile("s_nop 0" : "+a"(lacc[qb]));
+#pragma unroll
+  for (int qb = 0; qb < kNQ; ++qb) {
+    const int q_row = row_w + 16 * qb + c16;
+    const float l_tot = lacc[qb][0];
+    float inv = 1.f / l_tot;
+    if (l_tot > 3.0e38f) inv = __uint_as_float(0x7fc00000u);
+    if (q_row >= a.Lq) continue;
+    if (a.nsplit > 1) {
+      const int64_t row = ((int64_t)(split * a.B + b) * a.H + h) * a.Lq + q_row;
+      float* op = a.o_part + row * kD + 4 * g;
+#pragma unroll
+      for (int db = 0; db < 8; ++db) {
+        f32x4 w;
+#pragma unroll
+        for (int e = 0; e < 4; ++e) w[e] = oacc[db][qb][e] * inv;
+        *reinterpret_cast<f32x4*>(op + 16 * db) = w;
+      }
+      if (g == 0) a.lse_part[row] = m_run[qb] + __log2f(l_tot);
+    } else {
+      unsigned short* op = a.o + b * a.o_sb + h * a.o_sh + (int64_t)q_row * a.o_sl + 4 * g;
+#pragma unroll
+      for (int db = 0; db < 8; ++db) {
+        u16x4 w;
+#pragma unroll
+        for (int e = 0; e < 4; ++e) w[e] = f2bf(oacc[db][qb][e] * inv);
+        *reinterpret_cast<u16x4*>(op + 16 * db) = w;
+      }
+    }
+  }
+#undef WQ_MFMA
diff --git a/cosmos-predict2.5_amd/csrc/attn_wide_gate.hip b/cosmos-predict2.5_amd/csrc/attn_wide_gate.hip
--- /dev/null
+++ b/cosmos-predict2.5_amd/csrc/attn_wide_gate.hip
@@ -0,0 +1,22 @@
+#include "attn_wide_body.h"
+
+namespace cp25attn {
+namespace {
+
+template <int kNQ>
+__global__ void __launch_bounds__(kWqThreads, 1) attn_fwd_gwq(AttnArgs a) {
+  __shared__ __attribute__((aligned(16))) char smem[kLds16];
+  __shared__ float gate_max[4];
+  constexpr int kMode = 0, kGate = 1;
+#include "attn_wide_body.inc"
+}
+
+}
+
+AttnKernel wq_gate_kernel(int rows) {
+  if (rows == 320) return attn_fwd_gwq<5>;
+  if (rows == 384) return attn_fwd_gwq<6>;
+  return nullptr;
+}
+
+}
diff --git a/include/cp25.h b/include/cp25.h
--- a/include/cp25.h
+++ b/include/cp25.h
@@ -63,6 +63,15 @@
                                   const float* cos_tab, const float* sin_tab, float eps, float q_scale, int n_split,
                                   void* workspace, size_t ws_bytes, hipStream_t stream);
 
+int cp25_attn_fwd_prescaled_gate(const void* q, const void* k, const void* v, void* o, int B, int H, int Lq, int Lk,
+                                 int D, const int64_t* q_strides, const int64_t* k_strides, const int64_t* v_strides,
+                                 const int64_t* o_strides, float q_norm_bound, float k_norm_bound,
+                                 const float* k_norm_slots, int n_slots, const void* q_norm_weight,
+                                 const float* cos_tab, const float* sin_tab, float eps, float q_scale, int wide_gate,
+                                 int n_split, void* workspace, size_t ws_bytes, hipStream_t stream);
+
+size_t cp25_attn_gate_workspace_bytes(int B, int H, int Lq, int Lk);
+
 int cp25_cast_fp8_e4m3(const void* src, int64_t src_stride, void* dst, int64_t dst_stride, int64_t n_rows,
                        int64_t width, float scale, hipStream_t stream);
 
```

New measurement: 0.8356. No clear change (-0.2%).
